# duanzhiihao/lossy-vae

Hardware: AMD Instinct MI355X
Metric: Mpixels/s enc+dec (qarv_base, 512x768) (higher is better)
Workload: dtype f32 (2-term fp16 split of every fp32 operand, hi + lo*2^-11 = 23 of 24 significant bits; 3 fp16 MFMAs per product step in two fp32 accumulators: fp32-class accuracy, parity-tested); 1 GPU; qarv_base batch=8 512x768 synthetic per GPU, compress_batch+decompress_batch, HIP kernels (f16x2) + host rANS, seeded random-init weights (profile typical); global_batch=8, parallelism=dp1 (images sharded, no data-path collective)

## Files before the change

### include/lvae_hip.h

```cpp
#ifndef LVAE_HIP_H
#define LVAE_HIP_H

#include <stddef.h>
#include <stdint.h>

#ifdef __cplusplus
extern "C" {
#endif

int lvae_abi_version(void);
const char* lvae_build_info(void);

int lvae_pmf_to_quantized_cdf(const float* pmf, int n, int precision, uint32_t* cdf_out);

int lvae_build_gaussian_tables(const float* scale_table, int n_scales, double multiplier, int cdf_form,
                               int32_t* qcdf, int row_stride, int32_t* cdf_len, int32_t* offset);

long lvae_rans_encode_with_indexes(const int32_t* sym, const uint8_t* idx, size_t n,
                                   const int32_t* qcdf, int row_stride, const int32_t* cdf_len,
                                   const int32_t* offset, uint8_t* out, size_t out_cap);

int lvae_rans_enc_step_selftest(uint64_t x, uint32_t start, uint32_t freq, uint64_t* by_division, uint64_t* by_reciprocal);

int lvae_rans_decode_with_indexes(const uint8_t* in, size_t in_len, const uint8_t* idx, size_t n,
                                  const int32_t* qcdf, int row_stride, const int32_t* cdf_len,
                                  const int32_t* offset, int32_t* sym_out);

int lvae_rans_encode_batch(int n_streams, const int32_t* const* sym, const uint8_t* const* idx, const size_t* n,
                           const int32_t* qcdf, int row_stride, const int32_t* cdf_len, const int32_t* offset,
                           uint8_t* const* out, const size_t* out_cap, long* out_len, int n_threads);
int lvae_rans_decode_batch(int n_streams, const uint8_t* const* in, const size_t* in_len,
                           const uint8_t* const* idx, const size_t* n,
                           const int32_t* qcdf, int row_stride, const int32_t* cdf_len, const int32_t* offset,
                           int32_t* const* sym_out, int* status, int n_threads);

enum {
    LVAE_STATUS_RANGE = 1, LVAE_STATUS_NONFINITE_PRIOR = 2, LVAE_STATUS_NONFINITE_LATENT = 4, LVAE_STATUS_NONFINITE_IMAGE = 8
};

enum {
    LVAE_A_PLAIN  = 0,
    LVAE_A_PATCH2 = 1,
    LVAE_A_CONV3  = 2
};
enum {
    LVAE_EPI_BIAS       = 0,
    LVAE_EPI_BIAS_GELU  = 1,
    LVAE_EPI_GAMMA_RES  = 2,
    LVAE_EPI_RES        = 3
};
enum {
    LVAE_ST_ROWMAJOR    = 0,
    LVAE_ST_SHUFFLE     = 2,
    LVAE_ST_IMAGE       = 3
};
typedef struct {
    const float* A0; const float* A1;
    long lda0, lda1;
    int  K0, K1;
    int  H, W;
    const float* Wt; long ldw;
    const float* bias;
    const float* gamma;
    const float* res; long ldres;
    float* out; long ldo;
    int  M, N, K;
    int  a_mode, epi, store, r;
    int  a_gelu;
    int  prec;
    const unsigned short* Wt16;
    int  cfg;
    int  ksplit;
    float* ws;
    int  a_bf16, out_bf16;
    int* cnt;
    int* status;
    int  a_h2, out_h2;
    int  defer_reduce;
} lvae_gemm_desc;
int lvae_gemm_f32(const lvae_gemm_desc* d, void* stream);

typedef struct {
    const void* y; const void* w1; const float* b1; const void* w2; const float* b2; const float* gamma;
    const float* res; float* out;
    int M, C, hid;
} lvae_mlp_desc;
int lvae_mlp_h2f(const lvae_mlp_desc* d, void* stream);

typedef struct {
    const void* y; const void* w1; const float* b1; const void* w2; const float* b2; const float* gamma;
    const float* res; float* out; float* ws;
    int M, C, hid, S1, S2;
} lvae_mlp_sk_desc;
int lvae_mlp_sk(const lvae_mlp_sk_desc* d, void* stream);
int lvae_mlp_sk_supported(int C, int hid, int S1, int S2);
int lvae_gemm_num_configs(void);

enum {
    LVAE_OP_GEMM = 1, LVAE_OP_DWCONV_LN_F32, LVAE_OP_DWCONV_LN_H2, LVAE_OP_DWCONV_LN_BF16, LVAE_OP_DWCONV_LN_Q8, LVAE_OP_STEM_F32, LVAE_OP_STEM_BF16,
    LVAE_OP_BIAS_EXPAND_F32, LVAE_OP_BIAS_EXPAND_BF16, LVAE_OP_PRIOR_INDEX, LVAE_OP_QUANTIZE, LVAE_OP_DEQUANTIZE, LVAE_OP_GAUSSIAN_NLL,
    LVAE_OP_LOSSLESS_PARAMS, LVAE_OP_LOSSLESS_OUTPUT, LVAE_OP_MLP_H2F, LVAE_OP_MLP_SK, LVAE_OP_PRIOR_INDEX_SK, LVAE_OP_QUANTIZE_SK,
    LVAE_OP_GAUSSIAN_NLL_CHAN, LVAE_OP_RD_IMAGE, LVAE_OP_PIXEL_NLL,
    LVAE_OP_DWCONV_LN_F32_V, LVAE_OP_DWCONV_LN_H2_V, LVAE_OP_DWCONV_LN_BF16_V, LVAE_OP_DWCONV_LN_Q8_V, LVAE_OP_ORDER
};
typedef struct { int kind; int side; void* p[8]; long i[6]; double f[2]; } lvae_op;
#define LVAE_TRACE_MAGIC 1985229328.0
int lvae_run_ops(const lvae_op* ops, int n, void* stream, void* side_stream, int* failed_index);

typedef struct {
    const lvae_op* ops; int n_ops;
    const uint8_t* idx_dev; uint8_t* idx_host;
    int32_t* sym_host; int32_t* sym_dev;
    size_t per_image;
} lvae_dec_block;
int lvae_decode_blocks(const lvae_dec_block* blocks, int n_blocks, int n_images, const uint8_t* const* strings, const size_t* string_len,
                       const int32_t* qcdf, int row_stride, const int32_t* cdf_len, const int32_t* offset,
                       const lvae_op* tail_ops, int n_tail, const int* status_dev, int* status_host, void* stream, void* side_stream,
                       int n_threads, int* failed_block, int* failed_op, double* seconds);

typedef struct {
    const lvae_op* ops; int n_ops;
    const int32_t* sym_dev; int32_t* sym_host;
    const uint8_t* idx_dev; uint8_t* idx_host;
    size_t per_image;
} lvae_enc_block;
int lvae_encode_blocks(const lvae_enc_block* blocks, int n_blocks, int n_images, uint8_t* const* out, const size_t* out_cap, long* out_len,
                       const int32_t* qcdf, int row_stride, const int32_t* cdf_len, const int32_t* offset,
                       const int* status_dev, int* status_host, void* stream, void* side_stream, int n_threads,
                       int* failed_block, int* failed_op, double* seconds);

int lvae_dwconv_ln_f32(const float* x, const float* wt, const float* bias, const float* ln_w, const float* ln_b,
                       const float* shift, const float* scale1p, float* y,
                       int B, int H, int W, int C, int k, void* stream);

int lvae_dwconv_ln_h2(const float* x, const float* wt, const float* bias, const float* ln_w, const float* ln_b,
                      const float* shift, const float* scale1p, void* y,
                      int B, int H, int W, int C, int k, void* stream);

int lvae_dwconv_ln_q8(const void* x, const float* wt, const float* bias, const float* ln_w, const float* ln_b,
                      const float* shift, const float* scale1p, void* y,
                      int B, int H, int W, int C, int k, void* stream);

int lvae_dwconv_ln_bf16(const void* x, const float* wt, const float* bias, const float* ln_w, const float* ln_b,
                        const float* shift, const float* scale1p, void* y,
                        int B, int H, int W, int C, int k, void* stream);

int lvae_dwconv_ln_f32_v(const float* x, const float* wt, const float* bias, const float* shift, const float* scale1p, float* y,
                         int B, int H, int W, int C, int k, long vstride, void* stream);
int lvae_dwconv_ln_h2_v(const float* x, const float* wt, const float* bias, const float* shift, const float* scale1p, void* y,
                        int B, int H, int W, int C, int k, long vstride, void* stream);
int lvae_dwconv_ln_bf16_v(const void* x, const float* wt, const float* bias, const float* shift, const float* scale1p, void* y,
                          int B, int H, int W, int C, int k, long vstride, void* stream);
int lvae_dwconv_ln_q8_v(const void* x, const float* wt, const float* bias, const float* shift, const float* scale1p, void* y,
                        int B, int H, int W, int C, int k, long vstride, void* stream);

int lvae_dwconv_ln_choice(int fmt, int affines, int per_image_vectors, int B, int H, int W, int C, int k,
                          int* family, int* tile_rows, int* tiles_per_wg);

int lvae_gemm_h2_choice(const lvae_gemm_desc* d, int cu_count, int* kernel, int* params , int* splitk);

int lvae_stem_bf16(const float* im, const float* wt, const float* bias, void* out,
                   int B, int H, int W, int Cout, float im_shift, float im_scale, int* range_flag, void* stream);
int lvae_bias_expand_bf16(const float* bias, void* out, long M, int C, void* stream);

int lvae_stem_f32(const float* im, const float* wt, const float* bias, float* out,
                  int B, int H, int W, int Cout, float im_shift, float im_scale, int* range_flag, void* stream);
int lvae_range_flag_f32(const float* x, long n, float lo, float hi, int* flag, void* stream);

int lvae_gemv_f32(const float* Wt, const float* b, const float* x, float* y, int N, int K,
                  int gelu_in, int gelu_out, void* stream);
int lvae_gemv_batch_f32(const float* Wt, const float* b, const float* x, float* y, int N, int K, int nvec,
                        int gelu_in, int gelu_out, void* stream);

int lvae_prior_index_f32(const float* prm, float* pm, uint8_t* idx, const float* scale_table, int n_scales,
                         float scale_bound, int B, int HW, int z, int* status, void* stream);
int lvae_prior_index_sk_f32(const float* ws, int S, const float* bias, float* prm, float* pm, uint8_t* idx, const float* scale_table,
                            int n_scales, float scale_bound, int B, int HW, int z, int* status, void* stream);

int lvae_quantize_f32(const float* qm, const float* pm, int32_t* sym, float* zhat, int B, int HW, int z, int ldz,
                      int* status, void* stream);
int lvae_quantize_sk_f32(const float* ws, int S, const float* bias, float* qm, const float* pm, int32_t* sym, float* zhat, int B, int HW,
                         int z, int ldz, int* status, void* stream);
int lvae_dequantize_f32(const int32_t* sym, const float* pm, float* zhat, int B, int HW, int z, int ldz, void* stream);

int lvae_prior_sample_f32(const float* prm, float* z, long M, int zdim, int ldz, float t, unsigned long long seed,
                          unsigned long long offset, void* stream);

int lvae_latent_sample_box_f32(const float* prm, const float* lat, float* z, int B, int h, int w, int zdim, int ldz, int r0, int r1,
                               int c0, int c1, float t, unsigned long long seed, unsigned long long offset, void* stream);

int lvae_pixel_sample_f32(const float* raw, float* out, int B, int H, int W, float t, unsigned long long seed, unsigned long long offset,
                          int* status, void* stream);

int lvae_lossless_params_f32(const float* raw, const float* im, float* pm, uint8_t* idx, int32_t* sym, const float* table,
                             int n_scales, float bound, int B, int H, int W, int* status, void* stream);

int lvae_lossless_output_f32(const int32_t* sym, const float* pm, float* out, long n, int* status, void* stream);

int lvae_gaussian_nll_f32(const float* prm, const int32_t* sym, double* out_nats, float scale_bound, int B, int HW, int z,
                          int cdf_form, void* stream);

int lvae_gaussian_nll_map_f32(const float* prm, const int32_t* sym, float* out, float scale_bound, int B, int HW, int z, int cdf_form,
                              void* stream);

#define LVAE_EVAL_CHUNKS 256

int lvae_gaussian_nll_chan_f32(const float* prm, const int32_t* sym, double* out, float scale_bound, int B, int HW, int z, int cdf_form,
                               void* stream);

int lvae_rd_image_f32(const float* raw, const float* im, float* im_hat, double* sums, double* ws, int B, int H, int W, int* status,
                      void* stream);

int lvae_pixel_nll_f32(const float* raw6, const float* im, float* im_hat, double* sums, double* ws, int B, int H, int W, int* status,
                       void* stream);

int lvae_gelu_f32(const float* x, float* y, long n, void* stream);

int lvae_bias_expand_f32(const float* bias, float* out, long M, int C, void* stream);

int lvae_sqerr_sum_f32(const float* a, const float* b, double* out, int B, long n_per_image, void* stream);
int lvae_sqerr_partials_f32(const float* a, const float* b, double* partials, int n_partials, long n, void* stream);

int lvae_msssim_f32(const float* x, long x_img, long x_plane, long x_row, const float* y, long y_img, long y_plane, long y_row,
                    const int* hw, int B, int C, int Hmax, int Wmax, double* out, double* scale_means, void* ws, size_t ws_bytes,
                    void* stream);
size_t lvae_msssim_workspace_bytes(int B, int C, int Hmax, int Wmax);

enum { LVAE_SAMPLE_F32 = 0, LVAE_SAMPLE_U8 = 1, LVAE_SAMPLE_U16_LOW = 2, LVAE_SAMPLE_U16_HIGH = 3 };
int lvae_msssim_planes(const void* const* x, const long* x_row, const void* const* y, const long* y_row, const int* hw,
                       const int* pixstride, int n, int kind, int depth, double data_range, int scales, double* out, double* scale_means,
                       void* ws, size_t ws_bytes, void* stream);
size_t lvae_msssim_planes_workspace_bytes(int n, int Hmax, int Wmax, int scales);

int lvae_image_u8_to_f32(const uint8_t* const* src, const long* src_row, const int* hw, int B, float* dst, long dst_img, int H, int W,
                         void* stream);
int lvae_image_f32_to_u8(const float* src, long src_img, long src_plane, long src_row, int H, int W, const int* hw, int B,
                         uint8_t* const* dst, const long* dst_row, void* stream);

enum { LVAE_YUV_I420 = 0, LVAE_YUV_NV12 = 1 };
enum { LVAE_YUV_BT601 = 0, LVAE_YUV_BT709 = 1 };
enum { LVAE_YUV_LIMITED = 0, LVAE_YUV_FULL = 1 };
enum { LVAE_YUV_NEAREST = 0, LVAE_YUV_BILINEAR = 1 };
int lvae_image_yuv420_to_f32(const uint8_t* const* y, const uint8_t* const* u, const uint8_t* const* v, const long* y_row,
                             const long* u_row, const long* v_row, const int* hw, int B, int fmt, int matrix, int range, int chroma,
                             float* dst, long dst_img, int H, int W, void* stream);
int lvae_image_f32_to_yuv420(const float* src, long src_img, long src_plane, long src_row, int H, int W, const int* hw, int B, int fmt,
                             int matrix, int range, uint8_t* const* y, uint8_t* const* u, uint8_t* const* v, const long* y_row,
                             const long* u_row, const long* v_row, void* stream);
int lvae_sse_u8(const uint8_t* const* a, const long* a_row, const uint8_t* const* b, const long* b_row, const int* hw, int n,
                uint64_t* out, void* stream);

enum { LVAE_YUV_SUB_420 = 0, LVAE_YUV_SUB_422 = 1, LVAE_YUV_SUB_444 = 2 };
enum { LVAE_YUV_SITING_CENTER = 0, LVAE_YUV_SITING_LEFT = 1 };
enum { LVAE_YUV_BT2020 = 2 };
int lvae_image_yuv_to_f32(const void* const* y, const void* const* u, const void* const* v, const long* y_row, const long* u_row,
                          const long* v_row, const int* hw, int B, int depth, int subsampling, int siting, int matrix, int range, int chroma,
                          float* dst, long dst_img, int H, int W, void* stream);
int lvae_image_f32_to_yuv(const float* src, long src_img, long src_plane, long src_row, int H, int W, const int* hw, int B, int depth,
                          int subsampling, int siting, int matrix, int range, void* const* y, void* const* u, void* const* v,
                          const long* y_row, const long* u_row, const long* v_row, void* stream);
int lvae_sse_u16(const uint16_t* const* a, const long* a_row, const uint16_t* const* b, const long* b_row, const int* hw, int n,
                 uint64_t* out, void* stream);

enum { LVAE_YUV_LAYOUT_PLANAR = 0, LVAE_YUV_LAYOUT_SEMIPLANAR = 1 };
int lvae_image_yuvsp_to_f32(const uint16_t* const* y, const uint16_t* const* uv, const long* y_row, const long* uv_row, const int* hw, int B,
                            int depth, int subsampling, int siting, int matrix, int range, int chroma, float* dst, long dst_img, int H, int W,
                            void* stream);
int lvae_image_f32_to_yuvsp(const float* src, long src_img, long src_plane, long src_row, int H, int W, const int* hw, int B, int depth,
                            int subsampling, int siting, int matrix, int range, uint16_t* const* y, uint16_t* const* uv, const long* y_row,
                            const long* uv_row, void* stream);

int lvae_tile_stitch(const float* const* tiles, long tile_plane, long tile_row, const int* oy, const int* ox, int rows, int cols,
                     int th, int tw, int overlap, int h, int w, int y0, int x0, int hh, int ww, void* dst, long dst_plane,
                     long dst_row, int out_u8, void* ws, size_t ws_bytes, void* stream);
size_t lvae_tile_stitch_workspace_bytes(int rows, int cols);
int lvae_tile_stitch_yuv(const float* const* tiles, long tile_plane, long tile_row, const int* oy, const int* ox, int rows, int cols, int th,
                         int tw, int overlap, int h, int w, int y0, int x0, int hh, int ww, int depth, int subsampling, int siting, int matrix,
                         int range, int layout, void* y, void* u, void* v, long y_row, long u_row, long v_row, void* ws, size_t ws_bytes,
                         void* stream);

int lvae_resample_u8_to_f32(const uint8_t* const* src, const long* src_row, int B, int h_in, int w_in, int h_out, int w_out,
                            const int* ystart, const float* ywgt, int ytaps, int yspan, const int* xstart, const float* xwgt, int xtaps,
                            float* dst, long dst_img, int H, int W, void* stream);
int lvae_resample_f32_to_u8(const float* src, long src_img, long src_plane, long src_row, int B, int h_in, int w_in, int h_out, int w_out,
                            const int* ystart, const float* ywgt, int ytaps, int yspan, const int* xstart, const float* xwgt, int xtaps,
                            uint8_t* const* dst, const long* dst_row, void* stream);
int lvae_resample_f32(const float* src, long src_img, long src_plane, long src_row, int B, int h_in, int w_in, int h_out, int w_out,
                      const int* ystart, const float* ywgt, int ytaps, int yspan, const int* xstart, const float* xwgt, int xtaps,
                      int clamp, float* dst, long dst_img, int H, int W, void* stream);

int lvae_resample_yuv_to_f32(const void* const* y, const void* const* u, const void* const* v, const long* y_row, const long* u_row,
                             const long* v_row, const int* hw, int B, int depth, int subsampling, int siting, int matrix, int range, int chroma,
                             int layout, int h_in, int w_in, int h_out, int w_out, const int* ystart, const float* ywgt, int ytaps, int yspan,
                             const int* xstart, const float* xwgt, int xtaps, int xspan, float* dst, long dst_img, int H, int W, void* stream);
int lvae_resample_f32_to_yuv(const float* src, long src_img, long src_plane, long src_row, const int* hw, int B, int depth, int subsampling,
                             int siting, int matrix, int range, int layout, int h_in, int w_in, int h_out, int w_out, const int* ystart,
                             const float* ywgt, int ytaps, int yspan, const int* xstart, const float* xwgt, int xtaps, void* const* y,
                             void* const* u, void* const* v, const long* y_row, const long* u_row, const long* v_row, void* stream);

int lvae_gaussian_nll_pos_f32(const float* prm, const int32_t* sym, double* out, float scale_bound, int B, int HW, int z, int cdf_form,
                              void* stream);
int lvae_pixel_nll_pos_f32(const float* raw6, const float* im, double* out, int B, int H, int W, int* status, void* stream);
int lvae_rate_map_f32(const double* const* pos, const int* lat_h, const int* lat_w, int n_blocks, const double* pix, int B, int H, int W,
                      float* out, long out_img, long out_row, int crop_h, int crop_w, void* stream);

void* lvae_event_create(void);
int   lvae_event_destroy(void* event);
int   lvae_stream_order(void* from_stream, void* to_stream, void* event);

#ifdef __cplusplus
}
#endif
#endif
```

### lossy-vae_amd/csrc/plan_runtime.cpp

```cpp
#include <hip/hip_runtime.h>

#include <chrono>
#include <vector>

#include "plan_ops.h"

extern "C" int lvae_run_ops(const lvae_op* ops, int n, void* stream, void* side_stream, int* failed_index) {
    if (!ops || n < 0) return -22;
    for (int k = 0; k < n; ++k) {
        const lvae_op& o = ops[k];
        int rc = -22;
        if (o.kind == LVAE_OP_ORDER)
            rc = o.i[0] ? lvae_stream_order(stream, side_stream, o.p[0]) : lvae_stream_order(side_stream, stream, o.p[0]);
        else if (o.kind >= 1 && o.kind <= lvae_plan::n_ops)
            rc = lvae_plan::op_table[o.kind - 1].run(o, o.side ? side_stream : stream);
        if (rc != 0) {
            if (failed_index) *failed_index = k;
            return rc;
        }
    }
    return 0;
}


struct LvaeDecTabs;
LvaeDecTabs* lvae_dec_tabs_new();
void lvae_dec_tabs_free(LvaeDecTabs* t);
int lvae_rans_decode_batch_tabs(int n_streams, const uint8_t* const* in, const size_t* in_len, const uint8_t* const* idx,
                                const size_t* n, const int32_t* qcdf, int row_stride, const int32_t* cdf_len, const int32_t* offset,
                                int32_t* const* sym_out, int* status, int n_threads, LvaeDecTabs* tabs);

struct LvaeEncJob;
LvaeEncJob* lvae_rans_encode_batch_begin(int n_streams, const int32_t* const* sym, const uint8_t* const* idx, const size_t* n,
                                         const int32_t* qcdf, int row_stride, const int32_t* cdf_len, const int32_t* offset,
                                         uint8_t* const* out, const size_t* out_cap, long* out_len, int n_threads);
int lvae_rans_encode_batch_end(LvaeEncJob* e);

namespace {
inline double now_s() { return std::chrono::duration<double>(std::chrono::steady_clock::now().time_since_epoch()).count(); }
}

static int decode_blocks_impl(const lvae_dec_block* blocks, int n_blocks, int n_images, const uint8_t* const* strings,
                              const size_t* string_len, const int32_t* qcdf, int row_stride, const int32_t* cdf_len,
                              const int32_t* offset, const lvae_op* tail_ops, int n_tail, const int* status_dev, int* status_host,
                              void* stream, void* side_stream, int n_threads, int* failed_block, int* failed_op, double* seconds) {
    if (!blocks || n_blocks < 0 || n_images <= 0 || !strings || !string_len || !qcdf || !cdf_len || !offset) return -22;
    hipStream_t st = (hipStream_t)stream;
    std::vector<const uint8_t*> idx_ptr(n_images);
    std::vector<int32_t*> out_ptr(n_images);
    std::vector<size_t> cnt(n_images);
    std::vector<int> status(n_images);
    struct TabsGuard { LvaeDecTabs* t; ~TabsGuard() { lvae_dec_tabs_free(t); } } tabs{lvae_dec_tabs_new()};
    if (!tabs.t) return -12;
    double t_gpu = 0.0, t_coder = 0.0;
    int bad = -1;
    const int trace_cap = (seconds && seconds[0] <= -8.0 && seconds[0] >= -4096.0 && seconds[1] == LVAE_TRACE_MAGIC) ? (int)(-seconds[0]) : 0;
    auto stamp = [&](int slot, double t) { if (slot < trace_cap) seconds[slot] = t; };
    for (int b = 0; b < n_blocks; ++b) {
        const lvae_dec_block& k = blocks[b];
        const double t0 = now_s();
        int rc = lvae_run_ops(k.ops, k.n_ops, stream, side_stream, &bad);
        if (rc == 0 && k.idx_dev) rc = (int)hipMemcpyAsync(k.idx_host, k.idx_dev, k.per_image * n_images, hipMemcpyDeviceToHost, st);
        const double t_issued = now_s();
        if (rc == 0) {
            hipError_t q = hipErrorNotReady;
            for (int it = 0; it < 400000 && (q = hipStreamQuery(st)) == hipErrorNotReady; ++it) {}
            rc = q == hipErrorNotReady ? (int)hipStreamSynchronize(st) : (int)q;
        }
        if (rc != 0) {
            if (failed_block) *failed_block = b;
            if (failed_op) *failed_op = bad;
            return rc;
        }
        const double t1 = now_s();
        for (int i = 0; i < n_images; ++i) {
            idx_ptr[i] = k.idx_host + (size_t)i * k.per_image;
            out_ptr[i] = k.sym_host + (size_t)i * k.per_image;
            cnt[i] = k.per_image;
        }
        rc = lvae_rans_decode_batch_tabs(n_images, strings + (size_t)b * n_images, string_len + (size_t)b * n_images, idx_ptr.data(), cnt.data(),
                                         qcdf, row_stride, cdf_len, offset, out_ptr.data(), status.data(), n_threads, tabs.t);
        if (rc != 0) {
            if (failed_block) *failed_block = b;
            if (status_dev && status_host && hipMemcpyAsync(status_host, status_dev, sizeof(int), hipMemcpyDeviceToHost, st) == hipSuccess &&
                hipStreamSynchronize(st) == hipSuccess && *status_host != 0)
                return -75;
            return -74;
        }
        if (k.sym_dev) rc = (int)hipMemcpyAsync(k.sym_dev, k.sym_host, k.per_image * n_images * sizeof(int32_t), hipMemcpyHostToDevice, st);
        if (rc != 0) {
            if (failed_block) *failed_block = b;
            return rc;
        }
        const double t2 = now_s();
        t_gpu += t1 - t0; t_coder += t2 - t1;
        stamp(2 + 4 * b, t0); stamp(3 + 4 * b, t_issued); stamp(4 + 4 * b, t1); stamp(5 + 4 * b, t2);
    }
    if (n_tail > 0) {
        int rc = lvae_run_ops(tail_ops, n_tail, stream, side_stream, &bad);
        if (rc == 0 && status_dev && status_host) rc = (int)hipMemcpyAsync(status_host, status_dev, sizeof(int), hipMemcpyDeviceToHost, st);
        if (rc != 0) {
            if (failed_block) *failed_block = n_blocks;
            if (failed_op) *failed_op = bad;
            return rc;
        }
    }
    stamp(2 + 4 * n_blocks, now_s());
    if (seconds) { seconds[0] = t_gpu; seconds[1] = t_coder; }
    return 0;
}

static int encode_blocks_impl(const lvae_enc_block* blocks, int n_blocks, int n_images, uint8_t* const* out, const size_t* out_cap,
                              long* out_len, const int32_t* qcdf, int row_stride, const int32_t* cdf_len, const int32_t* offset,
                              const int* status_dev, int* status_host, void* stream, void* side_stream, int n_threads,
                              int* failed_block, int* failed_op, double* seconds) {
    if (!blocks || n_blocks <= 0 || n_images <= 0 || !out || !out_cap || !out_len || !qcdf || !cdf_len || !offset) return -22;
    hipStream_t st = (hipStream_t)stream;
    std::vector<hipEvent_t> ev(n_blocks, nullptr);
    auto cleanup = [&]() { for (hipEvent_t e : ev) if (e) (void)hipEventDestroy(e); };
    const double t0 = now_s();
    int bad = -1;
    for (int b = 0; b < n_blocks; ++b) {
        const lvae_enc_block& k = blocks[b];
        int rc = lvae_run_ops(k.ops, k.n_ops, stream, side_stream, &bad);
        if (rc == 0 && k.sym_dev) rc = (int)hipMemcpyAsync(k.sym_host, k.sym_dev, k.per_image * n_images * sizeof(int32_t), hipMemcpyDeviceToHost, st);
        if (rc == 0 && k.idx_dev) rc = (int)hipMemcpyAsync(k.idx_host, k.idx_dev, k.per_image * n_images, hipMemcpyDeviceToHost, st);
        if (rc == 0 && b == n_blocks - 1 && status_dev && status_host) rc = (int)hipMemcpyAsync(status_host, status_dev, sizeof(int), hipMemcpyDeviceToHost, st);
        if (rc == 0) rc = (int)hipEventCreateWithFlags(&ev[b], hipEventDisableTiming);
        if (rc == 0) rc = (int)hipEventRecord(ev[b], st);
        if (rc != 0) {
            if (failed_block) *failed_block = b;
            if (failed_op) *failed_op = bad;
            (void)hipStreamSynchronize(st);
            cleanup();
            return rc;
        }
    }
    const double t1 = now_s();
    std::vector<const int32_t*> sym_ptr(n_images);
    std::vector<const uint8_t*> idx_ptr(n_images);
    std::vector<size_t> cnt(n_images);
    std::vector<LvaeEncJob*> jobs(n_blocks, nullptr);
    double t_wait = 0.0, t_coder = 0.0;
    int rc_all = 0, bad_block = -1;
    for (int b = 0; b < n_blocks && rc_all == 0; ++b) {
        const lvae_enc_block& k = blocks[b];
        const double tw = now_s();
        int rc = (int)hipEventSynchronize(ev[b]);
        t_wait += now_s() - tw;
        if (rc == 0 && b == n_blocks - 1 && status_dev && status_host && *status_host != 0) rc = (*status_host & LVAE_STATUS_RANGE) ? -34 : -75;
        if (rc == 0) {
            for (int i = 0; i < n_images; ++i) {
                sym_ptr[i] = k.sym_host + (size_t)i * k.per_image;
                idx_ptr[i] = k.idx_host + (size_t)i * k.per_image;
                cnt[i] = k.per_image;
            }
            jobs[b] = lvae_rans_encode_batch_begin(n_images, sym_ptr.data(), idx_ptr.data(), cnt.data(), qcdf, row_stride, cdf_len, offset,
                                                   out + (size_t)b * n_images, out_cap + (size_t)b * n_images, out_len + (size_t)b * n_images, n_threads);
            if (!jobs[b]) rc = -12;
        }
        if (rc != 0) { rc_all = rc; bad_block = b; }
    }
    const double tc = now_s();
    for (int b = 0; b < n_blocks; ++b) {
        if (!jobs[b]) continue;
        const int rc = lvae_rans_encode_batch_end(jobs[b]);
        if (rc != 0 && rc_all == 0) { rc_all = rc; bad_block = b; }
    }
    t_coder = now_s() - tc;
    if (rc_all != 0) {
        if (failed_block) *failed_block = bad_block;
        (void)hipStreamSynchronize(st);
        cleanup();
        return rc_all;
    }
    cleanup();
    if (seconds) { seconds[0] = t1 - t0; seconds[1] = t_wait; seconds[2] = t_coder; }
    return 0;
}

extern "C" int lvae_decode_blocks(const lvae_dec_block* blocks, int n_blocks, int n_images, const uint8_t* const* strings,
                                  const size_t* string_len, const int32_t* qcdf, int row_stride, const int32_t* cdf_len,
                                  const int32_t* offset, const lvae_op* tail_ops, int n_tail, const int* status_dev, int* status_host,
                                  void* stream, void* side_stream, int n_threads, int* failed_block, int* failed_op, double* seconds) {
    try {
        return decode_blocks_impl(blocks, n_blocks, n_images, strings, string_len, qcdf, row_stride, cdf_len, offset, tail_ops, n_tail, status_dev,
                                  status_host, stream, side_stream, n_threads, failed_block, failed_op, seconds);
    } catch (...) {
        (void)hipStreamSynchronize((hipStream_t)stream);
        return -12;
    }
}

extern "C" int lvae_encode_blocks(const lvae_enc_block* blocks, int n_blocks, int n_images, uint8_t* const* out, const size_t* out_cap,
                                  long* out_len, const int32_t* qcdf, int row_stride, const int32_t* cdf_len, const int32_t* offset,
                                  const int* status_dev, int* status_host, void* stream, void* side_stream, int n_threads,
                                  int* failed_block, int* failed_op, double* seconds) {
    try {
        return encode_blocks_impl(blocks, n_blocks, n_images, out, out_cap, out_len, qcdf, row_stride, cdf_len, offset, status_dev, status_host,
                                  stream, side_stream, n_threads, failed_block, failed_op, seconds);
    } catch (...) {
        (void)hipStreamSynchronize((hipStream_t)stream);
        return -12;
    }
}
```

### lossy-vae_amd/csrc/pointwise.hip

```cpp
#include <hip/hip_runtime.h>
#include <stdint.h>

#include "../../include/lvae_hip.h"
#include "device_math.h"
#include "rate_terms.h"
#include "dwconv_choice.h"

namespace {

typedef float f32x4 __attribute__((ext_vector_type(4)));
typedef unsigned int u32x2 __attribute__((ext_vector_type(2)));

template <bool BF>
__device__ __forceinline__ f32x4 ld4(const void* base, long off) {
    if (BF) {
        const u32x2 q = *(const u32x2*)((const unsigned short*)base + off);
        return (f32x4){__uint_as_float(q[0] << 16), __uint_as_float(q[0] & 0xffff0000u), __uint_as_float(q[1] << 16),
                       __uint_as_float(q[1] & 0xffff0000u)};
    }
    return *(const f32x4*)((const float*)base + off);
}
__device__ __forceinline__ unsigned f2bf(float x) {
    const unsigned u = __float_as_uint(x);
    return (u + 0x7fffu + ((u >> 16) & 1u)) >> 16;
// ... 171 lines not shown
    switch (C) {
        case 128: return launch_dwln_th<KS, 2, 16, 1, true>(x, wt, bias, ln_w, ln_b, shift, scale1p, y, B, H, W, st);
        case 192: return launch_dwln_th<KS, 3, 16, 1, true>(x, wt, bias, ln_w, ln_b, shift, scale1p, y, B, H, W, st);
        case 256: return launch_dwln_th<KS, 2, 32, 1, true>(x, wt, bias, ln_w, ln_b, shift, scale1p, y, B, H, W, st);
        case 384: return launch_dwln_th<KS, 3, 32, 1, true>(x, wt, bias, ln_w, ln_b, shift, scale1p, y, B, H, W, st);
        case 512: return launch_dwln_th<KS, 4, 32, 1, true>(x, wt, bias, ln_w, ln_b, shift, scale1p, y, B, H, W, st);
    }
    return -22;
}

template <bool BF>
__global__ __launch_bounds__(256) void stem_kernel(const float* __restrict__ im, const float* __restrict__ wt, const float* __restrict__ bias,
                            void* __restrict__ out, int B, int H, int W, int Cout, float im_shift, float im_scale, long M,
                            int* __restrict__ range_flag) {
    __shared__ __attribute__((aligned(16))) float patch[64][48];
    const int n = threadIdx.x;
    const int Ho = H / 4, Wo = W / 4;
    const long p0 = (long)blockIdx.x * 64;
    bool bad = false;
    for (int e = n; e < 64 * 48; e += blockDim.x) {
        const int j = e & 3, p = (e >> 2) & 63, ci_i = e >> 8;
        const long pg = p0 + p;
        float v = 0.f;
        if (pg < M) {
            const int wo = (int)(pg % Wo);
            const long bho = pg / Wo;
            const int ho = (int)(bho % Ho);
            const long b = bho / Ho;
            const int ci = ci_i >> 2, i = ci_i & 3;
            v = im[((b * 3 + ci) * H + (4 * ho + i)) * (long)W + 4 * wo + j];
            bad |= !(v >= 0.0f && v <= 1.0f);
            v = (v + im_shift) * im_scale;
        }
        patch[p][ci_i * 4 + j] = v;
    }
    if (range_flag && bad) atomicOr(range_flag, 1);
    float wr[48];
#pragma unroll
    for (int k = 0; k < 48; ++k) wr[k] = wt[k * Cout + n];
    const float bv = bias[n];
    __syncthreads();
    for (int p = 0; p < 64; p += 4) {
        if (p0 + p >= M) break;
        float a[4] = {bv, bv, bv, bv};
#pragma unroll
        for (int k4 = 0; k4 < 12; ++k4) {
#pragma unroll
            for (int q = 0; q < 4; ++q) {
                const f32x4 pv = *(const f32x4*)&patch[p + q][k4 * 4];
                a[q] = fmaf(pv[0], wr[k4 * 4 + 0], a[q]);
                a[q] = fmaf(pv[1], wr[k4 * 4 + 1], a[q]);
                a[q] = fmaf(pv[2], wr[k4 * 4 + 2], a[q]);
                a[q] = fmaf(pv[3], wr[k4 * 4 + 3], a[q]);
            }
        }
#pragma unroll
        for (int q = 0; q < 4; ++q) {
            const long pg = p0 + p + q;
            if (pg < M) {
                if (BF) ((unsigned short*)out)[pg * Cout + n] = (unsigned short)f2bf(a[q]);
                else ((float*)out)[pg * Cout + n] = a[q];
            }
        }
    }
}

__global__ __launch_bounds__(256) void gemv_kernel(const float* __restrict__ Wt, const float* __restrict__ b,
                                                   const float* __restrict__ x, float* __restrict__ y, int N, int K,
                                                   int gelu_in, int gelu_out) {
    const int lane = threadIdx.x & 63;
    const int n = blockIdx.x * 4 + (threadIdx.x >> 6);
    if (n >= N) return;
    float s = 0.f;
    for (int k = lane * 4; k < K; k += 256) {
        const f32x4 wv = *(const f32x4*)(Wt + (long)n * K + k);
        f32x4 xv = *(const f32x4*)(x + k);
        if (gelu_in) { xv[0] = gelu_erf(xv[0]); xv[1] = gelu_erf(xv[1]); xv[2] = gelu_erf(xv[2]); xv[3] = gelu_erf(xv[3]); }
        s = fmaf(wv[0], xv[0], s); s = fmaf(wv[1], xv[1], s); s = fmaf(wv[2], xv[2], s); s = fmaf(wv[3], xv[3], s);
    }
#pragma unroll
    for (int o = 32; o > 0; o >>= 1) s += __shfl_xor(s, o, 64);
    if (lane == 0) {
        s += b[n];
        y[n] = gelu_out ? gelu_erf(s) : s;
    }
}

constexpr int GEMV_NB = 8, GEMV_KR = 4;
template <bool WREG>
__global__ __launch_bounds__(256) void gemv_batch_kernel(const float* __restrict__ Wt, const float* __restrict__ b,
                                                         const float* __restrict__ x, float* __restrict__ y, int N, int K, int nvec,
                                                         int gelu_in, int gelu_out) {
    const int lane = threadIdx.x & 63;
    const int n = blockIdx.x * 4 + (threadIdx.x >> 6);
    if (n >= N) return;
    f32x4 wr[GEMV_KR];
    if constexpr (WREG) {
#pragma unroll
        for (int t = 0; t < GEMV_KR; ++t) {
            const int k = lane * 4 + 256 * t;
            wr[t] = k < K ? *(const f32x4*)(Wt + (long)n * K + k) : (f32x4){0.f, 0.f, 0.f, 0.f};
        }
    }
    for (int i0 = 0; i0 < nvec; i0 += GEMV_NB) {
        float s[GEMV_NB];
#pragma unroll
        for (int i = 0; i < GEMV_NB; ++i) s[i] = 0.f;
        auto step = [&](const f32x4 wv, int k) {
#pragma unroll
            for (int i = 0; i < GEMV_NB; ++i) {
                if (i0 + i < nvec) {
                    f32x4 xv = *(const f32x4*)(x + (long)(i0 + i) * K + k);
                    if (gelu_in) { xv[0] = gelu_erf(xv[0]); xv[1] = gelu_erf(xv[1]); xv[2] = gelu_erf(xv[2]); xv[3] = gelu_erf(xv[3]); }
                    s[i] = fmaf(wv[0], xv[0], s[i]); s[i] = fmaf(wv[1], xv[1], s[i]); s[i] = fmaf(wv[2], xv[2], s[i]); s[i] = fmaf(wv[3], xv[3], s[i]);
                }
            }
        };
        if constexpr (WREG) {
#pragma unroll
            for (int t = 0; t < GEMV_KR; ++t) {
                const int k = lane * 4 + 256 * t;
                if (k < K) step(wr[t], k);
            }
        } else {
            for (int k = lane * 4; k < K; k += 256) step(*(const f32x4*)(Wt + (long)n * K + k), k);
        }
#pragma unroll
        for (int i = 0; i < GEMV_NB; ++i) {
            float t = s[i];
#pragma unroll
            for (int o = 32; o > 0; o >>= 1) t += __shfl_xor(t, o, 64);
            if (lane == 0 && i0 + i < nvec) {
                t += b[n];
                y[(long)(i0 + i) * N + n] = gelu_out ? gelu_erf(t) : t;
            }
        }
    }
}

__global__ void lossless_params_kernel(const float* __restrict__ raw, const float* __restrict__ im, float* __restrict__ pm,
                                       uint8_t* __restrict__ idx, int32_t* __restrict__ sym, const float* __restrict__ table,
                                       int n_scales, float bound, long total, int HW, int* __restrict__ status) {
#pragma clang fp contract(off)
    const long e = (long)blockIdx.x * blockDim.x + threadIdx.x;
    if (e >= total) return;
    const long bc = e / HW;
    const int p = (int)(e - bc * HW);
    const long b = bc / 3;
    const int c = (int)(bc - b * 3);
    const float* r = raw + (b * HW + p) * 6;
    const float bin = (float)(1.0 / 127.5);
    float m = r[c] * 127.5f;
    m = m + 127.5f;
    m = rintf(m) / 127.5f;
    m = m - 1.0f;
    m = m / bin;
    if (status && !(fabsf(r[c]) <= 3.4028234664e38f && fabsf(r[3 + c]) <= 3.4028234664e38f)) atomicOr(status, LVAE_STATUS_NONFINITE_PRIOR);
    const float ls = r[3 + c] - (float)(-4.848116360536466);
    const float s = fmaxf(expf(ls), bound);
    int lo = 0, hi = n_scales - 1;
    while (lo < hi) {
        const int mid = (lo + hi) >> 1;
        if (table[mid] < s) lo = mid + 1; else hi = mid;
    }
    pm[e] = m;
    idx[e] = (uint8_t)lo;
    if (im) {
        float x = im[e] - 0.5f;
        x = x * 2.0f;
        x = x / bin;
        sym[e] = (int32_t)rintf(x - m);
    }
}

__global__ void lossless_output_kernel(const int32_t* __restrict__ sym, const float* __restrict__ pm, float* __restrict__ out, long n,
                                       int* __restrict__ status) {
#pragma clang fp contract(off)
    const long e = (long)blockIdx.x * blockDim.x + threadIdx.x;
    if (e >= n) return;
    float x = (float)sym[e] + pm[e];
    if (status && !(fabsf(x) <= 3.4028234664e38f)) atomicOr(status, LVAE_STATUS_NONFINITE_IMAGE);
    x = x * (float)(1.0 / 127.5);
    x = fminf(fmaxf(x, -1.0f), 1.0f);
    x = x * 0.5f;
    out[e] = x + 0.5f;
}

__device__ __forceinline__ void philox4x32_10(uint32_t c0, uint32_t c1, uint32_t c2, uint32_t c3, uint32_t k0, uint32_t k1,
                                              uint32_t (&out)[4]) {
#pragma unroll
    for (int r = 0; r < 10; ++r) {
        const uint64_t p0 = (uint64_t)0xD2511F53u * c0, p1 = (uint64_t)0xCD9E8D57u * c2;
        const uint32_t n0 = (uint32_t)(p1 >> 32) ^ c1 ^ k0, n1 = (uint32_t)p1;
        const uint32_t n2 = (uint32_t)(p0 >> 32) ^ c3 ^ k1, n3 = (uint32_t)p0;
        c0 = n0; c1 = n1; c2 = n2; c3 = n3;
        k0 += 0x9E3779B9u; k1 += 0xBB67AE85u;
    }
    out[0] = c0; out[1] = c1; out[2] = c2; out[3] = c3;
}

__device__ __forceinline__ void philox_variates(uint64_t seed, uint64_t ctr, float& nrm, float& uni) {
    uint32_t r[4];
    philox4x32_10((uint32_t)ctr, (uint32_t)(ctr >> 32), 0u, 0u, (uint32_t)seed, (uint32_t)(seed >> 32), r);
    const float u1 = ((float)(r[0] >> 8) + 0.5f) * (1.0f / 16777216.0f);
    const float u2 = ((float)(r[1] >> 8) + 0.5f) * (1.0f / 16777216.0f);
    nrm = sqrtf(-2.0f * logf(u1)) * cospif(2.0f * u2);
    uni = ((float)(r[2] >> 8) + 0.5f) * (1.0f / 16777216.0f) - 0.5f;
}

__device__ __forceinline__ float prior_draw(float mean, float lv, float t, uint64_t seed, uint64_t ctr) {
    const float xs = lv + 2.3f;
    const float sp = xs > 20.0f ? xs : log1pf(expf(xs));
    const float pv = expf(sp - 2.3f);
    float nrm, uni;
    philox_variates(seed, ctr, nrm, uni);
    return mean + pv * nrm * t + uni * t;
}

__global__ void prior_sample_kernel(const float* __restrict__ prm, float* __restrict__ z, long total, int zdim, int ldz, float t,
                                    uint64_t seed, uint64_t offset) {
    const long e = (long)blockIdx.x * blockDim.x + threadIdx.x;
    if (e >= total) return;
    const long m = e / ldz;
    const int c = (int)(e - m * ldz);
    if (c >= zdim) { z[e] = 0.f; return; }
    z[e] = prior_draw(prm[m * 2 * zdim + c], prm[m * 2 * zdim + zdim + c], t, seed, offset + (uint64_t)(m * zdim + c));
}

__global__ void pixel_sample_kernel(const float* __restrict__ raw, float* __restrict__ out, long total, int HW, float t, uint64_t seed,
                                    uint64_t offset, int* __restrict__ status) {
#pragma clang fp contract(off)
    const long e = (long)blockIdx.x * blockDim.x + threadIdx.x;
    if (e >= total) return;
    const long bc = e / HW;
    const int p = (int)(e - bc * HW);
    const long b = bc / 3;
    const int c = (int)(bc - b * 3);
    const float* r = raw + (b * HW + p) * 6;
    float nrm, uni;
    philox_variates(seed, offset + (uint64_t)e, nrm, uni);
    float s = expf(r[3 + c]);
    s = s * t;
    float x = s * nrm;
    x = r[c] + x;
    if (status && !(fabsf(x) <= 3.4028234664e38f)) atomicOr(status, LVAE_STATUS_NONFINITE_IMAGE);
    x = fminf(fmaxf(x, -1.0f), 1.0f);
    x = x * 0.5f;
    out[e] = x + 0.5f;
}

constexpr int CT_PIX = 64, CT_CH = 16, CT_LD = CT_PIX + 1;

template <bool SK>
__global__ __launch_bounds__(256) void prior_index_kernel(const float* __restrict__ prm_in, float* __restrict__ pm, uint8_t* __restrict__ idx,
                                                          const float* __restrict__ table, int n_scales, float bound, int HW, int z,
                                                          int* __restrict__ status, const float* __restrict__ ws, int S, long plane,
                                                          const float* __restrict__ bias, float* __restrict__ prm_out) {
#pragma clang fp contract(off)
    __shared__ int tile[CT_CH * CT_LD];
    __shared__ float tab[256];
    if ((int)threadIdx.x < n_scales) tab[threadIdx.x] = table[threadIdx.x];
    __syncthreads();
    const int b = blockIdx.z, p0 = blockIdx.x * CT_PIX, np = (HW - p0) < CT_PIX ? (HW - p0) : CT_PIX;
    const long m0 = (long)b * HW + p0;
    {
        const int c0 = blockIdx.y * CT_CH;
        const int zc = (z - c0) < CT_CH ? (z - c0) : CT_CH;
        for (int i = threadIdx.x; i < np * zc; i += 256) {
            const int pl = i / zc, c = c0 + (i - pl * zc);
            const long m = m0 + pl;
            float mean, lv;
            if constexpr (SK) {
                const float* w = ws + m * 2 * z + c;
                mean = w[0]; lv = w[z];
                for (int sl = 1; sl < S; ++sl) { mean += w[sl * plane]; lv += w[sl * plane + z]; }
                mean += bias[c]; lv += bias[z + c];
                prm_out[m * 2 * z + c] = mean; prm_out[m * 2 * z + z + c] = lv;
            } else {
                mean = prm_in[m * 2 * z + c];
                lv = prm_in[m * 2 * z + z + c];
            }
            if (status && !(fabsf(mean) <= 3.4028234664e38f && fabsf(lv) <= 3.4028234664e38f)) atomicOr(status, LVAE_STATUS_NONFINITE_PRIOR);
            const float xs = lv + 2.3f;
            const float sp = xs > 20.0f ? xs : log1pf(expf(xs));
            const float pv = expf(sp - 2.3f);
            const float sc = fmaxf(pv, bound);
            int lo = 0, hi = n_scales - 1;
            while (lo < hi) {
                const int mid = (lo + hi) >> 1;
                if (tab[mid] < sc) lo = mid + 1; else hi = mid;
            }
            pm[m * z + c] = mean;
            tile[(c - c0) * CT_LD + pl] = lo;
        }
        __syncthreads();
        for (int j = threadIdx.x; j < zc * CT_PIX; j += 256) {
            const int cl = j / CT_PIX, pl = j - cl * CT_PIX;
            if (pl < np) idx[((long)b * z + c0 + cl) * HW + p0 + pl] = (uint8_t)tile[cl * CT_LD + pl];
        }
        __syncthreads();
    }
}

template <bool SK>
__global__ __launch_bounds__(256) void quantize_kernel(const float* __restrict__ qm, const float* __restrict__ pm, int32_t* __restrict__ sym,
                                                       float* __restrict__ zhat, int HW, int z, int ldz, int* __restrict__ status,
                                                       const float* __restrict__ ws, int S, long plane, const float* __restrict__ bias,
                                                       float* __restrict__ qm_out) {
#pragma clang fp contract(off)
    __shared__ int tile[CT_CH * CT_LD];
    const int b = blockIdx.z, p0 = blockIdx.x * CT_PIX, np = (HW - p0) < CT_PIX ? (HW - p0) : CT_PIX;
    const long m0 = (long)b * HW + p0;
    {
        const int c0 = blockIdx.y * CT_CH;
        const int zc = (ldz - c0) < CT_CH ? (ldz - c0) : CT_CH;
        for (int i = threadIdx.x; i < np * zc; i += 256) {
            const int pl = i / zc, c = c0 + (i - pl * zc);
            const long m = m0 + pl;
            if (c >= z) { zhat[m * ldz + c] = 0.f; continue; }
            const float mu = pm[m * z + c];
            float q;
            if constexpr (SK) {
                const float* w = ws + m * z + c;
                q = w[0];
                for (int sl = 1; sl < S; ++sl) q += w[sl * plane];
                q += bias[c];
                qm_out[m * z + c] = q;
            } else {
                q = qm[m * z + c];
            }
            const float r = rintf(q - mu);
            if (status && !(fabsf(r) < 2147483648.0f)) atomicOr(status, LVAE_STATUS_NONFINITE_LATENT);
            zhat[m * ldz + c] = r + mu;
            tile[(c - c0) * CT_LD + pl] = (int32_t)r;
        }
        __syncthreads();
        for (int j = threadIdx.x; j < zc * CT_PIX; j += 256) {
            const int cl = j / CT_PIX, pl = j - cl * CT_PIX;
            if (pl < np && c0 + cl < z) sym[((long)b * z + c0 + cl) * HW + p0 + pl] = tile[cl * CT_LD + pl];
        }
        __syncthreads();
    }
}

__global__ __launch_bounds__(256) void dequantize_kernel(const int32_t* __restrict__ sym, const float* __restrict__ pm, float* __restrict__ zhat,
                                                         int HW, int z, int ldz) {
    __shared__ int tile[CT_CH * CT_LD];
    const int b = blockIdx.z, p0 = blockIdx.x * CT_PIX, np = (HW - p0) < CT_PIX ? (HW - p0) : CT_PIX;
    const long m0 = (long)b * HW + p0;
    {
        const int c0 = blockIdx.y * CT_CH;
        const int zc = (ldz - c0) < CT_CH ? (ldz - c0) : CT_CH;
        for (int j = threadIdx.x; j < zc * CT_PIX; j += 256) {
            const int cl = j / CT_PIX, pl = j - cl * CT_PIX;
            if (pl < np && c0 + cl < z) tile[cl * CT_LD + pl] = sym[((long)b * z + c0 + cl) * HW + p0 + pl];
        }
        __syncthreads();
        for (int i = threadIdx.x; i < np * zc; i += 256) {
            const int pl = i / zc, c = c0 + (i - pl * zc);
            const long m = m0 + pl;
            zhat[m * ldz + c] = c >= z ? 0.f : (float)tile[(c - c0) * CT_LD + pl] + pm[m * z + c];
        }
        __syncthreads();
    }
}

__global__ __launch_bounds__(256) void latent_sample_box_kernel(const float* __restrict__ prm, const float* __restrict__ lat,
                                                                float* __restrict__ zout, int HW, int w, int zdim, int ldz, int r0,
                                                                int r1, int c0b, int c1b, float t, uint64_t seed, uint64_t offset) {
    __shared__ float tile[CT_CH * CT_LD];
    const int b = blockIdx.z, p0 = blockIdx.x * CT_PIX, np = (HW - p0) < CT_PIX ? (HW - p0) : CT_PIX;
    const long m0 = (long)b * HW + p0;
    const int c0 = blockIdx.y * CT_CH;
    const int zc = (ldz - c0) < CT_CH ? (ldz - c0) : CT_CH;
    if (lat) {
        for (int j = threadIdx.x; j < zc * CT_PIX; j += 256) {
            const int cl = j / CT_PIX, pl = j - cl * CT_PIX;
            if (pl < np && c0 + cl < zdim) tile[cl * CT_LD + pl] = lat[((long)b * zdim + c0 + cl) * HW + p0 + pl];
        }
        __syncthreads();
    }
    for (int i = threadIdx.x; i < np * zc; i += 256) {
        const int pl = i / zc, c = c0 + (i - pl * zc);
        const long m = m0 + pl;
        float v = 0.f;
        if (c < zdim) {
            const int p = p0 + pl, y = p / w, x = p - y * w;
            if (!lat || (y >= r0 && y < r1 && x >= c0b && x < c1b))
                v = prior_draw(prm[m * 2 * zdim + c], prm[m * 2 * zdim + zdim + c], t, seed, offset + (uint64_t)(m * zdim + c));
            else
                v = tile[(c - c0) * CT_LD + pl];
        }
        zout[m * ldz + c] = v;
    }
}

__global__ __launch_bounds__(256) void gaussian_nll_kernel(const float* __restrict__ prm, const int32_t* __restrict__ sym,
                                                           double* __restrict__ out, float bound, long per_image, int HW,
                                                           int z, int cdf_form) {
    const int b = blockIdx.y;
    double acc = 0.0;
    for (long e = (long)blockIdx.x * 256 + threadIdx.x; e < per_image; e += (long)gridDim.x * 256) {
        const long p = e / z;
        const int c = (int)(e - p * z);
        const long m = (long)b * HW + p;
        acc -= (double)gaussian_logp(prm[m * 2 * z + z + c], sym[((long)b * z + c) * HW + p], bound, cdf_form);
    }
#pragma unroll
    for (int o = 32; o > 0; o >>= 1) acc += __shfl_xor(acc, o, 64);
    __shared__ double ws[4];
    if ((threadIdx.x & 63) == 0) ws[threadIdx.x >> 6] = acc;
    __syncthreads();
    if (threadIdx.x == 0) atomicAdd(out + b, ws[0] + ws[1] + ws[2] + ws[3]);
}

__global__ __launch_bounds__(256) void gaussian_nll_map_kernel(const float* __restrict__ prm, const int32_t* __restrict__ sym,
                                                               float* __restrict__ out, float bound, long total, int HW, int z,
                                                               int cdf_form) {
    const long e = (long)blockIdx.x * 256 + threadIdx.x;
    if (e >= total) return;
    const long bc = e / HW;
    const int p = (int)(e - bc * HW);
    const long b = bc / z;
    const int c = (int)(bc - b * z);
    out[e] = -gaussian_logp(prm[(b * HW + p) * 2 * z + z + c], sym[e], bound, cdf_form);
}


template <int NT>
__device__ __forceinline__ double wg_sum_f64(double v, double* ws ) {
#pragma unroll
    for (int o = 32; o > 0; o >>= 1) v += __shfl_xor(v, o, 64);
    if ((threadIdx.x & 63) == 0) ws[threadIdx.x >> 6] = v;
    __syncthreads();
    double s = 0.0;
    if (threadIdx.x == 0)
        for (int w = 0; w < NT / 64; ++w) s += ws[w];
    return s;
}

template <int NT>
__global__ __launch_bounds__(NT) void gaussian_nll_chan_kernel(const float* __restrict__ prm, const int32_t* __restrict__ sym,
                                                               double* __restrict__ out, float bound, int HW, int z, int cdf_form) {
    __shared__ double ws[NT / 64];
    const int c = blockIdx.x, b = blockIdx.y;
    const int32_t* sc = sym + ((long)b * z + c) * HW;
    const float* lv = prm + (long)b * HW * 2 * z + z + c;
    double acc = 0.0;
    for (int p = threadIdx.x; p < HW; p += NT) acc += (double)(-gaussian_logp(lv[(long)p * 2 * z], sc[p], bound, cdf_form));
    acc = wg_sum_f64<NT>(acc, ws);
    if (threadIdx.x == 0) out[(long)b * z + c] = acc;
}

constexpr int EV_WG = 256;

__device__ __forceinline__ void eval_chunk(int HW, int& p_lo, int& p_hi) {
    const int cs = (HW + LVAE_EVAL_CHUNKS - 1) / LVAE_EVAL_CHUNKS;
    p_lo = blockIdx.x * cs;
    p_hi = (HW - p_lo) < cs ? HW : p_lo + cs;
}

__global__ __launch_bounds__(64) void eval_sums_kernel(const double* __restrict__ ws, double* __restrict__ sums) {
    const int b = blockIdx.x;
    const double* w = ws + (long)b * LVAE_EVAL_CHUNKS * 2;
#pragma unroll
    for (int q = 0; q < 2; ++q) {
        double s = 0.0;
        for (int k = threadIdx.x; k < LVAE_EVAL_CHUNKS; k += 64) s += w[2 * k + q];
#pragma unroll
        for (int o = 32; o > 0; o >>= 1) s += __shfl_xor(s, o, 64);
        if (threadIdx.x == 0) sums[2 * b + q] = s;
    }
}

__global__ __launch_bounds__(EV_WG) void rd_image_kernel(const float* __restrict__ raw, const float* __restrict__ im,
                                                         float* __restrict__ im_hat, double* __restrict__ part, int HW,
                                                         int* __restrict__ status) {
    __shared__ double ws[EV_WG / 64];
    const int b = blockIdx.y;
    int p_lo, p_hi;
    eval_chunk(HW, p_lo, p_hi);
    const float* r = raw + (long)b * HW * 3;
    const float* x = im + (long)b * 3 * HW;
    float* o = im_hat + (long)b * 3 * HW;
    double se = 0.0, sq = 0.0;
    bool bad = false;
    for (int p0 = p_lo + threadIdx.x; p0 < p_hi; p0 += 4 * EV_WG) {
        float vv[4][3], tt[4][3];
#pragma unroll
        for (int u = 0; u < 4; ++u) {
            const int p = p0 + u * EV_WG;
#pragma unroll
            for (int c = 0; c < 3; ++c) {
                vv[u][c] = p < p_hi ? r[(long)p * 3 + c] : 0.0f;
                tt[u][c] = p < p_hi ? x[(long)c * HW + p] : 0.0f;
            }
        }
#pragma unroll
        for (int u = 0; u < 4; ++u) {
            const int p = p0 + u * EV_WG;
            if (p >= p_hi) continue;
#pragma unroll
            for (int c = 0; c < 3; ++c) {
                const float v = vv[u][c], t = tt[u][c];
                bad |= !(fabsf(v) <= 3.4028234664e38f);
                const float h = fminf(fmaxf(v, -1.0f), 1.0f) * 0.5f + 0.5f;
                o[(long)c * HW + p] = h;
                const float d = v - (t - 0.5f) * 2.0f, e = h - t;
                se += (double)d * (double)d;
                sq += (double)e * (double)e;
            }
        }
    }
    if (status && bad) atomicOr(status, LVAE_STATUS_NONFINITE_IMAGE);
    se = wg_sum_f64<EV_WG>(se, ws);
    __syncthreads();
    sq = wg_sum_f64<EV_WG>(sq, ws);
    if (threadIdx.x == 0) {
        double* w = part + ((long)b * LVAE_EVAL_CHUNKS + blockIdx.x) * 2;
        w[0] = se;
        w[1] = sq;
    }
}

__global__ __launch_bounds__(EV_WG) void pixel_nll_kernel(const float* __restrict__ raw, const float* __restrict__ im,
                                                          float* __restrict__ im_hat, double* __restrict__ part, int HW,
                                                          int* __restrict__ status) {
#pragma clang fp contract(off)
    __shared__ double ws[EV_WG / 64];
    const int b = blockIdx.y;
    int p_lo, p_hi;
    eval_chunk(HW, p_lo, p_hi);
    const float* r6 = raw + (long)b * HW * 6;
    const float* xi = im + (long)b * 3 * HW;
    float* o = im_hat + (long)b * 3 * HW;
    double nll = 0.0, sq = 0.0;
    bool bad = false;
    for (int p = p_lo + threadIdx.x; p < p_hi; p += EV_WG) {
#pragma unroll
        for (int c = 0; c < 3; ++c) {
            const float m = r6[(long)p * 6 + c];
            const float t = xi[(long)c * HW + p];
            const float lp = pixel_logp(m, r6[(long)p * 6 + 3 + c], t);
            bad |= !(fabsf(m) <= 3.4028234664e38f) || !(fabsf(lp) <= 3.4028234664e38f);
            const float h = fminf(fmaxf(m, -1.0f), 1.0f) * 0.5f + 0.5f;
            o[(long)c * HW + p] = h;
            const float e = h - t;
            nll -= (double)lp;
            sq += (double)e * (double)e;
        }
    }
    if (status && bad) atomicOr(status, LVAE_STATUS_NONFINITE_IMAGE);
    nll = wg_sum_f64<EV_WG>(nll, ws);
    __syncthreads();
    sq = wg_sum_f64<EV_WG>(sq, ws);
    if (threadIdx.x == 0) {
        double* w = part + ((long)b * LVAE_EVAL_CHUNKS + blockIdx.x) * 2;
        w[0] = nll;
        w[1] = sq;
    }
}

__global__ void bias_expand_kernel(const float* __restrict__ bias, float* __restrict__ out, long total4, int C4) {
    const long e = (long)blockIdx.x * blockDim.x + threadIdx.x;
    if (e >= total4) return;
    ((f32x4*)out)[e] = ((const f32x4*)bias)[e % C4];
}

__global__ __launch_bounds__(256) void sqerr_kernel(const float* __restrict__ a, const float* __restrict__ b,
                                                    double* __restrict__ out, long n) {
    const int img = blockIdx.y;
    const float* pa = a + (long)img * n;
    const float* pb = b + (long)img * n;
    double s = 0.0;
    for (long i = (long)blockIdx.x * 256 + threadIdx.x; i < n; i += (long)gridDim.x * 256) {
        const float dlt = pa[i] - pb[i];
        s += (double)dlt * (double)dlt;
    }
#pragma unroll
    for (int o = 32; o > 0; o >>= 1) s += __shfl_xor(s, o, 64);
    __shared__ double ws[4];
    if ((threadIdx.x & 63) == 0) ws[threadIdx.x >> 6] = s;
    __syncthreads();
    if (threadIdx.x == 0) atomicAdd(out + img, ws[0] + ws[1] + ws[2] + ws[3]);
}

}

int lvae_dwln_cl_launch(int fmt, int C, int k, const void* x, const float* wt, const float* bias, const float* aw, const float* ab, void* y,
                        int B, int H, int W, int th, int tpw, long vs, hipStream_t st);

static int dwln(int fmt, const long* vstride, const void* x, const float* wt, const float* bias, const float* ln_w, const float* ln_b,
                const float* shift, const float* scale1p, void* y, int B, int H, int W, int C, int k, void* stream) {
    if (!x || !wt || !bias || !y || B <= 0 || H <= 0 || W <= 0) return -22;
    if (vstride ? (!shift || !scale1p || *vstride < 0) : ((ln_w == nullptr) != (ln_b == nullptr) || (shift == nullptr) != (scale1p == nullptr))) return -22;
    hipStream_t st = (hipStream_t)stream;
    lvae_dwln::Choice ch;
    const int rc = lvae_dwln::choose(fmt, (ln_w ? 1 : 0) + (shift ? 1 : 0), vstride != nullptr, B, H, W, C, k, &ch);
    if (rc) return rc;
    if (ch.family == 0)
        return lvae_dwln_cl_launch(fmt, C, k, x, wt, bias, ln_w ? ln_w : scale1p, ln_w ? ln_b : shift, y, B, H, W, ch.tile_rows, ch.tiles_per_wg,
                                   vstride ? *vstride : 0, st);
    const float* xf = (const float*)x;
    float* yf = (float*)y;
    const int th = ch.tile_rows;
    switch (k) {
        case 1: return fmt ? dispatch_dwln_bf16<1>(C, x, wt, bias, ln_w, ln_b, shift, scale1p, y, B, H, W, st)
                           : dispatch_dwln_c<1>(C, xf, wt, bias, ln_w, ln_b, shift, scale1p, yf, B, H, W, th, st);
        case 3: return fmt ? dispatch_dwln_bf16<3>(C, x, wt, bias, ln_w, ln_b, shift, scale1p, y, B, H, W, st)
                           : dispatch_dwln_c<3>(C, xf, wt, bias, ln_w, ln_b, shift, scale1p, yf, B, H, W, th, st);
        case 5: return fmt ? dispatch_dwln_bf16<5>(C, x, wt, bias, ln_w, ln_b, shift, scale1p, y, B, H, W, st)
                           : dispatch_dwln_c<5>(C, xf, wt, bias, ln_w, ln_b, shift, scale1p, yf, B, H, W, th, st);
        case 7: return fmt ? dispatch_dwln_bf16<7>(C, x, wt, bias, ln_w, ln_b, shift, scale1p, y, B, H, W, st)
                           : dispatch_dwln_c<7>(C, xf, wt, bias, ln_w, ln_b, shift, scale1p, yf, B, H, W, th, st);
    }
    return -22;
}

extern "C" int lvae_dwconv_ln_choice(int fmt, int affines, int per_image_vectors, int B, int H, int W, int C, int k, int* family,
                                     int* tile_rows, int* tiles_per_wg) {
    lvae_dwln::Choice ch;
    const int rc = lvae_dwln::choose(fmt, affines, per_image_vectors, B, H, W, C, k, &ch);
    if (rc) return rc;
    if (family) *family = ch.family;
    if (tile_rows) *tile_rows = ch.tile_rows;
    if (tiles_per_wg) *tiles_per_wg = ch.tiles_per_wg;
    return 0;
}

extern "C" int lvae_dwconv_ln_f32(const float* x, const float* wt, const float* bias, const float* ln_w, const float* ln_b,
                                  const float* shift, const float* scale1p, float* y, int B, int H, int W, int C, int k, void* stream) {
    return dwln(0, nullptr, x, wt, bias, ln_w, ln_b, shift, scale1p, y, B, H, W, C, k, stream);
}
extern "C" int lvae_dwconv_ln_bf16(const void* x, const float* wt, const float* bias, const float* ln_w, const float* ln_b,
                                   const float* shift, const float* scale1p, void* y, int B, int H, int W, int C, int k, void* stream) {
    return dwln(1, nullptr, x, wt, bias, ln_w, ln_b, shift, scale1p, y, B, H, W, C, k, stream);
}
extern "C" int lvae_dwconv_ln_h2(const float* x, const float* wt, const float* bias, const float* ln_w, const float* ln_b,
                                 const float* shift, const float* scale1p, void* y, int B, int H, int W, int C, int k, void* stream) {
    return dwln(2, nullptr, x, wt, bias, ln_w, ln_b, shift, scale1p, y, B, H, W, C, k, stream);
}
extern "C" int lvae_dwconv_ln_q8(const void* x, const float* wt, const float* bias, const float* ln_w, const float* ln_b,
                                 const float* shift, const float* scale1p, void* y, int B, int H, int W, int C, int k, void* stream) {
    return dwln(3, nullptr, x, wt, bias, ln_w, ln_b, shift, scale1p, y, B, H, W, C, k, stream);
}
extern "C" int lvae_dwconv_ln_f32_v(const float* x, const float* wt, const float* bias, const float* shift, const float* scale1p, float* y,
                                    int B, int H, int W, int C, int k, long vstride, void* stream) {
    return dwln(0, &vstride, x, wt, bias, nullptr, nullptr, shift, scale1p, y, B, H, W, C, k, stream);
}
extern "C" int lvae_dwconv_ln_bf16_v(const void* x, const float* wt, const float* bias, const float* shift, const float* scale1p, void* y,
                                     int B, int H, int W, int C, int k, long vstride, void* stream) {
    return dwln(1, &vstride, x, wt, bias, nullptr, nullptr, shift, scale1p, y, B, H, W, C, k, stream);
}
extern "C" int lvae_dwconv_ln_h2_v(const float* x, const float* wt, const float* bias, const float* shift, const float* scale1p, void* y,
                                   int B, int H, int W, int C, int k, long vstride, void* stream) {
    return dwln(2, &vstride, x, wt, bias, nullptr, nullptr, shift, scale1p, y, B, H, W, C, k, stream);
}
extern "C" int lvae_dwconv_ln_q8_v(const void* x, const float* wt, const float* bias, const float* shift, const float* scale1p, void* y,
                                   int B, int H, int W, int C, int k, long vstride, void* stream) {
    return dwln(3, &vstride, x, wt, bias, nullptr, nullptr, shift, scale1p, y, B, H, W, C, k, stream);
}

template <bool BF>
static int stem(const float* im, const float* wt, const float* bias, void* out, int B, int H, int W, int Cout, float im_shift, float im_scale,
                int* range_flag, void* stream) {
    if (!im || !wt || !bias || !out || B <= 0 || (H & 3) || (W & 3) || Cout <= 0 || Cout > 256) return -22;
    const long M = (long)B * (H / 4) * (W / 4);
    hipLaunchKernelGGL(stem_kernel<BF>, dim3((unsigned)((M + 63) / 64)), dim3(Cout), 0, (hipStream_t)stream, im, wt, bias, out,
                       B, H, W, Cout, im_shift, im_scale, M, range_flag);
    return (int)hipGetLastError();
}
extern "C" int lvae_stem_f32(const float* im, const float* wt, const float* bias, float* out, int B, int H, int W,
                             int Cout, float im_shift, float im_scale, int* range_flag, void* stream) {
    return stem<false>(im, wt, bias, out, B, H, W, Cout, im_shift, im_scale, range_flag, stream);
}
extern "C" int lvae_stem_bf16(const float* im, const float* wt, const float* bias, void* out, int B, int H, int W,
                              int Cout, float im_shift, float im_scale, int* range_flag, void* stream) {
    return stem<true>(im, wt, bias, out, B, H, W, Cout, im_shift, im_scale, range_flag, stream);
}

namespace {
__global__ void bias_expand_bf16_kernel(const float* __restrict__ bias, unsigned short* __restrict__ out, long total4, int C4) {
    const long e = (long)blockIdx.x * blockDim.x + threadIdx.x;
    if (e >= total4) return;
    st4<true>(out, e * 4, ((const f32x4*)bias)[e % C4]);
}
}

extern "C" int lvae_bias_expand_bf16(const float* bias, void* out, long M, int C, void* stream) {
    if (!bias || !out || M <= 0 || C <= 0 || (C & 3)) return -22;
    const long total4 = M * (C / 4);
    hipLaunchKernelGGL(bias_expand_bf16_kernel, dim3((unsigned)((total4 + 255) / 256)), dim3(256), 0, (hipStream_t)stream, bias,
                       (unsigned short*)out, total4, C / 4);
    return (int)hipGetLastError();
}

namespace {
__global__ __launch_bounds__(256) void range_flag_kernel(const float* __restrict__ x, long n4, float lo, float hi, int* __restrict__ flag) {
    bool bad = false;
    for (long i = (long)blockIdx.x * 256 + threadIdx.x; i < n4; i += (long)gridDim.x * 256) {
        const f32x4 v = ((const f32x4*)x)[i];
#pragma unroll
        for (int e = 0; e < 4; ++e) bad |= !(v[e] >= lo && v[e] <= hi);
    }
    if (bad) atomicOr(flag, 1);
}
}

extern "C" int lvae_range_flag_f32(const float* x, long n, float lo, float hi, int* flag, void* stream) {
    if (!x || !flag || n <= 0 || (n & 3)) return -22;
    const long n4 = n / 4;
    long bx = (n4 + 256 * 8 - 1) / (256 * 8);
    if (bx > 2048) bx = 2048;
    hipLaunchKernelGGL(range_flag_kernel, dim3((unsigned)bx), dim3(256), 0, (hipStream_t)stream, x, n4, lo, hi, flag);
    return (int)hipGetLastError();
}

extern "C" int lvae_gemv_f32(const float* Wt, const float* b, const float* x, float* y, int N, int K, int gelu_in,
                             int gelu_out, void* stream) {
    if (!Wt || !b || !x || !y || N <= 0 || K <= 0 || (K & 3)) return -22;
    hipLaunchKernelGGL(gemv_kernel, dim3((N + 3) / 4), dim3(256), 0, (hipStream_t)stream, Wt, b, x, y, N, K, gelu_in,
                       gelu_out);
    return (int)hipGetLastError();
}

extern "C" int lvae_gemv_batch_f32(const float* Wt, const float* b, const float* x, float* y, int N, int K, int nvec, int gelu_in,
                                   int gelu_out, void* stream) {
    if (!Wt || !b || !x || !y || N <= 0 || K <= 0 || (K & 3) || nvec <= 0) return -22;
    if (K <= 256 * GEMV_KR)
        hipLaunchKernelGGL(gemv_batch_kernel<true>, dim3((N + 3) / 4), dim3(256), 0, (hipStream_t)stream, Wt, b, x, y, N, K, nvec, gelu_in,
                           gelu_out);
    else
        hipLaunchKernelGGL(gemv_batch_kernel<false>, dim3((N + 3) / 4), dim3(256), 0, (hipStream_t)stream, Wt, b, x, y, N, K, nvec, gelu_in,
                           gelu_out);
    return (int)hipGetLastError();
}

extern "C" int lvae_prior_index_f32(const float* prm, float* pm, uint8_t* idx, const float* scale_table, int n_scales,
                                    float scale_bound, int B, int HW, int z, int* status, void* stream) {
    if (!prm || !pm || !idx || !scale_table || n_scales < 2 || n_scales > 256 || B <= 0 || B > 65535 || HW <= 0 || z <= 0) return -22;
    hipLaunchKernelGGL(prior_index_kernel<false>, dim3((unsigned)((HW + CT_PIX - 1) / CT_PIX), (unsigned)((z + CT_CH - 1) / CT_CH), (unsigned)B), dim3(256), 0, (hipStream_t)stream, prm, pm,
                       idx, scale_table, n_scales, scale_bound, HW, z, status, (const float*)nullptr, 0, 0L, (const float*)nullptr, (float*)nullptr);
    return (int)hipGetLastError();
}

extern "C" int lvae_prior_index_sk_f32(const float* ws, int S, const float* bias, float* prm, float* pm, uint8_t* idx, const float* scale_table,
                                       int n_scales, float scale_bound, int B, int HW, int z, int* status, void* stream) {
    if (!ws || S < 2 || !bias || !prm || !pm || !idx || !scale_table || n_scales < 2 || n_scales > 256 || B <= 0 || B > 65535 || HW <= 0 || z <= 0) return -22;
    hipLaunchKernelGGL(prior_index_kernel<true>, dim3((unsigned)((HW + CT_PIX - 1) / CT_PIX), (unsigned)((z + CT_CH - 1) / CT_CH), (unsigned)B), dim3(256), 0, (hipStream_t)stream,
                       (const float*)nullptr, pm, idx, scale_table, n_scales, scale_bound, HW, z, status, ws, S, (long)B * HW * 2 * z, bias, prm);
    return (int)hipGetLastError();
}

extern "C" int lvae_quantize_f32(const float* qm, const float* pm, int32_t* sym, float* zhat, int B, int HW, int z, int ldz,
                                 int* status, void* stream) {
    if (!qm || !pm || !sym || !zhat || B <= 0 || B > 65535 || HW <= 0 || z <= 0 || ldz < z) return -22;
    hipLaunchKernelGGL(quantize_kernel<false>, dim3((unsigned)((HW + CT_PIX - 1) / CT_PIX), (unsigned)((ldz + CT_CH - 1) / CT_CH), (unsigned)B), dim3(256), 0, (hipStream_t)stream, qm, pm, sym,
                       zhat, HW, z, ldz, status, (const float*)nullptr, 0, 0L, (const float*)nullptr, (float*)nullptr);
    return (int)hipGetLastError();
}

extern "C" int lvae_quantize_sk_f32(const float* ws, int S, const float* bias, float* qm, const float* pm, int32_t* sym, float* zhat, int B, int HW,
                                    int z, int ldz, int* status, void* stream) {
    if (!ws || S < 2 || !bias || !qm || !pm || !sym || !zhat || B <= 0 || B > 65535 || HW <= 0 || z <= 0 || ldz < z) return -22;
    hipLaunchKernelGGL(quantize_kernel<true>, dim3((unsigned)((HW + CT_PIX - 1) / CT_PIX), (unsigned)((ldz + CT_CH - 1) / CT_CH), (unsigned)B), dim3(256), 0, (hipStream_t)stream,
                       (const float*)nullptr, pm, sym, zhat, HW, z, ldz, status, ws, S, (long)B * HW * z, bias, qm);
    return (int)hipGetLastError();
}

extern "C" int lvae_dequantize_f32(const int32_t* sym, const float* pm, float* zhat, int B, int HW, int z, int ldz,
                                   void* stream) {
    if (!sym || !pm || !zhat || B <= 0 || B > 65535 || HW <= 0 || z <= 0 || ldz < z) return -22;
    hipLaunchKernelGGL(dequantize_kernel, dim3((unsigned)((HW + CT_PIX - 1) / CT_PIX), (unsigned)((ldz + CT_CH - 1) / CT_CH), (unsigned)B), dim3(256), 0, (hipStream_t)stream, sym, pm,
                       zhat, HW, z, ldz);
    return (int)hipGetLastError();
}

extern "C" int lvae_gaussian_nll_f32(const float* prm, const int32_t* sym, double* out_nats, float scale_bound, int B, int HW,
                                     int z, int cdf_form, void* stream) {
    if (!prm || !sym || !out_nats || B <= 0 || HW <= 0 || z <= 0 || (cdf_form != 0 && cdf_form != 1)) return -22;
    const long per_image = (long)HW * z;
    long bx = (per_image + 256 * 4 - 1) / (256 * 4);
    if (bx > 512) bx = 512;
    hipLaunchKernelGGL(gaussian_nll_kernel, dim3((unsigned)bx, (unsigned)B), dim3(256), 0, (hipStream_t)stream, prm, sym, out_nats,
                       scale_bound, per_image, HW, z, cdf_form);
    return (int)hipGetLastError();
}

extern "C" int lvae_gaussian_nll_map_f32(const float* prm, const int32_t* sym, float* out, float scale_bound, int B, int HW, int z,
                                         int cdf_form, void* stream) {
    if (!prm || !sym || !out || B <= 0 || HW <= 0 || z <= 0 || (cdf_form != 0 && cdf_form != 1)) return -22;
    const long total = (long)B * HW * z;
    hipLaunchKernelGGL(gaussian_nll_map_kernel, dim3((unsigned)((total + 255) / 256)), dim3(256), 0, (hipStream_t)stream, prm, sym, out,
                       scale_bound, total, HW, z, cdf_form);
    return (int)hipGetLastError();
}

extern "C" int lvae_gaussian_nll_chan_f32(const float* prm, const int32_t* sym, double* out, float scale_bound, int B, int HW, int z,
                                          int cdf_form, void* stream) {
    if (!prm || !sym || !out || B <= 0 || B > 65535 || HW <= 0 || z <= 0 || (cdf_form != 0 && cdf_form != 1)) return -22;
    if (HW <= 8192)
        hipLaunchKernelGGL(gaussian_nll_chan_kernel<256>, dim3((unsigned)z, (unsigned)B), dim3(256), 0, (hipStream_t)stream, prm, sym, out,
                           scale_bound, HW, z, cdf_form);
    else
        hipLaunchKernelGGL(gaussian_nll_chan_kernel<1024>, dim3((unsigned)z, (unsigned)B), dim3(1024), 0, (hipStream_t)stream, prm, sym, out,
                           scale_bound, HW, z, cdf_form);
    return (int)hipGetLastError();
}

extern "C" int lvae_rd_image_f32(const float* raw, const float* im, float* im_hat, double* sums, double* ws, int B, int H, int W, int* status,
                                 void* stream) {
    if (!raw || !im || !im_hat || !sums || !ws || B <= 0 || B > 65535 || H <= 0 || W <= 0 || (long)H * W * 6 > 0x7fffffffL) return -22;
    hipLaunchKernelGGL(rd_image_kernel, dim3(LVAE_EVAL_CHUNKS, (unsigned)B), dim3(EV_WG), 0, (hipStream_t)stream, raw, im, im_hat, ws, H * W,
                       status);
    hipLaunchKernelGGL(eval_sums_kernel, dim3((unsigned)B), dim3(64), 0, (hipStream_t)stream, ws, sums);
    return (int)hipGetLastError();
}

extern "C" int lvae_pixel_nll_f32(const float* raw6, const float* im, float* im_hat, double* sums, double* ws, int B, int H, int W, int* status,
                                  void* stream) {
    if (!raw6 || !im || !im_hat || !sums || !ws || B <= 0 || B > 65535 || H <= 0 || W <= 0 || (long)H * W * 6 > 0x7fffffffL) return -22;
    hipLaunchKernelGGL(pixel_nll_kernel, dim3(LVAE_EVAL_CHUNKS, (unsigned)B), dim3(EV_WG), 0, (hipStream_t)stream, raw6, im, im_hat, ws, H * W,
                       status);
    hipLaunchKernelGGL(eval_sums_kernel, dim3((unsigned)B), dim3(64), 0, (hipStream_t)stream, ws, sums);
    return (int)hipGetLastError();
}

extern "C" int lvae_bias_expand_f32(const float* bias, float* out, long M, int C, void* stream) {
    if (!bias || !out || M <= 0 || C <= 0 || (C & 3)) return -22;
    const long total4 = M * (C / 4);
    hipLaunchKernelGGL(bias_expand_kernel, dim3((unsigned)((total4 + 255) / 256)), dim3(256), 0, (hipStream_t)stream, bias,
                       out, total4, C / 4);
    return (int)hipGetLastError();
}

namespace {
__global__ __launch_bounds__(256) void sqerr_partials_kernel(const float* __restrict__ a, const float* __restrict__ b,
                                                             double* __restrict__ partials, long n) {
    double s = 0.0;
    for (long i = (long)blockIdx.x * 256 + threadIdx.x; i < n; i += (long)gridDim.x * 256) {
        const float dlt = a[i] - b[i];
        s += (double)dlt * (double)dlt;
    }
#pragma unroll
    for (int o = 32; o > 0; o >>= 1) s += __shfl_xor(s, o, 64);
    __shared__ double ws[4];
    if ((threadIdx.x & 63) == 0) ws[threadIdx.x >> 6] = s;
    __syncthreads();
    if (threadIdx.x == 0) partials[blockIdx.x] = (ws[0] + ws[1]) + (ws[2] + ws[3]);
}
}

extern "C" int lvae_sqerr_partials_f32(const float* a, const float* b, double* partials, int n_partials, long n, void* stream) {
    if (!a || !b || !partials || n_partials <= 0 || n <= 0) return -22;
    hipLaunchKernelGGL(sqerr_partials_kernel, dim3((unsigned)n_partials), dim3(256), 0, (hipStream_t)stream, a, b, partials, n);
    return (int)hipGetLastError();
}

extern "C" int lvae_sqerr_sum_f32(const float* a, const float* b, double* out, int B, long n_per_image, void* stream) {
    if (!a || !b || !out || B <= 0 || n_per_image <= 0) return -22;
    long bx = (n_per_image + 256 * 8 - 1) / (256 * 8);
    if (bx > 1024) bx = 1024;
    hipLaunchKernelGGL(sqerr_kernel, dim3((unsigned)bx, (unsigned)B), dim3(256), 0, (hipStream_t)stream, a, b, out,
                       n_per_image);
    return (int)hipGetLastError();
}

namespace {
__global__ void gelu_kernel(const float* __restrict__ x, float* __restrict__ y, long n) {
    const long i = (long)blockIdx.x * blockDim.x + threadIdx.x;
    if (i < n) y[i] = gelu_erf(x[i]);
}
}

extern "C" int lvae_gelu_f32(const float* x, float* y, long n, void* stream) {
    if (!x || !y || n <= 0) return -22;
    hipLaunchKernelGGL(gelu_kernel, dim3((unsigned)((n + 255) / 256)), dim3(256), 0, (hipStream_t)stream, x, y, n);
    return (int)hipGetLastError();
}

extern "C" int lvae_prior_sample_f32(const float* prm, float* z, long M, int zdim, int ldz, float t, unsigned long long seed,
                                     unsigned long long offset, void* stream) {
    if (!prm || !z || M <= 0 || zdim <= 0 || ldz < zdim) return -22;
    const long total = M * ldz;
    hipLaunchKernelGGL(prior_sample_kernel, dim3((unsigned)((total + 255) / 256)), dim3(256), 0, (hipStream_t)stream, prm, z, total,
                       zdim, ldz, t, (uint64_t)seed, (uint64_t)offset);
    return (int)hipGetLastError();
}

extern "C" int lvae_latent_sample_box_f32(const float* prm, const float* lat, float* z, int B, int h, int w, int zdim, int ldz, int r0,
                                          int r1, int c0, int c1, float t, unsigned long long seed, unsigned long long offset,
                                          void* stream) {
    if (!prm || !z || B <= 0 || B > 65535 || h <= 0 || w <= 0 || zdim <= 0 || ldz < zdim || (long)h * w > 0x7fffffffL) return -22;
    const int HW = h * w;
    hipLaunchKernelGGL(latent_sample_box_kernel, dim3((unsigned)((HW + CT_PIX - 1) / CT_PIX), (unsigned)((ldz + CT_CH - 1) / CT_CH), (unsigned)B),
                       dim3(256), 0, (hipStream_t)stream, prm, lat, z, HW, w, zdim, ldz, r0, r1, c0, c1, t, (uint64_t)seed, (uint64_t)offset);
    return (int)hipGetLastError();
}

extern "C" int lvae_pixel_sample_f32(const float* raw, float* out, int B, int H, int W, float t, unsigned long long seed,
                                     unsigned long long offset, int* status, void* stream) {
    if (!raw || !out || B <= 0 || H <= 0 || W <= 0 || (long)H * W > 0x7fffffffL) return -22;
    const long total = (long)B * 3 * H * W;
    hipLaunchKernelGGL(pixel_sample_kernel, dim3((unsigned)((total + 255) / 256)), dim3(256), 0, (hipStream_t)stream, raw, out, total, H * W,
                       t, (uint64_t)seed, (uint64_t)offset, status);
    return (int)hipGetLastError();
}

extern "C" int lvae_lossless_params_f32(const float* raw, const float* im, float* pm, uint8_t* idx, int32_t* sym, const float* table,
                                        int n_scales, float bound, int B, int H, int W, int* status, void* stream) {
    if (!raw || !pm || !idx || !table || n_scales <= 0 || n_scales > 256 || B <= 0 || H <= 0 || W <= 0 || (im && !sym)) return -22;
    const long total = (long)B * 3 * H * W;
    hipLaunchKernelGGL(lossless_params_kernel, dim3((unsigned)((total + 255) / 256)), dim3(256), 0, (hipStream_t)stream, raw, im, pm,
                       idx, sym, table, n_scales, bound, total, H * W, status);
    return (int)hipGetLastError();
}

extern "C" int lvae_lossless_output_f32(const int32_t* sym, const float* pm, float* out, long n, int* status, void* stream) {
    if (!sym || !pm || !out || n <= 0) return -22;
    hipLaunchKernelGGL(lossless_output_kernel, dim3((unsigned)((n + 255) / 256)), dim3(256), 0, (hipStream_t)stream, sym, pm, out, n, status);
    return (int)hipGetLastError();
}

extern "C" void* lvae_event_create(void) {
    hipEvent_t e = nullptr;
    if (hipEventCreateWithFlags(&e, hipEventDisableTiming) != hipSuccess) return nullptr;
    return (void*)e;
}
extern "C" int lvae_event_destroy(void* ev) { return ev ? (int)hipEventDestroy((hipEvent_t)ev) : -22; }
extern "C" int lvae_stream_order(void* from_stream, void* to_stream, void* ev) {
    if (!ev) return -22;
    hipError_t e = hipEventRecord((hipEvent_t)ev, (hipStream_t)from_stream);
    if (e != hipSuccess) return (int)e;
    return (int)hipStreamWaitEvent((hipStream_t)to_stream, (hipEvent_t)ev, 0);
}

extern "C" int lvae_abi_version(void) { return 27; }
extern "C" const char* lvae_build_info(void) { return "liblvae_hip gfx950 (MI355X) fp32-MFMA; hipcc " __VERSION__; }
```

### lossy-vae_amd/csrc/rans_host.cpp

```cpp
#include <atomic>
#include <cmath>
#include <cstdint>
#include <cstdlib>
#include <cstring>
#include <condition_variable>
#include <deque>
#include <memory>
#include <mutex>
#include <new>
#include <thread>
#include <vector>

#include "../../include/lvae_hip.h"

namespace {
constexpr uint32_t kPrecision = 16;
constexpr uint32_t kBypassPrecision = 4;
constexpr int32_t kMaxBypassVal = (1 << kBypassPrecision) - 1;
constexpr uint64_t kRansL = 1ull << 31;
constexpr int32_t kMaxCdfLen = 257, kMinCdfLenEnc = 3, kMinCdfLenDec = 2;

struct BackWriter {
    uint32_t* base;
    uint32_t* ptr;
    bool overflow = false;
    inline void put(uint32_t w) {
        if (ptr == base) { overflow = true; return; }
        *--ptr = w;
    }
};

inline void enc_put(uint64_t& x, BackWriter& w, uint32_t start, uint32_t freq) {
    const uint64_t x_max = ((kRansL >> kPrecision) << 32) * freq;
    if (x >= x_max) { w.put((uint32_t)x); x >>= 32; }
    x = ((x / freq) << kPrecision) + (x % freq) + start;
}
inline void enc_put_bits(uint64_t& x, BackWriter& w, uint32_t val) {
    const uint32_t freq = 1u << (16 - kBypassPrecision);
    const uint64_t x_max = ((kRansL >> 16) << 32) * freq;
    if (x >= x_max) { w.put((uint32_t)x); x >>= 32; }
    x = (x << kBypassPrecision) | val;
}
inline uint32_t dec_get_bits(uint64_t& x, const uint32_t*& ptr, const uint32_t* end, bool& overrun) {
    const uint32_t val = (uint32_t)(x & ((1u << kBypassPrecision) - 1));
    x >>= kBypassPrecision;
    if (x < kRansL) {
        uint32_t w = 0;
        if (ptr < end) w = *ptr; else overrun = true;
        ++ptr;
        x = (x << 32) | w;
    }
    return val;
}
}

extern "C" int lvae_pmf_to_quantized_cdf(const float* pmf, int n, int precision, uint32_t* cdf) {
    if (n <= 0 || precision <= 0 || precision > 16) return -22;
    for (int i = 0; i < n; ++i)
        if (pmf[i] < 0 || !std::isfinite(pmf[i])) return -1;
    cdf[0] = 0;
    const float scale = (float)(1 << precision);
    for (int i = 0; i < n; ++i) cdf[i + 1] = (uint32_t)std::round(pmf[i] * scale);
    uint32_t total = 0;
    for (int i = 0; i <= n; ++i) total += cdf[i];
    if (total == 0) return -2;
    for (int i = 0; i <= n; ++i) cdf[i] = (uint32_t)((((uint64_t)1 << precision) * cdf[i]) / total);
    for (int i = 1; i <= n; ++i) cdf[i] += cdf[i - 1];
    cdf[n] = 1u << precision;
    for (int i = 0; i < n; ++i) {
        if (cdf[i] != cdf[i + 1]) continue;
        uint32_t best_freq = ~0u;
        int best = -1;
        for (int j = 0; j < n; ++j) {
            const uint32_t f = cdf[j + 1] - cdf[j];
            if (f > 1 && f < best_freq) { best_freq = f; best = j; }
        }
        if (best < 0) return -3;
        if (best < i) for (int j = best + 1; j <= i; ++j) cdf[j]--;
        else          for (int j = i + 1; j <= best; ++j) cdf[j]++;
    }
    return 0;
}

extern "C" int lvae_build_gaussian_tables(const float* scale_table, int n_scales, double multiplier, int cdf_form,
                                          int32_t* qcdf, int row_stride, int32_t* cdf_len, int32_t* offset) {
    if (n_scales <= 0) return -22;
    int max_len = 0;
    std::vector<int> centers(n_scales);
    const float mult = (float)multiplier;
    for (int i = 0; i < n_scales; ++i) {
        centers[i] = (int)std::ceil(scale_table[i] * mult);
        max_len = std::max(max_len, 2 * centers[i] + 1);
    }
    if (max_len + 2 > row_stride) return -2;
    auto phi = [cdf_form](float v) -> float {
        if (cdf_form == 0) return 0.5f * (1.0f + (float)erf((double)(v / (float)M_SQRT2)));
        return 0.5f * (float)erfc((double)(-(float)M_SQRT1_2 * v));
    };
    std::vector<float> pmf(max_len + 1);
    std::vector<uint32_t> cdf(max_len + 2);
    for (int i = 0; i < n_scales; ++i) {
        const int c = centers[i], len = 2 * c + 1;
        const float s = scale_table[i];
        float lower0 = 0.f;
        for (int k = 0; k < len; ++k) {
            const float a = (float)std::abs(k - c);
            const float up = phi((0.5f - a) / s), lo = phi((-0.5f - a) / s);
            pmf[k] = up - lo;
            if (k == 0) lower0 = lo;
        }
        pmf[len] = 2.0f * lower0;
        const int rc = lvae_pmf_to_quantized_cdf(pmf.data(), len + 1, 16, cdf.data());
        if (rc) return rc;
        int32_t* row = qcdf + (size_t)i * row_stride;
        std::memset(row, 0, sizeof(int32_t) * row_stride);
        for (int k = 0; k < len + 2; ++k) row[k] = (int32_t)cdf[k];
        cdf_len[i] = len + 2;
        offset[i] = -c;
    }
    return max_len + 2;
}

namespace {
struct EncEnt { uint64_t rcp; uint32_t bias; uint16_t freq; uint8_t shift; uint8_t ready; };
struct EncRow {
    int32_t offset = 0, max_value = 0;
    EncEnt e[kMaxCdfLen - 1];
};
inline void enc_ent_init(EncEnt& s, uint32_t start, uint32_t freq) {
    s.freq = (uint16_t)freq;
    s.ready = 1;
    if (freq < 2) {
        s.rcp = ~0ull; s.shift = 0; s.bias = start + (1u << kPrecision) - 1;
    } else {
        uint32_t shift = 0;
        while (freq > (1u << shift)) ++shift;
        uint64_t x0 = freq - 1;
        const uint64_t x1 = 1ull << (shift + 31);
        const uint64_t t1 = x1 / freq;
        x0 += (x1 % freq) << 32;
        const uint64_t t0 = x0 / freq;
        s.rcp = t0 + (t1 << 32);
        s.shift = (uint8_t)(shift - 1);
        s.bias = start;
    }
}
inline void enc_put_ent(uint64_t& x, BackWriter& w, const EncEnt& s) {
    const uint64_t x_max = (uint64_t)s.freq << 47;
    if (x >= x_max) { w.put((uint32_t)x); x >>= 32; }
    const uint64_t q = (uint64_t)(((unsigned __int128)x * s.rcp) >> 64) >> s.shift;
    x = x + s.bias + q * (uint64_t)((1u << kPrecision) - s.freq);
}
struct EncTabs {
    std::unique_ptr<EncRow> rows[256];
    EncRow* row(int r, const int32_t* cdf_len, const int32_t* offset) {
        if (rows[r]) return rows[r].get();
        if (cdf_len[r] < kMinCdfLenEnc || cdf_len[r] > kMaxCdfLen) return nullptr;
        const int32_t mv = cdf_len[r] - 2;
        rows[r].reset(new (std::nothrow) EncRow);
        if (!rows[r]) return nullptr;
        rows[r]->offset = offset[r];
        rows[r]->max_value = mv;
        for (auto& e : rows[r]->e) e.ready = 0;
        return rows[r].get();
    }
};
}

extern "C" long lvae_rans_encode_with_indexes(const int32_t* sym, const uint8_t* idx, size_t n,
                                              const int32_t* qcdf, int row_stride, const int32_t* cdf_len,
                                              const int32_t* offset, uint8_t* out, size_t out_cap) {
    if (out_cap < 8) return -2;
    uint8_t* aligned = (uint8_t*)(((uintptr_t)out + 3) & ~(uintptr_t)3);
    const size_t cap_words = (out_cap - (size_t)(aligned - out)) / 4;
    BackWriter w{(uint32_t*)aligned, (uint32_t*)aligned + cap_words};
    uint64_t x = kRansL;
    std::unique_ptr<EncTabs> T(new (std::nothrow) EncTabs);
    if (!T) return -12;
    EncRow* cur = nullptr;
    int32_t cur_row = -1;
    for (size_t ii = n; ii-- > 0;) {
        const int32_t row_i = idx[ii];
        if (row_i != cur_row) {
            cur = T->row(row_i, cdf_len, offset);
            if (!cur) return -4;
            cur_row = row_i;
        }
        const int32_t max_value = cur->max_value;
        const int32_t value = sym[ii] - cur->offset;
        const bool in_range = value >= 0 && value < max_value;
        EncEnt& e = cur->e[in_range ? value : max_value];
        if (__builtin_expect(!e.ready, 0)) {
            const int32_t* cdf = qcdf + (size_t)row_i * row_stride;
            const int32_t v = in_range ? value : max_value;
            enc_ent_init(e, (uint32_t)cdf[v], (uint32_t)(cdf[v + 1] - cdf[v]));
        }
        if (__builtin_expect(in_range, 1)) {
            enc_put_ent(x, w, e);
            continue;
        }
        uint32_t raw;
        if (value < 0) raw = (uint32_t)(-2 * (int64_t)value - 1);
        else           raw = (uint32_t)(2 * ((int64_t)value - max_value));
        int32_t n_bypass = 0;
        while (n_bypass < 8 && (raw >> (n_bypass * kBypassPrecision)) != 0) ++n_bypass;
        for (int32_t j = n_bypass - 1; j >= 0; --j) enc_put_bits(x, w, (raw >> (j * kBypassPrecision)) & kMaxBypassVal);
        const int32_t n15 = n_bypass / kMaxBypassVal, rem = n_bypass % kMaxBypassVal;
        enc_put_bits(x, w, (uint32_t)rem);
        for (int32_t j = 0; j < n15; ++j) enc_put_bits(x, w, (uint32_t)kMaxBypassVal);
        enc_put_ent(x, w, e);
    }
    w.put((uint32_t)(x >> 32));
    w.put((uint32_t)x);
    if (w.overflow) return -2;
    const size_t nbytes = (size_t)(((uint32_t*)aligned + cap_words) - w.ptr) * 4;
    std::memmove(out, w.ptr, nbytes);
    return (long)nbytes;
}

extern "C" int lvae_rans_enc_step_selftest(uint64_t x, uint32_t start, uint32_t freq, uint64_t* by_division, uint64_t* by_reciprocal) {
    if (freq < 1 || freq > 65535 || !by_division || !by_reciprocal) return -22;
    uint32_t sink[4];
    BackWriter w1{sink, sink + 4}, w2{sink, sink + 4};
    uint64_t a = x, b = x;
    enc_put(a, w1, start, freq);
    EncEnt e;
    enc_ent_init(e, start, freq);
    enc_put_ent(b, w2, e);
    *by_division = a; *by_reciprocal = b;
    return (w1.ptr == w2.ptr) ? 0 : 1;
}

struct RowTab { uint16_t freq[256]; uint16_t start[256]; uint8_t lut[256]; };
struct RowInfo { uint32_t mfreq, mstart; int32_t msym, max_value; uint32_t mpeak; };
struct LvaeDecTabs {
    RowTab tabs[256];
    RowInfo info[256];
    std::atomic<uint8_t> state[256];
    LvaeDecTabs() { for (auto& st : state) st.store(0, std::memory_order_relaxed); }
};

namespace {
inline void spin_pause() {
#if defined(__x86_64__) || defined(__i386__)
    __builtin_ia32_pause();
#endif
}
constexpr uint32_t kMpsPeak = 52429;
inline bool ensure_row(LvaeDecTabs& D, int row, const int32_t* cdf, int32_t size) {
    uint8_t st = D.state[row].load(std::memory_order_acquire);
    if (st == 2) return true;
    for (;;) {
        if (st == 3) return false;
        if (st == 0 && D.state[row].compare_exchange_strong(st, 1, std::memory_order_acq_rel)) break;
        if (st == 2) return true;
        spin_pause();
        st = D.state[row].load(std::memory_order_acquire);
    }
    if (size < kMinCdfLenDec || size > kMaxCdfLen) { D.state[row].store(3, std::memory_order_release); return false; }
    RowTab& T = D.tabs[row];
    int32_t sidx = 0;
    for (int b = 0; b < 256; ++b) {
        const uint32_t v = (uint32_t)b << 8;
        while (sidx + 1 < size - 1 && (uint32_t)cdf[sidx + 1] <= v) ++sidx;
        T.lut[b] = (uint8_t)sidx;
        const uint32_t f = (uint32_t)(cdf[sidx + 1] - cdf[sidx]);
        const bool pure = (uint32_t)cdf[sidx + 1] >= v + 256 && f <= 0xFFFFu;
        T.freq[b] = pure ? (uint16_t)f : (uint16_t)0;
        T.start[b] = pure ? (uint16_t)cdf[sidx] : (uint16_t)0;
    }
    RowInfo& R = D.info[row];
    R.max_value = size - 2;
    R.mfreq = 0; R.mstart = 0; R.msym = 0;
    for (int32_t s = 0; s < size - 2; ++s) {
        const uint32_t f = (uint32_t)(cdf[s + 1] - cdf[s]);
        if (cdf[s] >= 0 && cdf[s + 1] <= 65536 && cdf[s + 1] > cdf[s] && f > R.mfreq) { R.mfreq = f; R.mstart = (uint32_t)cdf[s]; R.msym = s; }
    }
    R.mpeak = R.mfreq >= kMpsPeak ? R.mfreq : 0;
    D.state[row].store(2, std::memory_order_release);
    return true;
}

constexpr size_t kMpsWindow = 1024;
constexpr uint32_t kMpsMaxMiss = 200;
constexpr int kMpsCoolWindows = 8;
constexpr int kMpsCoolMax = 512;

int decode_stream(const uint8_t* in, size_t in_len, const uint8_t* idx, size_t n, const int32_t* qcdf, int row_stride,
                  const int32_t* cdf_len, const int32_t* offset, int32_t* sym_out, LvaeDecTabs& D) {
    if (in_len < 8 || (in_len & 3)) return -1;
    std::vector<uint32_t> tmp;
    const uint32_t* words;
    if (((uintptr_t)in & 3) == 0) words = (const uint32_t*)in;
    else { tmp.resize(in_len / 4); std::memcpy(tmp.data(), in, in_len); words = tmp.data(); }
    const uint32_t* ptr = words;
    const uint32_t* end = words + in_len / 4;
    uint64_t x = (uint64_t)ptr[0] | ((uint64_t)ptr[1] << 32);
    ptr += 2;
    bool overrun = false;
    bool mine[256] = {false};
    bool use_mps = true;
    uint32_t miss = 0;
    int cool = 0, cool_len = kMpsCoolWindows;
    size_t next_look = kMpsWindow;
    for (size_t i = 0; i < n; ++i) {
        const int32_t row_i = idx[i];
        if (!mine[row_i]) {
            if (!ensure_row(D, row_i, qcdf + (size_t)row_i * row_stride, cdf_len[row_i])) return -4;
            mine[row_i] = true;
        }
        if (i == next_look) {
            if (use_mps) {
                if (miss > kMpsMaxMiss) { use_mps = false; cool = cool_len; cool_len = cool_len * 2 < kMpsCoolMax ? cool_len * 2 : kMpsCoolMax; }
                else cool_len = kMpsCoolWindows;
            } else if (--cool <= 0) use_mps = true;
            miss = 0;
            next_look += kMpsWindow;
        }
        const RowInfo& R = D.info[row_i];
        const uint32_t cf = (uint32_t)(x & 0xFFFF);
        const uint32_t dm = cf - R.mstart;
        if (__builtin_expect(dm < (use_mps ? R.mfreq : R.mpeak), 1)) {
            x = (uint64_t)R.mfreq * (x >> kPrecision) + dm;
            if (x < kRansL) {
                uint32_t wv = 0;
                if (ptr < end) wv = *ptr; else overrun = true;
                ++ptr;
                x = (x << 32) | wv;
                if (overrun) return -3;
            }
            sym_out[i] = R.msym + offset[row_i];
            continue;
        }
        ++miss;
        const int32_t* cdf = qcdf + (size_t)row_i * row_stride;
        const RowTab& T = D.tabs[row_i];
        uint32_t freq = T.freq[cf >> 8], start = T.start[cf >> 8];
        int32_t s = T.lut[cf >> 8];
        if (__builtin_expect(freq == 0, 0)) {
            while ((uint32_t)cdf[s + 1] <= cf) ++s;
            start = (uint32_t)cdf[s]; freq = (uint32_t)(cdf[s + 1] - cdf[s]);
        }
        x = (uint64_t)freq * (x >> kPrecision) + cf - start;
        if (x < kRansL) {
            uint32_t wv = 0;
            if (ptr < end) wv = *ptr; else overrun = true;
            ++ptr;
            x = (x << 32) | wv;
        }
        int32_t value = s;
        if (value == R.max_value) {
            int32_t val = (int32_t)dec_get_bits(x, ptr, end, overrun);
            int32_t n_bypass = val;
            while (val == kMaxBypassVal) {
                val = (int32_t)dec_get_bits(x, ptr, end, overrun);
                n_bypass += val;
                if (overrun) return -3;
            }
            uint32_t raw = 0;
            for (int32_t j = 0; j < n_bypass; ++j) {
                val = (int32_t)dec_get_bits(x, ptr, end, overrun);
                if (j < 8) raw |= (uint32_t)val << (j * kBypassPrecision);
            }
            value = (int32_t)(raw >> 1);
            if (raw & 1) value = -value - 1;
            else value += R.max_value;
        }
        sym_out[i] = value + offset[row_i];
        if (overrun) return -3;
    }
    return 0;
}
}

extern "C" int lvae_rans_decode_with_indexes(const uint8_t* in, size_t in_len, const uint8_t* idx, size_t n,
                                             const int32_t* qcdf, int row_stride, const int32_t* cdf_len,
                                             const int32_t* offset, int32_t* sym_out) {
    std::unique_ptr<LvaeDecTabs> D(new (std::nothrow) LvaeDecTabs);
    if (!D) return -12;
    try { return decode_stream(in, in_len, idx, n, qcdf, row_stride, cdf_len, offset, sym_out, *D); } catch (...) { return -12; }
}

namespace {
inline void cpu_relax() {
#if defined(__x86_64__) || defined(__i386__)
    __builtin_ia32_pause();
#elif defined(__aarch64__)
    asm volatile("yield" ::: "memory");
#else
    std::this_thread::yield();
#endif
}

struct Job {
    int n = 0, max_workers = 0;
    std::atomic<int> next{0}, done{0}, workers{0};
    void (*run)(void*, int) = nullptr;
    void* ctx = nullptr;
    std::mutex m;
    std::condition_variable cv;
};

class Pool {
public:
    static Pool& get() { static Pool* p = new Pool;  return *p; }
    void submit(const std::shared_ptr<Job>& j) {
        { std::lock_guard<std::mutex> l(m_); q_.push_back(j); }
        epoch_.fetch_add(1, std::memory_order_release);
        const int need = j->max_workers < (int)th_.size() ? j->max_workers : (int)th_.size();
        for (int i = 0; i < need; ++i) cv_.notify_one();
    }
    int size() const { return (int)th_.size(); }
private:
    Pool() {
        int n = (int)std::thread::hardware_concurrency();
        if (n < 2) n = 2;
        if (n > 64) n = 64;
        for (int i = 0; i < n; ++i) th_.emplace_back([this, i] { loop(i < kSpinners); });
        for (auto& t : th_) t.detach();
    }
    static constexpr int kSpinners = 8;
    void loop(bool spinner) {
        for (;;) {
            std::shared_ptr<Job> j;
            if (spinner) {
                const unsigned seen = epoch_.load(std::memory_order_acquire);
                for (int it = 0; it < 20000 && epoch_.load(std::memory_order_acquire) == seen; ++it) cpu_relax();
            }
            {
                std::unique_lock<std::mutex> l(m_);
                cv_.wait(l, [this] { return !q_.empty(); });
                while (!q_.empty()) {
                    const std::shared_ptr<Job>& f = q_.front();
                    if (f->next.load() >= f->n || f->workers.load() >= f->max_workers) { q_.pop_front(); continue; }
                    j = f;
                    j->workers.fetch_add(1);
                    break;
                }
            }
            if (j) work(*j);
        }
    }
public:
    static void work(Job& j) {
        int did = 0;
        for (int i; (i = j.next.fetch_add(1)) < j.n;) { j.run(j.ctx, i); ++did; }
        if (did && j.done.fetch_add(did) + did == j.n) { std::lock_guard<std::mutex> l(j.m); j.cv.notify_all(); }
    }
private:
    std::mutex m_;
    std::condition_variable cv_;
    std::atomic<unsigned> epoch_{0};
    std::deque<std::shared_ptr<Job>> q_;
    std::vector<std::thread> th_;
};

template <class F>
void parallel_for(int n, int n_threads, F&& f) {
    if (n_threads <= 0) n_threads = (int)std::thread::hardware_concurrency();
    if (n_threads < 1) n_threads = 1;
    if (n_threads > n) n_threads = n;
    if (n_threads <= 1) { for (int i = 0; i < n; ++i) f(i); return; }
    auto j = std::make_shared<Job>();
    j->n = n;
    j->max_workers = n_threads - 1;
    j->ctx = (void*)&f;
    j->run = [](void* c, int i) { (*(typename std::remove_reference<F>::type*)c)(i); };
    Pool::get().submit(j);
    Pool::work(*j);
    for (int it = 0; it < 20000 && j->done.load(std::memory_order_acquire) < n; ++it) cpu_relax();
    std::unique_lock<std::mutex> l(j->m);
    j->cv.wait(l, [&] { return j->done.load() >= n; });
}
}

extern "C" int lvae_rans_encode_batch(int n_streams, const int32_t* const* sym, const uint8_t* const* idx,
                                      const size_t* n, const int32_t* qcdf, int row_stride, const int32_t* cdf_len,
                                      const int32_t* offset, uint8_t* const* out, const size_t* out_cap,
                                      long* out_len, int n_threads) {
    if (n_streams < 0) return -22;
    try {
        parallel_for(n_streams, n_threads, [&](int s) {
            out_len[s] = lvae_rans_encode_with_indexes(sym[s], idx[s], n[s], qcdf, row_stride, cdf_len, offset, out[s],
                                                       out_cap[s]);
        });
    } catch (...) { return -12; }
    int rc = 0;
    for (int s = 0; s < n_streams; ++s) if (out_len[s] < 0) rc = (int)out_len[s];
    return rc;
}

struct LvaeEncJob {
    std::vector<const int32_t*> sym;
    std::vector<const uint8_t*> idx;
    std::vector<size_t> n, out_cap;
    std::vector<uint8_t*> out;
    long* out_len = nullptr;
    const int32_t *qcdf = nullptr, *cdf_len = nullptr, *offset = nullptr;
    int row_stride = 0;
    std::shared_ptr<Job> job;
    void run(int s) {
        out_len[s] = lvae_rans_encode_with_indexes(sym[s], idx[s], n[s], qcdf, row_stride, cdf_len, offset, out[s], out_cap[s]);
    }
};
LvaeEncJob* lvae_rans_encode_batch_begin(int n_streams, const int32_t* const* sym, const uint8_t* const* idx, const size_t* n,
                                         const int32_t* qcdf, int row_stride, const int32_t* cdf_len, const int32_t* offset,
                                         uint8_t* const* out, const size_t* out_cap, long* out_len, int n_threads) {
    if (n_streams < 0) return nullptr;
    LvaeEncJob* e = new (std::nothrow) LvaeEncJob;
    if (!e) return nullptr;
    try {
    e->sym.assign(sym, sym + n_streams); e->idx.assign(idx, idx + n_streams); e->n.assign(n, n + n_streams);
    e->out.assign(out, out + n_streams); e->out_cap.assign(out_cap, out_cap + n_streams);
    e->out_len = out_len; e->qcdf = qcdf; e->cdf_len = cdf_len; e->offset = offset; e->row_stride = row_stride;
    for (int s = 0; s < n_streams; ++s) out_len[s] = 0;
    if (n_threads <= 0) n_threads = (int)std::thread::hardware_concurrency();
    if (n_threads <= 1) {
        for (int s = 0; s < n_streams; ++s) e->run(s);
    } else if (n_streams > 0) {
        auto j = std::make_shared<Job>();
        j->n = n_streams;
        j->max_workers = n_threads < n_streams ? n_threads : n_streams;
        j->ctx = (void*)e;
        j->run = [](void* c, int i) { ((LvaeEncJob*)c)->run(i); };
        e->job = j;
        Pool::get().submit(j);
    }
    } catch (...) {
        delete e;
        return nullptr;
    }
    return e;
}
int lvae_rans_encode_batch_end(LvaeEncJob* e) {
    if (!e) return -12;
    const int n = (int)e->sym.size();
    if (e->job) {
        Job& j = *e->job;
        Pool::work(j);
        for (int it = 0; it < 20000 && j.done.load(std::memory_order_acquire) < n; ++it) cpu_relax();
        std::unique_lock<std::mutex> l(j.m);
        j.cv.wait(l, [&] { return j.done.load() >= n; });
    }
    int rc = 0;
    for (int s = 0; s < n; ++s) if (e->out_len[s] < 0) rc = (int)e->out_len[s];
    delete e;
    return rc;
}

LvaeDecTabs* lvae_dec_tabs_new() { return new (std::nothrow) LvaeDecTabs; }
void lvae_dec_tabs_free(LvaeDecTabs* t) { delete t; }
int lvae_rans_decode_batch_tabs(int n_streams, const uint8_t* const* in, const size_t* in_len, const uint8_t* const* idx,
                                const size_t* n, const int32_t* qcdf, int row_stride, const int32_t* cdf_len, const int32_t* offset,
                                int32_t* const* sym_out, int* status, int n_threads, LvaeDecTabs* tabs) {
    if (n_streams < 0 || !tabs) return -22;
    try {
        parallel_for(n_streams, n_threads, [&](int s) {
            int rc = -12;
            try { rc = decode_stream(in[s], in_len[s], idx[s], n[s], qcdf, row_stride, cdf_len, offset, sym_out[s], *tabs); } catch (...) {}
            status[s] = rc;
        });
    } catch (...) { return -12; }
    int rc = 0;
    for (int s = 0; s < n_streams; ++s) if (status[s] < 0) rc = status[s];
    return rc;
}

extern "C" int lvae_rans_decode_batch(int n_streams, const uint8_t* const* in, const size_t* in_len,
                                      const uint8_t* const* idx, const size_t* n, const int32_t* qcdf,
                                      int row_stride, const int32_t* cdf_len, const int32_t* offset,
                                      int32_t* const* sym_out, int* status, int n_threads) {
    if (n_streams < 0) return -22;
    std::unique_ptr<LvaeDecTabs> D(new (std::nothrow) LvaeDecTabs);
    if (!D) return -12;
    return lvae_rans_decode_batch_tabs(n_streams, in, in_len, idx, n, qcdf, row_stride, cdf_len, offset, sym_out, status, n_threads, D.get());
}
```

### lossy-vae_amd/lvae/_native/__init__.py

```python
import ctypes as C
import os

_HERE = os.path.dirname(os.path.abspath(__file__))
LIB_PATH = os.path.join(_HERE, 'liblvae_hip.so')
ABI_VERSION = 27
_lib = None


class GemmDesc(C.Structure):
    _fields_ = [
        ('A0', C.c_void_p), ('A1', C.c_void_p),
        ('lda0', C.c_long), ('lda1', C.c_long),
        ('K0', C.c_int), ('K1', C.c_int),
        ('H', C.c_int), ('W', C.c_int),
        ('Wt', C.c_void_p), ('ldw', C.c_long),
        ('bias', C.c_void_p), ('gamma', C.c_void_p),
        ('res', C.c_void_p), ('ldres', C.c_long),
        ('out', C.c_void_p), ('ldo', C.c_long),
        ('M', C.c_int), ('N', C.c_int), ('K', C.c_int),
        ('a_mode', C.c_int), ('epi', C.c_int), ('store', C.c_int), ('r', C.c_int),
        ('a_gelu', C.c_int), ('prec', C.c_int), ('Wt16', C.c_void_p), ('cfg', C.c_int), ('ksplit', C.c_int), ('ws', C.c_void_p), ('a_bf16', C.c_int), ('out_bf16', C.c_int), ('cnt', C.c_void_p),
        ('status', C.c_void_p), ('a_h2', C.c_int), ('out_h2', C.c_int), ('defer_reduce', C.c_int),
    ]


class Op(C.Structure):
    _fields_ = [('kind', C.c_int), ('side', C.c_int), ('p', C.c_void_p * 8), ('i', C.c_long * 6), ('f', C.c_double * 2)]


class MlpDesc(C.Structure):
    _fields_ = [('y', C.c_void_p), ('w1', C.c_void_p), ('b1', C.c_void_p), ('w2', C.c_void_p), ('b2', C.c_void_p), ('gamma', C.c_void_p),
                ('res', C.c_void_p), ('out', C.c_void_p), ('M', C.c_int), ('C', C.c_int), ('hid', C.c_int)]


class MlpSkDesc(C.Structure):
    _fields_ = [('y', C.c_void_p), ('w1', C.c_void_p), ('b1', C.c_void_p), ('w2', C.c_void_p), ('b2', C.c_void_p), ('gamma', C.c_void_p),
                ('res', C.c_void_p), ('out', C.c_void_p), ('ws', C.c_void_p), ('M', C.c_int), ('C', C.c_int), ('hid', C.c_int),
                ('S1', C.c_int), ('S2', C.c_int)]


class DecBlock(C.Structure):
    _fields_ = [('ops', C.c_void_p), ('n_ops', C.c_int), ('idx_dev', C.c_void_p), ('idx_host', C.c_void_p), ('sym_host', C.c_void_p),
                ('sym_dev', C.c_void_p), ('per_image', C.c_size_t)]


class EncBlock(C.Structure):
    _fields_ = [('ops', C.c_void_p), ('n_ops', C.c_int), ('sym_dev', C.c_void_p), ('sym_host', C.c_void_p), ('idx_dev', C.c_void_p),
                ('idx_host', C.c_void_p), ('per_image', C.c_size_t)]


OP_KINDS = {name: k + 1 for k, name in enumerate([
    'lvae_gemm_f32', 'lvae_dwconv_ln_f32', 'lvae_dwconv_ln_h2', 'lvae_dwconv_ln_bf16', 'lvae_dwconv_ln_q8', 'lvae_stem_f32', 'lvae_stem_bf16',
    'lvae_bias_expand_f32', 'lvae_bias_expand_bf16', 'lvae_prior_index_f32', 'lvae_quantize_f32', 'lvae_dequantize_f32',
    'lvae_gaussian_nll_f32', 'lvae_lossless_params_f32', 'lvae_lossless_output_f32', 'lvae_mlp_h2f', 'lvae_mlp_sk', 'lvae_prior_index_sk_f32', 'lvae_quantize_sk_f32',
    'lvae_gaussian_nll_chan_f32', 'lvae_rd_image_f32', 'lvae_pixel_nll_f32',
    'lvae_dwconv_ln_f32_v', 'lvae_dwconv_ln_h2_v', 'lvae_dwconv_ln_bf16_v', 'lvae_dwconv_ln_q8_v'])}
OP_ORDER = len(OP_KINDS) + 1

TRACE_MAGIC = 1985229328.0
A_PLAIN, A_PATCH2, A_CONV3 = 0, 1, 2
STATUS_RANGE, STATUS_NONFINITE_PRIOR, STATUS_NONFINITE_LATENT, STATUS_NONFINITE_IMAGE = 1, 2, 4, 8
EPI_BIAS, EPI_BIAS_GELU, EPI_GAMMA_RES, EPI_RES = 0, 1, 2, 3
ST_ROWMAJOR, ST_SHUFFLE, ST_IMAGE = 0, 2, 3
YUV_FORMATS, YUV_MATRICES, YUV_RANGES, YUV_CHROMA = ('i420', 'nv12'), ('bt601', 'bt709'), ('limited', 'full'), ('nearest', 'bilinear')
YUV_SUBSAMPLINGS, YUV_SITINGS, YUV_MATRICES2 = ('420', '422', '444'), ('center', 'left'), ('bt601', 'bt709', 'bt2020')
YUV_DEPTHS = (8, 10, 12)
YUV_LAYOUTS = ('planar', 'semiplanar')
SAMPLE_KINDS = ('f32', 'u8', 'u16_low', 'u16_high')
EVAL_CHUNKS = 256

_vp, _i, _l, _f, _d, _sz = C.c_void_p, C.c_int, C.c_long, C.c_float, C.c_double, C.c_size_t
SIGNATURES = {
    'lvae_abi_version': (_i, []),
    'lvae_build_info': (C.c_char_p, []),
    'lvae_pmf_to_quantized_cdf': (_i, [_vp, _i, _i, _vp]),
    'lvae_build_gaussian_tables': (_i, [_vp, _i, _d, _i, _vp, _i, _vp, _vp]),
    'lvae_rans_encode_with_indexes': (_l, [_vp, _vp, _sz, _vp, _i, _vp, _vp, _vp, _sz]),
    'lvae_rans_decode_with_indexes': (_i, [_vp, _sz, _vp, _sz, _vp, _i, _vp, _vp, _vp]),
    'lvae_rans_enc_step_selftest': (_i, [C.c_uint64, C.c_uint32, C.c_uint32, _vp, _vp]),
    'lvae_rans_encode_batch': (_i, [_i, _vp, _vp, _vp, _vp, _i, _vp, _vp, _vp, _vp, _vp, _i]),
    'lvae_rans_decode_batch': (_i, [_i, _vp, _vp, _vp, _vp, _vp, _i, _vp, _vp, _vp, _vp, _i]),
    'lvae_gemm_f32': (_i, [C.POINTER(GemmDesc), _vp]),
    'lvae_gemm_num_configs': (_i, []),
    'lvae_gemm_h2_choice': (_i, [C.POINTER(GemmDesc), _i, _vp, _vp, _vp]),
    'lvae_mlp_h2f': (_i, [C.POINTER(MlpDesc), _vp]),
    'lvae_mlp_sk': (_i, [C.POINTER(MlpSkDesc), _vp]),
    'lvae_mlp_sk_supported': (_i, [_i, _i, _i, _i]),
    'lvae_gelu_f32': (_i, [_vp, _vp, _l, _vp]),
    'lvae_dwconv_ln_f32': (_i, [_vp] * 8 + [_i] * 5 + [_vp]),
    'lvae_dwconv_ln_h2': (_i, [_vp] * 8 + [_i] * 5 + [_vp]),
    'lvae_dwconv_ln_q8': (_i, [_vp] * 8 + [_i] * 5 + [_vp]),
    'lvae_stem_f32': (_i, [_vp, _vp, _vp, _vp, _i, _i, _i, _i, _f, _f, _vp, _vp]),
    'lvae_range_flag_f32': (_i, [_vp, _l, _f, _f, _vp, _vp]),
    'lvae_dwconv_ln_bf16': (_i, [_vp] * 8 + [_i] * 5 + [_vp]),
    'lvae_dwconv_ln_f32_v': (_i, [_vp] * 6 + [_i] * 5 + [_l, _vp]),
    'lvae_dwconv_ln_h2_v': (_i, [_vp] * 6 + [_i] * 5 + [_l, _vp]),
    'lvae_dwconv_ln_bf16_v': (_i, [_vp] * 6 + [_i] * 5 + [_l, _vp]),
    'lvae_dwconv_ln_q8_v': (_i, [_vp] * 6 + [_i] * 5 + [_l, _vp]),
    'lvae_dwconv_ln_choice': (_i, [_i] * 8 + [_vp] * 3),
    'lvae_stem_bf16': (_i, [_vp, _vp, _vp, _vp, _i, _i, _i, _i, _f, _f, _vp, _vp]),
    'lvae_bias_expand_bf16': (_i, [_vp, _vp, _l, _i, _vp]),
    'lvae_gemv_f32': (_i, [_vp, _vp, _vp, _vp, _i, _i, _i, _i, _vp]),
    'lvae_gemv_batch_f32': (_i, [_vp, _vp, _vp, _vp, _i, _i, _i, _i, _i, _vp]),
    'lvae_prior_index_f32': (_i, [_vp, _vp, _vp, _vp, _i, _f, _i, _i, _i, _vp, _vp]),
    'lvae_prior_index_sk_f32': (_i, [_vp, _i, _vp, _vp, _vp, _vp, _vp, _i, _f, _i, _i, _i, _vp, _vp]),
    'lvae_quantize_sk_f32': (_i, [_vp, _i, _vp, _vp, _vp, _vp, _vp, _i, _i, _i, _i, _vp, _vp]),
    'lvae_quantize_f32': (_i, [_vp, _vp, _vp, _vp, _i, _i, _i, _i, _vp, _vp]),
    'lvae_dequantize_f32': (_i, [_vp, _vp, _vp, _i, _i, _i, _i, _vp]),
    'lvae_lossless_params_f32': (_i, [_vp, _vp, _vp, _vp, _vp, _vp, _i, _f, _i, _i, _i, _vp, _vp]),
    'lvae_lossless_output_f32': (_i, [_vp, _vp, _vp, C.c_long, _vp, _vp]),
    'lvae_prior_sample_f32': (_i, [_vp, _vp, C.c_long, _i, _i, C.c_float, C.c_ulonglong, C.c_ulonglong, _vp]),
    'lvae_gaussian_nll_f32': (_i, [_vp, _vp, _vp, _f, _i, _i, _i, _i, _vp]),
    'lvae_latent_sample_box_f32': (_i, [_vp, _vp, _vp] + [_i] * 9 + [C.c_float, C.c_ulonglong, C.c_ulonglong, _vp]),
    'lvae_pixel_sample_f32': (_i, [_vp, _vp, _i, _i, _i, C.c_float, C.c_ulonglong, C.c_ulonglong, _vp, _vp]),
    'lvae_gaussian_nll_map_f32': (_i, [_vp, _vp, _vp, _f, _i, _i, _i, _i, _vp]),
    'lvae_gaussian_nll_chan_f32': (_i, [_vp, _vp, _vp, _f, _i, _i, _i, _i, _vp]),
    'lvae_rd_image_f32': (_i, [_vp, _vp, _vp, _vp, _vp, _i, _i, _i, _vp, _vp]),
    'lvae_pixel_nll_f32': (_i, [_vp, _vp, _vp, _vp, _vp, _i, _i, _i, _vp, _vp]),
    'lvae_bias_expand_f32': (_i, [_vp, _vp, _l, _i, _vp]),
    'lvae_event_create': (_vp, []),
    'lvae_event_destroy': (_i, [_vp]),
    'lvae_stream_order': (_i, [_vp, _vp, _vp]),
    'lvae_run_ops': (_i, [_vp, _i, _vp, _vp, _vp]),
    'lvae_decode_blocks': (_i, [_vp, _i, _i, _vp, _vp, _vp, _i, _vp, _vp, _vp, _i, _vp, _vp, _vp, _vp, _i, _vp, _vp, _vp]),
    'lvae_encode_blocks': (_i, [_vp, _i, _i, _vp, _vp, _vp, _vp, _i, _vp, _vp, _vp, _vp, _vp, _vp, _i, _vp, _vp, _vp]),
    'lvae_sqerr_sum_f32': (_i, [_vp, _vp, _vp, _i, _l, _vp]),
    'lvae_sqerr_partials_f32': (_i, [_vp, _vp, _vp, _i, _l, _vp]),
    'lvae_msssim_f32': (_i, [_vp, _l, _l, _l, _vp, _l, _l, _l, _vp, _i, _i, _i, _i, _vp, _vp, _vp, _sz, _vp]),
    'lvae_msssim_workspace_bytes': (_sz, [_i, _i, _i, _i]),
    'lvae_msssim_planes': (_i, [_vp] * 6 + [_i, _i, _i, _d, _i, _vp, _vp, _vp, _sz, _vp]),
    'lvae_msssim_planes_workspace_bytes': (_sz, [_i, _i, _i, _i]),
    'lvae_image_u8_to_f32': (_i, [_vp, _vp, _vp, _i, _vp, _l, _i, _i, _vp]),
    'lvae_image_f32_to_u8': (_i, [_vp, _l, _l, _l, _i, _i, _vp, _i, _vp, _vp, _vp]),
    'lvae_image_yuv420_to_f32': (_i, [_vp] * 7 + [_i] * 5 + [_vp, _l, _i, _i, _vp]),
    'lvae_image_f32_to_yuv420': (_i, [_vp, _l, _l, _l, _i, _i, _vp] + [_i] * 4 + [_vp] * 7),
    'lvae_sse_u8': (_i, [_vp] * 5 + [_i, _vp, _vp]),
    'lvae_image_yuv_to_f32': (_i, [_vp] * 7 + [_i] * 7 + [_vp, _l, _i, _i, _vp]),
    'lvae_image_f32_to_yuv': (_i, [_vp, _l, _l, _l, _i, _i, _vp] + [_i] * 6 + [_vp] * 7),
    'lvae_image_yuvsp_to_f32': (_i, [_vp] * 5 + [_i] * 7 + [_vp, _l, _i, _i, _vp]),
    'lvae_image_f32_to_yuvsp': (_i, [_vp, _l, _l, _l, _i, _i, _vp] + [_i] * 6 + [_vp] * 5),
    'lvae_sse_u16': (_i, [_vp] * 5 + [_i, _vp, _vp]),
    'lvae_tile_stitch': (_i, [_vp, _l, _l, _vp, _vp] + [_i] * 11 + [_vp, _l, _l, _i, _vp, _sz, _vp]),
    'lvae_tile_stitch_workspace_bytes': (_sz, [_i, _i]),
    'lvae_tile_stitch_yuv': (_i, [_vp, _l, _l, _vp, _vp] + [_i] * 17 + [_vp, _vp, _vp, _l, _l, _l, _vp, _sz, _vp]),
    'lvae_resample_u8_to_f32': (_i, [_vp, _vp] + [_i] * 5 + [_vp, _vp, _i, _i, _vp, _vp, _i] + [_vp, _l, _i, _i, _vp]),
    'lvae_resample_f32_to_u8': (_i, [_vp, _l, _l, _l] + [_i] * 5 + [_vp, _vp, _i, _i, _vp, _vp, _i] + [_vp, _vp, _vp]),
    'lvae_resample_f32': (_i, [_vp, _l, _l, _l] + [_i] * 5 + [_vp, _vp, _i, _i, _vp, _vp, _i] + [_i, _vp, _l, _i, _i, _vp]),
    'lvae_resample_yuv_to_f32': (_i, [_vp] * 7 + [_i] * 8 + [_i] * 4 + [_vp, _vp, _i, _i, _vp, _vp, _i, _i] + [_vp, _l, _i, _i, _vp]),
    'lvae_resample_f32_to_yuv': (_i, [_vp, _l, _l, _l, _vp] + [_i] * 7 + [_i] * 4 + [_vp, _vp, _i, _i, _vp, _vp, _i] + [_vp] * 7),
    'lvae_gaussian_nll_pos_f32': (_i, [_vp, _vp, _vp, _f, _i, _i, _i, _i, _vp]),
    'lvae_pixel_nll_pos_f32': (_i, [_vp, _vp, _vp, _i, _i, _i, _vp, _vp]),
    'lvae_rate_map_f32': (_i, [_vp, _vp, _vp, _i, _vp, _i, _i, _i, _vp, _l, _l, _i, _i, _vp]),
}


def lib():
    global _lib
    if _lib is None:
        if not os.path.exists(LIB_PATH):
            raise RuntimeError(
                f'{LIB_PATH} not found: the HIP extension is the product path and there is no fallback. '
                f'Build it with `python lossy-vae_amd/build_native.py` (hipcc --offload-arch=gfx950).')
        L = C.CDLL(LIB_PATH)
        for name, (res, args) in SIGNATURES.items():
            fn = getattr(L, name)
            fn.restype, fn.argtypes = res, args
            fn.lvae_name = name
        v = L.lvae_abi_version()
        if v != ABI_VERSION:
            raise RuntimeError(f'liblvae_hip.so ABI {v} != expected {ABI_VERSION}; rebuild')
        _lib = L
    return _lib


def check(rc, what):
    if rc != 0:
        raise RuntimeError(f'{what} failed with code {rc} (hipError_t if > 0, argument error if < 0)')
```

### lossy-vae_amd/lvae/models/base.py

```python
import ctypes
import functools
import logging
import math
import os
import threading
import time

import numpy as np
import torch
import torch.nn as nn

from .. import _native
from ..engine import NonFiniteError, Plan
from .entropy_coding import rans_decode_streams

_W16_LOCK = threading.Lock()


def split_bf16x3(t):
    hi = t.to(torch.bfloat16)
    r1 = t - hi.float()
    mid = r1.to(torch.bfloat16)
    lo = (r1 - mid.float()).to(torch.bfloat16)
    return torch.stack([hi, mid, lo], 0).contiguous()


def pack_bf16x3(t):
    planes = split_bf16x3(t)
    n, k = t.shape
    if k % 32:
        return planes.reshape(-1)
    inter = planes.view(3, n, k // 16, 16).permute(1, 2, 0, 3).contiguous()
    return torch.cat([planes.reshape(-1), inter.reshape(-1)])


def split_f16x2(t):
    hi = t.to(torch.float16)
    lo = ((t - hi.float()) * 2048.0).to(torch.float16)
    return torch.stack([hi, lo], 0).contiguous()


def pack_f16x2(t):
    n, k = t.shape
    if k % 16 or not bool(torch.isfinite(t).all()) or float(t.abs().max()) >= 65504.0:
        return None
    planes = split_f16x2(t.float())
    return planes.view(2, n, k // 16, 16).permute(1, 2, 0, 3).contiguous().reshape(-1)


def pack_f16x2_k32(t):
    n, k = t.shape
    if k % 32 or not bool(torch.isfinite(t).all()) or float(t.abs().max()) >= 65504.0:
        return None
    planes = split_f16x2(t.float())
    return planes.view(2, n, k // 32, 32).permute(1, 2, 0, 3).contiguous().reshape(-1)


def unpack_f16x2_k32(buf, n, k):
    v = buf.view(torch.float16).reshape(n, k // 32, 2, 32)
    return v[:, :, 0, :].reshape(n, k), v[:, :, 1, :].reshape(n, k)


def pack_mxfp8(t):
    n, k = t.shape
    kp = (k + 63) // 64 * 64
    w = torch.zeros(n, kp, dtype=torch.float32, device=t.device)
    w[:, :k] = t.float()
    blk = w.view(n, kp // 32, 32)
    amax = blk.abs().amax(dim=2)
    bits = amax.view(torch.int32)
    eb = ((bits >> 23) & 0xff) - 8
    eb = eb + ((bits & 0x7fffff) > 0x600000).to(torch.int32)
    eb = eb.clamp(1, 254)
    inv = ((254 - eb) << 23).view(torch.float32)
    q = (blk * inv.unsqueeze(2)).to(torch.float8_e4m3fn).view(torch.uint8).reshape(n, kp)
    return torch.cat([q.reshape(-1), eb.to(torch.uint8).reshape(-1)]).contiguous()


def pack_mxfp8_q8(t):
    n, k = t.shape
    assert k % 64 == 0
    buf = pack_mxfp8(t)
    data, sc = buf[:n * k], buf[n * k:].view(n, k // 64, 2)
    return torch.cat([data, sc.permute(1, 0, 2).contiguous().reshape(-1)]).contiguous()


def unpack_mxfp8_q8(buf, n, k):
    buf = buf.view(torch.uint8).reshape(-1)
    data, sc = buf[:n * k], buf[n * k:n * k + n * k // 32].view(k // 64, n, 2).permute(1, 0, 2).contiguous().reshape(-1)
    return unpack_mxfp8(torch.cat([data, sc]), n, k)


def unpack_mxfp8(buf, n, k):
    kp = (k + 63) // 64 * 64
    q = buf[:n * kp].view(torch.float8_e4m3fn).float().view(n, kp // 32, 32)
    eb = buf[n * kp:].to(torch.int32).view(n, kp // 32)
    scale = torch.pow(2.0, (eb - 127).double()).float()
    return (q * scale.unsqueeze(2)).view(n, kp)[:, :k].contiguous()


class LazyW16:

    def __init__(self, tensors, mode):
        self.by_ptr = {t.data_ptr(): t for t in tensors.values()
                       if t.dim() == 2 and t.dtype == torch.float32 and t.shape[1] % 8 == 0}
        self.mode, self.map, self.keep = mode, {}, []

    def get(self, ptr):
        h = self.map.get(ptr)
        if h is not None:
            return h
        t = self.by_ptr.get(ptr)
        if t is None:
            return None
        with _W16_LOCK:
            h = self.map.get(ptr)
            if h is None:
                c = (pack_bf16x3(t) if self.mode == 'bf16x3' else pack_mxfp8(t) if self.mode == 'fp8'
                     else pack_f16x2(t) if self.mode == 'f16x2' else pack_f16x2_k32(t) if self.mode == 'f16x2k32'
                     else (pack_mxfp8_q8(t) if t.shape[1] % 64 == 0 else None) if self.mode == 'mxfp8q8'
                     else t.to(torch.bfloat16).contiguous())
                if c is None:
                    self.map[ptr] = 0
                    return None
                self.keep.append(c)
                h = self.map[ptr] = c.data_ptr()
        return h or None


DEFAULT_PRECISION = 'f16x2'
PRECISIONS = ('fp32', 'bf16', 'bf16x3', 'f16x2', 'fp8')
PREC_CODE = {'fp32': 0, 'bf16': 1, 'bf16x3': 2, 'fp8': 3, 'f16x2': 4}
assert DEFAULT_PRECISION in PRECISIONS, DEFAULT_PRECISION
_log = logging.getLogger('lvae')


class PackedWeights:

    def __init__(self, model, device):
        self.t, self.device, self._w16 = {}, device, {}
        dg = model._dg()
        self.scale_table = dg.scale_table.detach().to(device=device, dtype=torch.float32).contiguous()
        self.scale_bound = float(dg.lower_bound_scale.bound.item())

    def put(self, name, t):
        self.t[name] = t.detach().to(device=self.device, dtype=torch.float32).contiguous()

    def p(self, name):
        return self.t[name].data_ptr()

    def bf16_map(self, mode):
        with _W16_LOCK:
            if mode not in self._w16:
                self._w16[mode] = LazyW16(self.t, mode)
        return self._w16[mode]


class CodecPlan(Plan):
    lp_storage = False
    use_mlp_sk = False

    def __init__(self, model, pk, B):
        super().__init__(pk.device)
        self.model, self.pk, self.B = model, pk, B
        if model._prec == 'fp8' and not self.lp_storage:
            raise NotImplementedError("the 'fp8' mode (bf16 activation storage + MX-fp8 GEMMs, BASELINE config 5) is built for qarv_base")
        self.prec = PREC_CODE[model._prec]
        self.prec_name = model._prec
        self.w16 = pk.bf16_map(model._prec) if self.prec else None
        self.w16_x3 = pk.bf16_map('bf16x3') if self.prec == 4 else None
        self.w16_k32 = pk.bf16_map('f16x2k32') if self.prec == 4 else None
        self.w16_q8 = pk.bf16_map('mxfp8q8') if self.prec == 3 else None
        self.lp = self.prec == 3
        self.adt = torch.bfloat16 if self.lp else torch.float32
        self.lat_shapes, self.lat_hw = [], []
        self.idx_off, self.sym_off = [], []
        self.cuts, self.qcuts = [], []
        self.pm_bufs = []
        self.prm_bufs, self.qm_bufs, self.zhat_bufs, self.zhat_ld = [], [], [], []

    def alloc_symbols(self, n_sym, host=True):
        self.n_sym = n_sym
        self.sym_all, self.idx_all = self.new(n_sym, torch.int32), self.new(n_sym, torch.uint8)
        if host:
            self.sym_host = torch.empty(n_sym, dtype=torch.int32).pin_memory()
            self.idx_host = torch.empty(n_sym, dtype=torch.uint8).pin_memory()
            self.sym_np, self.idx_np = self.sym_host.numpy(), self.idx_host.numpy()

    def alloc_pos(self):
        self.pos_bufs = [self.new(self.B * hw, torch.float64) for _, hw in self.lat_shapes]

    def dwln_add(self, fmt, p, x, y, H, W, C, k):
        raise NotImplementedError

    def cnx(self, p, m, x, out, H, W):
        pk = self.pk
        C, k, hid = m.dim, m.kernel_size, m.hidden
        M = self.B * H * W
        y = self.buf(self.sname('y'), M * C, self.adt).data_ptr()
        mlp = dict(y=y, M=M, C=C, hid=hid, w1=pk.p(p + '.fc1_w'), b1=pk.p(p + '.fc1_b'), w2=pk.p(p + '.fc2_w'), b2=pk.p(p + '.fc2_b'),
                   gamma=pk.p(p + '.gamma'), res=x, out=out, label=p + '.mlp')
        if self.mlp_fused_ok(C, hid, k, M=M, rows_per_image=H * W):
            self.dwln_add('h2', p, x, y, H, W, C, k)
            self.mlp_fused(**mlp)
            return
        sk = self.mlp_sk_ok(C, hid, k, H * W, M) if self.use_mlp_sk else None
        if sk is not None:
            self.dwln_add('h2', p, x, y, H, W, C, k)
            self.mlp_sk(S1=sk[0], S2=sk[1], **mlp)
            return
        h = self.buf(self.sname('hid'), M * hid, self.adt).data_ptr()
        if self.mlp_q8_ok(C, hid, k):
            pre1, pre2, S1, S2 = True, True, None, None
        else:
            pre1, pre2, S1, S2 = self.mlp_pipeline(C, hid, k, H * W)
        fmt = ('q8' if pre1 else 'bf16') if self.lp else ('h2' if pre1 else 'f32')
        self.dwln_add(fmt, p, x, y, H, W, C, k)
        self.gemm(A0=y, K0=C, M=M, N=hid, Wt=pk.p(p + '.fc1_w'), bias=pk.p(p + '.fc1_b'), out=h,
                  epi=_native.EPI_BIAS_GELU, a_h2=pre1, out_h2=pre2, ksplit=S1, label=p + '.fc1')
        self.gemm(A0=h, K0=hid, M=M, N=C, Wt=pk.p(p + '.fc2_w'), bias=pk.p(p + '.fc2_b'),
                  gamma=pk.p(p + '.gamma'), res=x, ldres=C, out=out, epi=_native.EPI_GAMMA_RES, a_h2=pre2, ksplit=S2, label=p + '.fc2')


def on_model_device(fn):
    @functools.wraps(fn)
    def wrapper(self, *a, **k):
        dev = self._dummy.device
        if dev.type == 'cuda' and torch.cuda.current_device() != dev.index:
            with torch.cuda.device(dev):
                return fn(self, *a, **k)
        return fn(self, *a, **k)
    return wrapper


class CodecBase(nn.Module):
    def _init_codec_base(self):
        self.coder_threads = 0
        self.pipeline_groups = int(os.environ.get('LVAE_GROUPS', '2'))
        self.enc_groups = int(os.environ.get('LVAE_ENC_GROUPS', '0'))
        self.dec_groups = int(os.environ.get('LVAE_DEC_GROUPS', '0'))
        self._streams = []
        self._pool = None
        self.serial_groups = False
        self._prec = DEFAULT_PRECISION
        self._packed, self._plans = None, {}

    def _invalidate(self):
        self._packed, self._plans = None, {}

    def _apply(self, fn, *a, **k):
        self._invalidate()
        return super()._apply(fn, *a, **k)

    def load_state_dict(self, *a, **k):
        self._invalidate()
        return super().load_state_dict(*a, **k)

    def _prepare(self):
        dev = self._dummy.device
        if self._packed is None or self._packed.device != dev:
            if dev.type != 'cuda':
                raise RuntimeError('lvae (MI355X build): compress/decompress run on the GPU only; move the model with '
                                   '.to("cuda") -- there is deliberately no CPU fallback')
            _native.lib()
            self._invalidate()
            with torch.no_grad():
                self._packed = self._build_packed(dev)
        return self._packed

    def _plan(self, kind, *a, **k):
        key = self._plan_key(kind, *a, **k)
        pl = self._plans.get(key)
        if pl is None:
            self._prepare()
            pl = self._plans[key] = self._build_plan(kind, *a, **k)
        return pl

    def _dg(self):
        for b in self._latent_blocks():
            return b.discrete_gaussian
        raise RuntimeError('no latent block')

    def _build_cdf_tables(self, build):
        first, *rest = dgs = [b.discrete_gaussian for b in self._latent_blocks()]
        build(first)
        for dg in rest:
            dg._quantized_cdf, dg._offset, dg._cdf_length, dg._host = first._quantized_cdf, first._offset, first._cdf_length, None
        return dgs

    def set_gemm_precision(self, mode):
        assert mode in PRECISIONS
        self._prec = mode
        self._prec_logged = None

    def _log_precision(self):
        if getattr(self, '_prec_logged', None) != self._prec:
            self._prec_logged = self._prec
            _log.warning("lvae: %s codes with GEMM arithmetic %r%s; a bitstream decodes only under the arithmetic that wrote it "
                         "(streams of builds that defaulted to 'bf16x3' need model.set_gemm_precision('bf16x3') on this side too)",
                         type(self).__name__, self._prec, ' (package default)' if self._prec == DEFAULT_PRECISION else ' (set explicitly)')

    native_group_loops = True


    @staticmethod
    def _alias_host(pl, seg, n_ops):
        raster_ops = {_native.OP_KINDS[k] for k in ('lvae_prior_index_f32', 'lvae_prior_index_sk_f32', 'lvae_quantize_f32', 'lvae_quantize_sk_f32', 'lvae_dequantize_f32')}
        spans = [(pl.sym_all.data_ptr(), pl.sym_all.numel() * 4, pl.sym_host.data_ptr()), (pl.idx_all.data_ptr(), pl.idx_all.numel(), pl.idx_host.data_ptr())]
        out = (_native.Op * max(1, n_ops))()
        ctypes.memmove(out, seg, ctypes.sizeof(_native.Op) * n_ops)
        for o in out[:n_ops]:
            if o.kind not in raster_ops:
                continue
            for j in range(len(o.p)):
                a = o.p[j]
                if a:
                    for lo_, size, host in spans:
                        if lo_ <= a < lo_ + size:
                            o.p[j] = host + (a - lo_)
        return out

    @classmethod
    def _group_blocks(cls_, pl, kind, cuts, offs, n):
        key = '_native_blocks_' + kind
        cached = getattr(pl, key, None)
        if cached is None:
            cls = _native.DecBlock if kind == 'dec' else _native.EncBlock
            arr = (cls * len(cuts))()
            segs, lo = [], 0
            for li, cut in enumerate(cuts):
                seg, n_ops = pl._segment(lo, cut)
                seg = cls_._alias_host(pl, seg, n_ops)
                segs.append(seg)
                z, hw = pl.lat_shapes[li]
                o = offs[li]
                b = arr[li]
                b.ops, b.n_ops, b.per_image = ctypes.cast(seg, ctypes.c_void_p).value, n_ops, z * hw
                b.idx_dev, b.idx_host = None, pl.idx_host.data_ptr() + o
                b.sym_dev, b.sym_host = None, pl.sym_host.data_ptr() + 4 * o
                lo = cut
            tail, n_tail = pl._segment(lo, len(pl.ops)) if kind == 'dec' else (None, 0)
            if n_tail:
                tail = cls_._alias_host(pl, tail, n_tail)
            early = None
            if kind == 'dec' and len(cuts):
                early = (cls * len(cuts))()
                ctypes.memmove(early, arr, ctypes.sizeof(arr))
                early[0].n_ops = 0
            cached = (arr, segs, tail, n_tail, early)
            setattr(pl, key, cached)
        return cached

    def _decode_group_native(self, pl, cuts, offs, n, strings, tables, nthreads, stream, T=None):
        arr, segs, tail, n_tail, early = self._group_blocks(pl, 'dec', cuts, offs, n)
        nb = len(cuts)
        if early is not None:
            with torch.cuda.device(pl.device):
                pl._run_native(0, cuts[0], stream.cuda_stream, seg=(segs[0], arr[0].n_ops))
            arr = early
        if callable(strings):
            strings = strings()
        qcdf, cdf_len, offset = tables
        addr, size = [], []
        for li in range(nb):
            for b in range(n):
                s_ = strings[b][li]
                if isinstance(s_, tuple):
                    base, off, ln = s_
                    assert isinstance(base, bytes)
                    addr.append(ctypes.cast(ctypes.c_char_p(base), ctypes.c_void_p).value + off); size.append(ln)
                else:
                    addr.append(ctypes.cast(ctypes.c_char_p(s_), ctypes.c_void_p).value if len(s_) else None); size.append(len(s_))
        sp = (ctypes.c_void_p * len(addr))(*addr)
        sl = (ctypes.c_size_t * len(size))(*size)
        fb, fo = ctypes.c_int(-1), ctypes.c_int(-1)
        trace = getattr(self, 'dec_trace', None)
        secs = (ctypes.c_double * (64 if trace is not None else 2))()
        if trace is not None:
            secs[0], secs[1] = -64.0, _native.TRACE_MAGIC
        ss = pl.side_stream.cuda_stream if pl.side_stream is not None else None
        st_dev = pl.status_ptr()
        with torch.cuda.device(pl.device):
            rc = _native.lib().lvae_decode_blocks(arr, nb, n, sp, sl, qcdf.ctypes.data, qcdf.shape[1], cdf_len.ctypes.data, offset.ctypes.data,
                                                  ctypes.cast(tail, ctypes.c_void_p) if n_tail else None, n_tail, st_dev, pl.status_host.data_ptr(),
                                                  ctypes.c_void_p(stream.cuda_stream),
                                                  ctypes.c_void_p(ss) if ss is not None else None, int(nthreads), ctypes.byref(fb), ctypes.byref(fo), secs)
        if rc != 0:
            stream.synchronize()
            word = int(pl.status_host[0]) if rc == -75 else 0
            self._reset_status(pl)
            if rc == -75:
                raise NonFiniteError(word, getattr(pl, 'prec_name', None), f'while decoding (latent block {fb.value} of {nb})')
            if rc == -74:
                raise ValueError(f'rANS decode failed in latent block {fb.value} (corrupt or truncated bitstream)')
            raise RuntimeError(f'native decode failed: rc={rc} at latent block {fb.value}, launch {fo.value}')
        if trace is not None:
            trace.append((n, nb, list(secs)))
        if T is not None:
            T['dec_gpu_seg'] = T.get('dec_gpu_seg', 0) + secs[0]
            T['dec_rans'] = T.get('dec_rans', 0) + secs[1]

    def _encode_group_native(self, pl, cuts, offs, n, tables, nthreads, stream, T=None):
        arr, _segs, _tail, _nt, _early = self._group_blocks(pl, 'enc', cuts, offs, n)
        nb = len(cuts)
        qcdf, cdf_len, offset = tables
        caps = [8 * pl.lat_shapes[li][0] * pl.lat_shapes[li][1] + 64 for li in range(nb)]
        outs = getattr(pl, '_native_enc_out', None)
        if outs is None:
            outs = pl._native_enc_out = [np.empty(caps[li], dtype=np.uint8) for li in range(nb) for _ in range(n)]
        op = (ctypes.c_void_p * len(outs))(*[x.ctypes.data for x in outs])
        oc = (ctypes.c_size_t * len(outs))(*[caps[li] for li in range(nb) for _ in range(n)])
        out_len = (ctypes.c_long * len(outs))()
        fb, fo = ctypes.c_int(-1), ctypes.c_int(-1)
        secs = (ctypes.c_double * 3)()
        ss = pl.side_stream.cuda_stream if pl.side_stream is not None else None
        st_dev = pl.status_ptr()
        with torch.cuda.device(pl.device):
            rc = _native.lib().lvae_encode_blocks(arr, nb, n, op, oc, out_len, qcdf.ctypes.data, qcdf.shape[1], cdf_len.ctypes.data, offset.ctypes.data,
                                                  st_dev, pl.status_host.data_ptr(), ctypes.c_void_p(stream.cuda_stream),
                                                  ctypes.c_void_p(ss) if ss is not None else None, int(nthreads), ctypes.byref(fb), ctypes.byref(fo), secs)
        if rc in (-34, -75):
            word = int(pl.status_host[0])
            self._reset_status(pl)
            pl.raise_if_flagged(word, where='while encoding')
            raise RuntimeError(f'native encode reported rc={rc} without a status word')
        if rc != 0:
            self._reset_status(pl)
            raise RuntimeError(f'native encode failed: rc={rc} at latent block {fb.value}, launch {fo.value}')
        if T is not None:
            T['enc_launch'] = T.get('enc_launch', 0) + secs[0]
            T['enc_gpu_wait'] = T.get('enc_gpu_wait', 0) + secs[1]
            T['enc_rans'] = T.get('enc_rans', 0) + secs[2]
        return [[outs[li * n + b][:out_len[li * n + b]].tobytes() for b in range(n)] for li in range(nb)]

    def _decode_group_loop(self, pl, n, strings, tables, nthreads, stream, T=None):
        lo = 0
        for li, cut in enumerate(pl.cuts):
            t0 = time.time()
            pl.run(lo, cut, stream=stream.cuda_stream)
            lo = cut
            t1 = self._decode_block(pl, li, n, [s[li] for s in strings], tables, nthreads, stream)
            if T is not None:
                t2 = time.time()
                T['dec_gpu_seg'] = T.get('dec_gpu_seg', 0) + t1 - t0
                T['dec_rans'] = T.get('dec_rans', 0) + t2 - t1
        pl.run(lo, None, stream=stream.cuda_stream)
        pl.fetch_status()

    def _decode_block(self, pl, li, n, strings, tables, nthreads, stream):
        z, hw = pl.lat_shapes[li]
        o, cnt = pl.idx_off[li], n * z * hw
        pl.idx_host[o:o + cnt].copy_(pl.idx_all[o:o + cnt], non_blocking=True)
        stream.synchronize()
        t1 = time.time()
        iv = [pl.idx_np[o + b * z * hw:o + (b + 1) * z * hw] for b in range(n)]
        sv = [pl.sym_np[o + b * z * hw:o + (b + 1) * z * hw] for b in range(n)]
        rans_decode_streams(tables, strings, iv, sv, nthreads)
        pl.sym_all[o:o + cnt].copy_(pl.sym_host[o:o + cnt], non_blocking=True)
        return t1

    @staticmethod
    def _reset_status(pl):
        if getattr(pl, 'status', None) is not None:
            torch.cuda.synchronize(pl.device)
            pl.status.zero_()
            pl.status_host.zero_()
            torch.cuda.synchronize(pl.device)

    def _check_decoded(self, groups, plan_of):
        torch.cuda.current_stream(self._dummy.device).synchronize()
        err = None
        for g, (_start, n) in enumerate(groups):
            try:
                plan_of(g, n).raise_if_flagged(where='while decoding')
            except ArithmeticError as e:
                err = err or e
        if err is not None:
            raise err

    variable_rate = False

    def _pack_blob(self, body, size):
        raise NotImplementedError

    def _unpack_blob(self, blob):
        raise NotImplementedError

    @staticmethod
    def _load_input(dst, im, u8, start, n):
        if u8 is not None:
            u8.fill(dst, start, n)
        else:
            dst.copy_(im[start:start + n])

    @torch.no_grad()
    def compress_images(self, images, lmb=None):
        from ..utils.image import U8Batch
        return self._compress_byte_batch(U8Batch(images, self.max_stride, self._dummy.device), lmb, 'compress_images')

    def _compress_byte_batch(self, batch, lmb, who):
        _, _, H, W = batch.shape
        d = self.max_stride
        assert all((d * math.ceil(h / d), d * math.ceil(w / d)) == (H, W) for h, w in batch.sizes), f'{who}: padded sizes differ'
        if self.variable_rate:
            bodies = self.compress_batch(None, lmb=lmb, u8=batch)
        else:
            if lmb is not None:
                raise ValueError(f'{type(self).__name__} is a fixed-rate model: it takes no lmb')
            bodies = self.compress_batch(None, u8=batch)
        return [self._pack_blob(body, size) for body, size in zip(bodies, batch.sizes)]

    def _decompress_blobs(self, blobs, convert):
        parsed = [self._unpack_blob(b) for b in blobs]
        by_key = {}
        for i, (_, _, key) in enumerate(parsed):
            by_key.setdefault(key, []).append(i)
        out = [None] * len(blobs)
        for idxs in by_key.values():
            x = self.decompress_batch([parsed[i][0] for i in idxs])
            for i, item in zip(idxs, convert(x, [parsed[i][1] for i in idxs])):
                out[i] = item
        return out

    @torch.no_grad()
    def compress_yuv420(self, frames, lmb=None, matrix='bt709', range='limited', chroma='bilinear'):
        from ..utils.yuv import Yuv420Frame, _as_frames
        return self.compress_yuv(_as_frames(frames, Yuv420Frame), lmb, matrix, range, chroma)

    @torch.no_grad()
    def decompress_yuv420(self, blobs, fmt='i420', matrix='bt709', range='limited'):
        from ..utils.yuv import _check
        _check(matrix, range, fmt=fmt)
        return self.decompress_yuv(blobs, matrix=matrix, range=range, layout=fmt)

    @torch.no_grad()
    def compress_yuv(self, frames, lmb=None, matrix='bt709', range='limited', chroma='bilinear', siting='center'):
        from ..utils.yuv import FrameFormat
        frames, fmt = FrameFormat.shared(frames, 'compress_yuv')
        return self._compress_byte_batch(fmt.batch(frames, self.max_stride, self._dummy.device, matrix, range, chroma, siting), lmb, 'compress_yuv')

    @torch.no_grad()
    def decompress_yuv(self, blobs, depth=8, subsampling='420', siting='center', matrix='bt709', range='limited', layout='planar'):
        from ..utils.yuv import _check2, _extent_ok, check_layout, from_rgb01_any
        _check2(range=range)
        check_layout(layout, depth, subsampling, siting, matrix)
        for i, b in enumerate(blobs):
            h, w = self._unpack_blob(b)[1]
            if not _extent_ok(h, w, subsampling):
                raise ValueError(f'decompress_yuv: blob {i} holds a {h} x {w} image, which does not fit subsampling {subsampling}')
        conv = lambda x, sizes: from_rgb01_any(x, sizes, depth=depth, subsampling=subsampling, siting=siting, matrix=matrix, range=range,
                                               layout=layout)
        return self._decompress_blobs(blobs, conv)

    @property
    def _registry_name(self):
        return getattr(self, 'model_name', None) or type(self).__name__

    @torch.no_grad()
    def compress_yuv_sequence(self, frames_or_path, width=None, height=None, depth=8, subsampling='420', layout='planar', siting='center',
                              matrix='bt709', range='limited', chroma='bilinear', frames=None, lmb=None, max_batch=8, tile=None, overlap=0,
                              scale=None, size=None, filter='lanczos3'):
        from ..utils import resample, yuv, yuvseq
        scaled = scale is not None or size is not None
        if scaled:
            if tile is not None:
                raise ValueError('compress_yuv_sequence: scale / size and tile may not be combined (scaled and tiled coding are separate)')
            if scale is not None and size is not None:
                raise ValueError('compress_yuv_sequence: give one of scale and size, not both')
            resample._filter(filter)
        if lmb is not None and not self.variable_rate:
            raise ValueError(f'{type(self).__name__} is a fixed-rate model: it takes no lmb')
        if isinstance(frames_or_path, (str, os.PathLike)):
            if width is None or height is None:
                raise ValueError('compress_yuv_sequence: a raw file needs width and height')
            fmt = yuv.FrameFormat(layout, depth, subsampling, siting, matrix)
            path, limit = frames_or_path, None if frames is None else int(frames)
            per, nbytes = fmt.frame_bytes(width, height), os.path.getsize(path)
            if nbytes == 0 or nbytes % per:
                raise ValueError(f'compress_yuv_sequence: {path} holds {nbytes} bytes, not a whole number of {width}x{height} frames of {per} bytes')
            total = nbytes // per if limit is None else min(limit, nbytes // per)
            source = lambda start, n: fmt.read(path, width, height, frames=min(n, total - start), start=start) if start < total else []
        else:
            source, fmt = yuv.FrameFormat.shared(frames_or_path, 'compress_yuv_sequence')
            (height, width) = source[0].size
            if any(yuv.FrameFormat.of(f) != fmt or f.size != (height, width) for f in source):
                raise ValueError('compress_yuv_sequence: the frames of a sequence share one kind, one plane layout and one size')
            yuvseq.check_layout(*fmt, siting, matrix)
        compress = lambda chunk, **kw: self.compress_yuv(chunk, matrix=matrix, range=range, chroma=chroma, siting=siting, **kw)
        if scaled:
            resample.scaled_size(height, width, scale=scale, size=size)
            compress = lambda chunk, **kw: self.compress_yuv_scaled(chunk, scale=scale, size=size, filter=filter, matrix=matrix, range=range,
                                                                    chroma=chroma, siting=siting, **kw)
        if tile is not None:
            self._tile_args(tile, overlap)

            def compress(chunk, lmb=None):
                per = lmb if isinstance(lmb, list) else [lmb] * len(chunk)
                return [self.compress_yuv_tiled(f, tile=tile, overlap=overlap, lmb=v, max_batch=max_batch, matrix=matrix, range=range,
                                                chroma=chroma, siting=siting) for f, v in zip(chunk, per)]
        blobs = yuvseq.code_sequence(compress, source, max_batch, lmb)
        meta = dict(fmt._asdict(), width=width, height=height, siting=siting, matrix=matrix, range=range, chroma=chroma,
                    model=self._registry_name, gemm=self._prec)
        return yuvseq.pack_sequence(meta, blobs)

    def yuv_sequence_info(self, blob):
        from ..utils import resample, tiling, yuvseq
        info = yuvseq.yuv_sequence_info(blob)
        lmb_of = lambda fb: (self.tiled_info(fb)['lmb'] if tiling.is_tiled(fb) else self.scaled_info(fb)['lmb'] if resample.is_scaled(fb)
                             else self._blob_lmb(fb))
        info['lmb'] = [lmb_of(yuvseq.frame_blob(blob, info, k)) for k in range(info['frames'])] if self.variable_rate else None
        return info

    @torch.no_grad()
    def decompress_yuv_sequence(self, blob, frames=None, layout=None, out_path=None, max_batch=8):
        from ..utils import resample, tiling, yuv, yuvseq
        info = yuvseq.yuv_sequence_info(blob)
        if info['model'] != self._registry_name:
            raise ValueError(f"decompress_yuv_sequence: the sequence was written by model {info['model']!r}, this model is {self._registry_name!r}")
        if info['gemm'] != self._prec:
            raise ValueError(f"decompress_yuv_sequence: the sequence was written under GEMM precision {info['gemm']!r}, this model runs "
                             f"{self._prec!r}; call set_gemm_precision({info['gemm']!r}) first")
        how = {k: info[k] for k in ('depth', 'subsampling', 'siting', 'matrix', 'range')}
        how['layout'] = info['layout'] if layout is None else layout
        yuvseq.check_layout(**{k: v for k, v in how.items() if k != 'range'})
        decode = lambda bl: self.decompress_yuv(bl, **how)
        decode_tiled = lambda b: self.decompress_yuv_tiled(b, max_batch=max_batch, **how)
        idxs, step, out = yuvseq.frame_indexes(info, frames), max(1, int(max_batch)), []
        for o in range(0, len(idxs), step):
            entries = [yuvseq.frame_blob(blob, info, k) for k in idxs[o:o + step]]
            whole = [b for b in entries if not tiling.is_tiled(b) and not resample.is_scaled(b)]
            small = [b for b in entries if resample.is_scaled(b)]
            got, got_small = iter(decode(whole) if whole else []), iter(self.decompress_yuv_scaled(small, **how) if small else [])
            got = [decode_tiled(b) if tiling.is_tiled(b) else next(got_small) if resample.is_scaled(b) else next(got) for b in entries]
            for f in got:
                if f.size != (info['height'], info['width']):
                    raise ValueError(f"YUV sequence container: a frame holds {f.size[1]} x {f.size[0]} pixels, the header says {info['width']} x {info['height']}")
            if out_path is None:
                out += got
            else:
                yuv.write_frames(got, out_path, append=o > 0)
        return out if out_path is None else len(idxs)

    @torch.no_grad()
    def decompress_images(self, blobs):
        from ..utils.image import to_u8
        return self._decompress_blobs(blobs, to_u8)

    @torch.no_grad()
    def decompress_to_files(self, bits_paths, image_paths):
        from ..utils.image import save_u8
        blobs = []
        for p in bits_paths:
            with open(p, 'rb') as f:
                blobs.append(f.read())
        ims = self.decompress_images(blobs)
        host = [torch.empty(t.shape, dtype=torch.uint8, pin_memory=True).copy_(t, non_blocking=True) for t in ims]
        torch.cuda.current_stream(self._dummy.device).synchronize()
        for t, p in zip(host, image_paths):
            save_u8(t, p)

    def _compress_to_files(self, images, output_paths, lmb=None):
        for blob, out in zip(self.compress_images(images, lmb=lmb), output_paths):
            with open(out, 'wb') as f:
                f.write(blob)

    LOG2E = 1.4426950408889634

    @staticmethod
    def _run_with_pos(pl, cdf_form, upto=None):
        lib = pl.lib
        st = ctypes.c_void_p(torch.cuda.current_stream(pl.device).cuda_stream)
        lo = 0
        for li, cut in enumerate(pl.qcuts):
            pl.run(lo, cut)
            lo = cut
            z, hw = pl.lat_shapes[li]
            _native.check(lib.lvae_gaussian_nll_pos_f32(pl.prm_bufs[li].data_ptr(), pl.sym_all.data_ptr() + 4 * pl.sym_off[li],
                                                        pl.pos_bufs[li].data_ptr(), pl.pk.scale_bound, pl.B, hw, z, cdf_form, st),
                          'lvae_gaussian_nll_pos_f32')
        if upto is None or upto > lo:
            pl.run(lo, upto)

    def _rate_map_run(self, im, u8, B, H, W, lmb, return_rec):
        raise NotImplementedError

    @torch.no_grad()
    @on_model_device
    def rate_map(self, im, lmb=None, blocks=False, return_rec=False):
        if lmb is not None and not self.variable_rate:
            raise TypeError(f'{type(self).__name__} is a fixed-rate model: rate_map takes no lmb')
        u8 = None
        if isinstance(im, (list, tuple)):
            from ..utils.image import U8Batch
            u8 = U8Batch(im, self.max_stride, self._dummy.device)
            B, _, H, W = u8.shape
            d = self.max_stride
            assert all((d * math.ceil(h / d), d * math.ceil(w / d)) == (H, W) for h, w in u8.sizes), 'rate_map: padded sizes differ'
            im = None
        else:
            im = im.to(self._dummy.device)
            assert im.dim() == 4 and im.shape[1] == 3 and im.dtype == torch.float32 and not im.requires_grad, f'{im.shape=}'
            B, _, H, W = im.shape
        assert H % self.max_stride == 0 and W % self.max_stride == 0, f'{(B, 3, H, W)=}'
        pl, pix, im_hat = self._rate_map_run(im, u8, B, H, W, lmb, return_rec)
        n = len(pl.pos_bufs)
        lat_h = (ctypes.c_int * n)(*[h for h, _ in pl.lat_hw])
        lat_w = (ctypes.c_int * n)(*[w for _, w in pl.lat_hw])
        lib = _native.lib()
        st = ctypes.c_void_p(torch.cuda.current_stream(pl.device).cuda_stream)
        dev = pl.device

        def compose(out, b0, nb, row, ch, cw):
            pos = (ctypes.c_void_p * n)(*[t.data_ptr() + 8 * b0 * h * w for t, (h, w) in zip(pl.pos_bufs, pl.lat_hw)])
            _native.check(lib.lvae_rate_map_f32(pos, lat_h, lat_w, n, None if pix is None else pix.data_ptr() + 8 * b0 * H * W, nb, H, W,
                                                out.data_ptr(), ch * row, row, ch, cw, st), 'lvae_rate_map_f32')

        if u8 is None:
            out = torch.empty(B, 1, H, W, dtype=torch.float32, device=dev)
            compose(out, 0, B, W, H, W)
        else:
            out = [torch.empty(1, h, w, dtype=torch.float32, device=dev) for h, w in u8.sizes]
            for b, (h, w) in enumerate(u8.sizes):
                compose(out[b], b, 1, w, h, w)
# ... 423 lines not shown
```

Measured before the change: 174.9 Mpixels/s.

## Transfer quantized symbols as int8 over host link with int32 fallback

Adds int8 symbol paths for quantize, dequantize and rANS encode/decode, so latent symbols cross the host-device link as one byte instead of four. A 'wide' flag detects symbols that do not fit, and those blocks fall back to the int32 path. It also widens int8 to int32 on the host in background jobs and can optionally use a separate copy stream for the D2H transfers. This cuts PCIe traffic and host memory bandwidth per block, at the cost of more code paths and a re-run of a block whenever the fallback triggers.

```diff
diff --git a/include/lvae_hip.h b/include/lvae_hip.h
--- a/include/lvae_hip.h
+++ b/include/lvae_hip.h
@@ -33,6 +33,14 @@
                            const uint8_t* const* idx, const size_t* n,
                            const int32_t* qcdf, int row_stride, const int32_t* cdf_len, const int32_t* offset,
                            int32_t* const* sym_out, int* status, int n_threads);
+#define LVAE_RANS_SYMBOL_TOO_WIDE (-7)
+int lvae_rans_encode_batch8(int n_streams, const int8_t* const* sym, const uint8_t* const* idx, const size_t* n,
+                            const int32_t* qcdf, int row_stride, const int32_t* cdf_len, const int32_t* offset,
+                            uint8_t* const* out, const size_t* out_cap, long* out_len, int n_threads);
+int lvae_rans_decode_batch8(int n_streams, const uint8_t* const* in, const size_t* in_len,
+                            const uint8_t* const* idx, const size_t* n,
+                            const int32_t* qcdf, int row_stride, const int32_t* cdf_len, const int32_t* offset,
+                            int8_t* const* sym_out, int* status, int n_threads);
 
 enum {
     LVAE_STATUS_RANGE = 1, LVAE_STATUS_NONFINITE_PRIOR = 2, LVAE_STATUS_NONFINITE_LATENT = 4, LVAE_STATUS_NONFINITE_IMAGE = 8
@@ -129,6 +137,28 @@
                        const int* status_dev, int* status_host, void* stream, void* side_stream, int n_threads,
                        int* failed_block, int* failed_op, double* seconds);
 
+typedef struct {
+    const lvae_op* ops; int n_ops;
+    uint8_t* idx_host;
+    int8_t* sym8_host; int32_t* sym_host;
+    size_t per_image;
+} lvae_dec_block8;
+int lvae_decode_blocks8(const lvae_dec_block8* blocks, int n_blocks, int n_images, const uint8_t* const* strings, const size_t* string_len,
+                        const int32_t* qcdf, int row_stride, const int32_t* cdf_len, const int32_t* offset,
+                        const lvae_op* tail_ops, int n_tail, const int* status_dev, int* status_host, void* stream, void* side_stream,
+                        int n_threads, int* failed_block, int* failed_op, double* seconds, int* wide_blocks);
+typedef struct {
+    const lvae_op* ops; int n_ops;
+    int8_t* sym8_dev; int8_t* sym8_host; int32_t* sym_host;
+    const uint8_t* idx_dev; uint8_t* idx_host;
+    int* wide;
+    size_t per_image;
+} lvae_enc_block8;
+int lvae_encode_blocks8(const lvae_enc_block8* blocks, int n_blocks, int n_images, uint8_t* const* out, const size_t* out_cap, long* out_len,
+                        const int32_t* qcdf, int row_stride, const int32_t* cdf_len, const int32_t* offset,
+                        const int* status_dev, int* status_host, void* stream, void* side_stream, void* copy_stream, int n_threads,
+                        int* failed_block, int* failed_op, double* seconds, int* wide_blocks);
+
 int lvae_dwconv_ln_f32(const float* x, const float* wt, const float* bias, const float* ln_w, const float* ln_b,
                        const float* shift, const float* scale1p, float* y,
                        int B, int H, int W, int C, int k, void* stream);
@@ -182,6 +212,12 @@
 int lvae_quantize_sk_f32(const float* ws, int S, const float* bias, float* qm, const float* pm, int32_t* sym, float* zhat, int B, int HW,
                          int z, int ldz, int* status, void* stream);
 int lvae_dequantize_f32(const int32_t* sym, const float* pm, float* zhat, int B, int HW, int z, int ldz, void* stream);
+
+int lvae_quantize8_f32(const float* qm, const float* pm, int8_t* sym, float* zhat, int B, int HW, int z, int ldz,
+                       int* status, int* wide, void* stream);
+int lvae_quantize8_sk_f32(const float* ws, int S, const float* bias, float* qm, const float* pm, int8_t* sym, float* zhat, int B, int HW,
+                          int z, int ldz, int* status, int* wide, void* stream);
+int lvae_dequantize8_f32(const int8_t* sym, const float* pm, float* zhat, int B, int HW, int z, int ldz, void* stream);
 
 int lvae_prior_sample_f32(const float* prm, float* z, long M, int zdim, int ldz, float t, unsigned long long seed,
                           unsigned long long offset, void* stream);
diff --git a/lossy-vae_amd/csrc/plan_runtime.cpp b/lossy-vae_amd/csrc/plan_runtime.cpp
--- a/lossy-vae_amd/csrc/plan_runtime.cpp
+++ b/lossy-vae_amd/csrc/plan_runtime.cpp
@@ -35,6 +35,16 @@
                                          const int32_t* qcdf, int row_stride, const int32_t* cdf_len, const int32_t* offset,
                                          uint8_t* const* out, const size_t* out_cap, long* out_len, int n_threads);
 int lvae_rans_encode_batch_end(LvaeEncJob* e);
+
+int lvae_rans_decode_batch_tabs8(int n_streams, const uint8_t* const* in, const size_t* in_len, const uint8_t* const* idx,
+                                 const size_t* n, const int32_t* qcdf, int row_stride, const int32_t* cdf_len, const int32_t* offset,
+                                 int8_t* const* sym_out, int* status, int n_threads, LvaeDecTabs* tabs);
+LvaeEncJob* lvae_rans_encode_batch_begin8(int n_streams, const int8_t* const* sym, int32_t* const* mirror, const uint8_t* const* idx, const size_t* n,
+                                          const int32_t* qcdf, int row_stride, const int32_t* cdf_len, const int32_t* offset,
+                                          uint8_t* const* out, const size_t* out_cap, long* out_len, int n_threads);
+struct LvaeWidenJob;
+LvaeWidenJob* lvae_widen_begin(int n_streams, const int8_t* const* src, int32_t* const* dst, const size_t* n);
+void lvae_widen_end(LvaeWidenJob* e);
 
 namespace {
 inline double now_s() { return std::chrono::duration<double>(std::chrono::steady_clock::now().time_since_epoch()).count(); }
@@ -179,6 +189,243 @@
     return 0;
 }
 
+namespace {
+int launch_dequantize(const lvae_op& o, const int8_t* sym8, void* stream, void* side_stream) {
+    if (o.kind != LVAE_OP_DEQUANTIZE) return -22;
+    void* st = o.side ? side_stream : stream;
+    if (!sym8) return lvae_plan::op_table[o.kind - 1].run(o, st);
+    return lvae_dequantize8_f32(sym8, (const float*)o.p[1], (float*)o.p[2], (int)o.i[0], (int)o.i[1], (int)o.i[2], (int)o.i[3], st);
+}
+int launch_quantize8(const lvae_op& o, int8_t* sym8, int* wide, void* stream, void* side_stream) {
+    void* st = o.side ? side_stream : stream;
+    if (o.kind == LVAE_OP_QUANTIZE)
+        return lvae_quantize8_f32((const float*)o.p[0], (const float*)o.p[1], sym8, (float*)o.p[3], (int)o.i[0], (int)o.i[1], (int)o.i[2], (int)o.i[3],
+                                  (int*)o.p[4], wide, st);
+    if (o.kind == LVAE_OP_QUANTIZE_SK)
+        return lvae_quantize8_sk_f32((const float*)o.p[0], (int)o.i[0], (const float*)o.p[1], (float*)o.p[2], (const float*)o.p[3], sym8, (float*)o.p[5],
+                                     (int)o.i[1], (int)o.i[2], (int)o.i[3], (int)o.i[4], (int*)o.p[6], wide, st);
+    return -22;
+}
+struct WidenJobs {
+    std::vector<LvaeWidenJob*> jobs;
+    ~WidenJobs() { for (LvaeWidenJob* j : jobs) lvae_widen_end(j); }
+};
+}
+
+static int decode_blocks8_impl(const lvae_dec_block8* blocks, int n_blocks, int n_images, const uint8_t* const* strings,
+                               const size_t* string_len, const int32_t* qcdf, int row_stride, const int32_t* cdf_len,
+                               const int32_t* offset, const lvae_op* tail_ops, int n_tail, const int* status_dev, int* status_host,
+                               void* stream, void* side_stream, int n_threads, int* failed_block, int* failed_op, double* seconds, int* wide_blocks) {
+    if (!blocks || n_blocks < 0 || n_blocks > 32 || n_images <= 0 || !strings || !string_len || !qcdf || !cdf_len || !offset) return -22;
+    hipStream_t st = (hipStream_t)stream;
+    std::vector<const uint8_t*> idx_ptr(n_images);
+    std::vector<int32_t*> out_ptr(n_images);
+    std::vector<int8_t*> out8_ptr(n_images);
+    std::vector<size_t> cnt(n_images);
+    std::vector<int> status(n_images);
+    struct TabsGuard { LvaeDecTabs* t; ~TabsGuard() { lvae_dec_tabs_free(t); } } tabs{lvae_dec_tabs_new()};
+    if (!tabs.t) return -12;
+    WidenJobs widen;
+    widen.jobs.reserve(n_blocks);
+    double t_gpu = 0.0, t_coder = 0.0;
+    int bad = -1, wide = 0;
+    bool prev_wide = false;
+    const int trace_cap = (seconds && seconds[0] <= -8.0 && seconds[0] >= -4096.0 && seconds[1] == LVAE_TRACE_MAGIC) ? (int)(-seconds[0]) : 0;
+    auto stamp = [&](int slot, double t) { if (slot < trace_cap) seconds[slot] = t; };
+    auto run_segment = [&](const lvae_op* ops, int n, int b) {
+        int first = 0, rc = 0;
+        if (b > 0 && n > 0) {
+            rc = launch_dequantize(ops[0], prev_wide ? nullptr : blocks[b - 1].sym8_host, stream, side_stream);
+            bad = 0;
+            first = 1;
+        }
+        if (rc == 0) {
+            rc = lvae_run_ops(ops + first, n - first, stream, side_stream, &bad);
+            if (rc != 0) bad += first;
+        }
+        return rc;
+    };
+    for (int b = 0; b < n_blocks; ++b) {
+        const lvae_dec_block8& k = blocks[b];
+        if (!k.idx_host || !k.sym8_host || !k.sym_host) return -22;
+        const double t0 = now_s();
+        int rc = run_segment(k.ops, k.n_ops, b);
+        const double t_issued = now_s();
+        if (rc == 0) {
+            hipError_t q = hipErrorNotReady;
+            for (int it = 0; it < 400000 && (q = hipStreamQuery(st)) == hipErrorNotReady; ++it) {}
+            rc = q == hipErrorNotReady ? (int)hipStreamSynchronize(st) : (int)q;
+        }
+        if (rc != 0) {
+            if (failed_block) *failed_block = b;
+            if (failed_op) *failed_op = bad;
+            return rc;
+        }
+        const double t1 = now_s();
+        for (int i = 0; i < n_images; ++i) {
+            idx_ptr[i] = k.idx_host + (size_t)i * k.per_image;
+            out_ptr[i] = k.sym_host + (size_t)i * k.per_image;
+            out8_ptr[i] = k.sym8_host + (size_t)i * k.per_image;
+            cnt[i] = k.per_image;
+        }
+        const uint8_t* const* in = strings + (size_t)b * n_images;
+        const size_t* in_len = string_len + (size_t)b * n_images;
+        rc = lvae_rans_decode_batch_tabs8(n_images, in, in_len, idx_ptr.data(), cnt.data(), qcdf, row_stride, cdf_len, offset, out8_ptr.data(),
+                                          status.data(), n_threads, tabs.t);
+        prev_wide = rc == LVAE_RANS_SYMBOL_TOO_WIDE;
+        if (prev_wide) {
+            wide |= 1 << b;
+            rc = lvae_rans_decode_batch_tabs(n_images, in, in_len, idx_ptr.data(), cnt.data(), qcdf, row_stride, cdf_len, offset, out_ptr.data(),
+                                             status.data(), n_threads, tabs.t);
+        }
+        if (rc != 0) {
+            if (failed_block) *failed_block = b;
+            if (status_dev && status_host && hipMemcpyAsync(status_host, status_dev, sizeof(int), hipMemcpyDeviceToHost, st) == hipSuccess &&
+                hipStreamSynchronize(st) == hipSuccess && *status_host != 0)
+                return -75;
+            return -74;
+        }
+        if (!prev_wide) {
+            LvaeWidenJob* j = lvae_widen_begin(n_images, out8_ptr.data(), out_ptr.data(), cnt.data());
+            if (j) widen.jobs.push_back(j);
+            else for (int i = 0; i < n_images; ++i) for (size_t e = 0; e < cnt[i]; ++e) out_ptr[i][e] = out8_ptr[i][e];
+        }
+        const double t2 = now_s();
+        t_gpu += t1 - t0; t_coder += t2 - t1;
+        stamp(2 + 4 * b, t0); stamp(3 + 4 * b, t_issued); stamp(4 + 4 * b, t1); stamp(5 + 4 * b, t2);
+    }
+    if (n_tail > 0) {
+        int rc = run_segment(tail_ops, n_tail, n_blocks);
+        if (rc == 0 && status_dev && status_host) rc = (int)hipMemcpyAsync(status_host, status_dev, sizeof(int), hipMemcpyDeviceToHost, st);
+        if (rc != 0) {
+            if (failed_block) *failed_block = n_blocks;
+            if (failed_op) *failed_op = bad;
+            return rc;
+        }
+    }
+    stamp(2 + 4 * n_blocks, now_s());
+    if (wide_blocks) *wide_blocks = wide;
+    if (seconds) { seconds[0] = t_gpu; seconds[1] = t_coder; }
+    return 0;
+}
+
+static int encode_blocks8_impl(const lvae_enc_block8* blocks, int n_blocks, int n_images, uint8_t* const* out, const size_t* out_cap,
+                               long* out_len, const int32_t* qcdf, int row_stride, const int32_t* cdf_len, const int32_t* offset,
+                               const int* status_dev, int* status_host, void* stream, void* side_stream, void* copy_stream, int n_threads,
+                               int* failed_block, int* failed_op, double* seconds, int* wide_blocks) {
+    if (!blocks || n_blocks <= 0 || n_blocks > 32 || n_images <= 0 || !out || !out_cap || !out_len || !qcdf || !cdf_len || !offset) return -22;
+    for (int b = 0; b < n_blocks; ++b) {
+        const lvae_enc_block8& k = blocks[b];
+        if (!k.ops || k.n_ops < 1 || !k.sym8_host || !k.sym_host || !k.idx_host || !k.wide || ((k.sym8_dev || k.idx_dev) && !copy_stream)) return -22;
+        const int kind = k.ops[k.n_ops - 1].kind;
+        if (kind != LVAE_OP_QUANTIZE && kind != LVAE_OP_QUANTIZE_SK) return -22;
+    }
+    hipStream_t st = (hipStream_t)stream, cs = (hipStream_t)copy_stream;
+    std::vector<hipEvent_t> evq(n_blocks, nullptr), ev(n_blocks, nullptr);
+    auto cleanup = [&]() { for (hipEvent_t e : evq) if (e) (void)hipEventDestroy(e); for (hipEvent_t e : ev) if (e) (void)hipEventDestroy(e); };
+    auto drain = [&]() { (void)hipStreamSynchronize(st); if (cs) (void)hipStreamSynchronize(cs); };
+    const double t0 = now_s();
+    int bad = -1;
+    for (int b = 0; b < n_blocks; ++b) *blocks[b].wide = 0;
+    for (int b = 0; b < n_blocks; ++b) {
+        const lvae_enc_block8& k = blocks[b];
+        const size_t cnt = k.per_image * n_images;
+        int rc = lvae_run_ops(k.ops, k.n_ops - 1, stream, side_stream, &bad);
+        if (rc == 0) { bad = k.n_ops - 1; rc = launch_quantize8(k.ops[k.n_ops - 1], k.sym8_dev ? k.sym8_dev : k.sym8_host, k.wide, stream, side_stream); }
+        hipStream_t es = st;
+        if (k.sym8_dev || k.idx_dev) {
+            es = cs;
+            if (rc == 0) rc = (int)hipEventCreateWithFlags(&evq[b], hipEventDisableTiming);
+            if (rc == 0) rc = (int)hipEventRecord(evq[b], st);
+            if (rc == 0) rc = (int)hipStreamWaitEvent(cs, evq[b], 0);
+            if (rc == 0 && k.sym8_dev) rc = (int)hipMemcpyAsync(k.sym8_host, k.sym8_dev, cnt, hipMemcpyDeviceToHost, cs);
+            if (rc == 0 && k.idx_dev) rc = (int)hipMemcpyAsync(k.idx_host, k.idx_dev, cnt, hipMemcpyDeviceToHost, cs);
+        }
+        if (rc == 0 && b == n_blocks - 1 && status_dev && status_host) rc = (int)hipMemcpyAsync(status_host, status_dev, sizeof(int), hipMemcpyDeviceToHost, es);
+        if (rc == 0) rc = (int)hipEventCreateWithFlags(&ev[b], hipEventDisableTiming);
+        if (rc == 0) rc = (int)hipEventRecord(ev[b], es);
+        if (rc != 0) {
+            if (failed_block) *failed_block = b;
+            if (failed_op) *failed_op = bad;
+            drain();
+            cleanup();
+            return rc;
+        }
+    }
+    const double t1 = now_s();
+    std::vector<const int8_t*> sym8_ptr(n_images);
+    std::vector<const int32_t*> sym_ptr(n_images);
+    std::vector<int32_t*> mirror_ptr(n_images);
+    std::vector<const uint8_t*> idx_ptr(n_images);
+    std::vector<size_t> cnt(n_images);
+    std::vector<LvaeEncJob*> jobs(n_blocks, nullptr);
+    double t_wait = 0.0, t_coder = 0.0;
+    int rc_all = 0, bad_block = -1, wide = 0;
+    auto end_jobs = [&]() {
+        for (int b = 0; b < n_blocks; ++b) {
+            if (!jobs[b]) continue;
+            const int rc = lvae_rans_encode_batch_end(jobs[b]);
+            jobs[b] = nullptr;
+            if (rc != 0 && rc_all == 0) { rc_all = rc; bad_block = b; }
+        }
+    };
+    for (int b = 0; b < n_blocks && rc_all == 0; ++b) {
+        const lvae_enc_block8& k = blocks[b];
+        const double tw = now_s();
+        int rc = (int)hipEventSynchronize(ev[b]);
+        t_wait += now_s() - tw;
+        if (rc == 0 && b == n_blocks - 1 && status_dev && status_host && *status_host != 0) rc = (*status_host & LVAE_STATUS_RANGE) ? -34 : -75;
+        if (rc == 0 && *(volatile int*)k.wide != 0) { wide |= 1 << b; continue; }
+        if (rc == 0) {
+            for (int i = 0; i < n_images; ++i) {
+                sym8_ptr[i] = k.sym8_host + (size_t)i * k.per_image;
+                mirror_ptr[i] = k.sym_host + (size_t)i * k.per_image;
+                idx_ptr[i] = k.idx_host + (size_t)i * k.per_image;
+                cnt[i] = k.per_image;
+            }
+            jobs[b] = lvae_rans_encode_batch_begin8(n_images, sym8_ptr.data(), mirror_ptr.data(), idx_ptr.data(), cnt.data(), qcdf, row_stride, cdf_len,
+                                                    offset, out + (size_t)b * n_images, out_cap + (size_t)b * n_images, out_len + (size_t)b * n_images, n_threads);
+            if (!jobs[b]) rc = -12;
+        }
+        if (rc != 0) { rc_all = rc; bad_block = b; }
+    }
+    const double tc = now_s();
+    end_jobs();
+    if (rc_all == 0 && wide != 0) {
+        int rc = (int)hipStreamSynchronize(st);
+        for (int b = 0; b < n_blocks && rc == 0; ++b) {
+            rc = lvae_run_ops(blocks[b].ops, blocks[b].n_ops, stream, side_stream, &bad);
+            if (rc != 0) { bad_block = b; if (failed_op) *failed_op = bad; }
+        }
+        if (rc == 0) rc = (int)hipStreamSynchronize(st);
+        for (int b = 0; b < n_blocks && rc == 0; ++b) {
+            if (!(wide >> b & 1)) continue;
+            const lvae_enc_block8& k = blocks[b];
+            for (int i = 0; i < n_images; ++i) {
+                sym_ptr[i] = k.sym_host + (size_t)i * k.per_image;
+                idx_ptr[i] = k.idx_host + (size_t)i * k.per_image;
+                cnt[i] = k.per_image;
+            }
+            jobs[b] = lvae_rans_encode_batch_begin(n_images, sym_ptr.data(), idx_ptr.data(), cnt.data(), qcdf, row_stride, cdf_len, offset,
+                                                   out + (size_t)b * n_images, out_cap + (size_t)b * n_images, out_len + (size_t)b * n_images, n_threads);
+            if (!jobs[b]) { rc = -12; bad_block = b; }
+        }
+        if (rc != 0 && rc_all == 0) rc_all = rc;
+        end_jobs();
+    }
+    t_coder = now_s() - tc;
+    if (rc_all != 0) {
+        if (failed_block) *failed_block = bad_block;
+        drain();
+        cleanup();
+        return rc_all;
+    }
+    cleanup();
+    if (wide_blocks) *wide_blocks = wide;
+    if (seconds) { seconds[0] = t1 - t0; seconds[1] = t_wait; seconds[2] = t_coder; }
+    return 0;
+}
+
 extern "C" int lvae_decode_blocks(const lvae_dec_block* blocks, int n_blocks, int n_images, const uint8_t* const* strings,
                                   const size_t* string_len, const int32_t* qcdf, int row_stride, const int32_t* cdf_len,
                                   const int32_t* offset, const lvae_op* tail_ops, int n_tail, const int* status_dev, int* status_host,
@@ -204,3 +451,31 @@
         return -12;
     }
 }
+
+extern "C" int lvae_decode_blocks8(const lvae_dec_block8* blocks, int n_blocks, int n_images, const uint8_t* const* strings,
+                                   const size_t* string_len, const int32_t* qcdf, int row_stride, const int32_t* cdf_len,
+                                   const int32_t* offset, const lvae_op* tail_ops, int n_tail, const int* status_dev, int* status_host,
+                                   void* stream, void* side_stream, int n_threads, int* failed_block, int* failed_op, double* seconds,
+                                   int* wide_blocks) {
+    try {
+        return decode_blocks8_impl(blocks, n_blocks, n_images, strings, string_len, qcdf, row_stride, cdf_len, offset, tail_ops, n_tail, status_dev,
+                                   status_host, stream, side_stream, n_threads, failed_block, failed_op, seconds, wide_blocks);
+    } catch (...) {
+        (void)hipStreamSynchronize((hipStream_t)stream);
+        return -12;
+    }
+}
+
+extern "C" int lvae_encode_blocks8(const lvae_enc_block8* blocks, int n_blocks, int n_images, uint8_t* const* out, const size_t* out_cap,
+                                   long* out_len, const int32_t* qcdf, int row_stride, const int32_t* cdf_len, const int32_t* offset,
+                                   const int* status_dev, int* status_host, void* stream, void* side_stream, void* copy_stream, int n_threads,
+                                   int* failed_block, int* failed_op, double* seconds, int* wide_blocks) {
+    try {
+        return encode_blocks8_impl(blocks, n_blocks, n_images, out, out_cap, out_len, qcdf, row_stride, cdf_len, offset, status_dev, status_host,
+                                   stream, side_stream, copy_stream, n_threads, failed_block, failed_op, seconds, wide_blocks);
+    } catch (...) {
+        (void)hipStreamSynchronize((hipStream_t)stream);
+        if (copy_stream) (void)hipStreamSynchronize((hipStream_t)copy_stream);
+        return -12;
+    }
+}
diff --git a/lossy-vae_amd/csrc/pointwise.hip b/lossy-vae_amd/csrc/pointwise.hip
--- a/lossy-vae_amd/csrc/pointwise.hip
+++ b/lossy-vae_amd/csrc/pointwise.hip
@@ -497,11 +497,41 @@
     }
 }
 
-template <bool SK>
-__global__ __launch_bounds__(256) void quantize_kernel(const float* __restrict__ qm, const float* __restrict__ pm, int32_t* __restrict__ sym,
+__device__ __forceinline__ void raster8_store(const int* tile, int8_t* __restrict__ sym, int b, int z, int HW, int c0, int zc, int p0, int np) {
+    const int cl = threadIdx.x >> 2, q0 = (threadIdx.x & 3) * 16;
+    if (cl >= zc || c0 + cl >= z || q0 >= np) return;
+    int8_t* dst = sym + ((long)b * z + c0 + cl) * HW + p0 + q0;
+    const int* src = tile + cl * CT_LD + q0;
+    if (q0 + 16 <= np && ((uintptr_t)dst & 15) == 0) {
+        uint32_t w[4];
+#pragma unroll
+        for (int k = 0; k < 4; ++k)
+            w[k] = (uint32_t)(src[4 * k] & 255) | ((uint32_t)(src[4 * k + 1] & 255) << 8) | ((uint32_t)(src[4 * k + 2] & 255) << 16) | ((uint32_t)src[4 * k + 3] << 24);
+        *reinterpret_cast<uint4*>(dst) = make_uint4(w[0], w[1], w[2], w[3]);
+    } else {
+        for (int k = 0; k < 16 && q0 + k < np; ++k) dst[k] = (int8_t)src[k];
+    }
+}
+__device__ __forceinline__ void raster8_load(int* tile, const int8_t* __restrict__ sym, int b, int z, int HW, int c0, int zc, int p0, int np) {
+    const int cl = threadIdx.x >> 2, q0 = (threadIdx.x & 3) * 16;
+    if (cl >= zc || c0 + cl >= z || q0 >= np) return;
+    const int8_t* src = sym + ((long)b * z + c0 + cl) * HW + p0 + q0;
+    int* dst = tile + cl * CT_LD + q0;
+    if (q0 + 16 <= np && ((uintptr_t)src & 15) == 0) {
+        const uint4 v = *reinterpret_cast<const uint4*>(src);
+        const uint32_t w[4] = {v.x, v.y, v.z, v.w};
+#pragma unroll
+        for (int k = 0; k < 16; ++k) dst[k] = (int)(int8_t)(w[k >> 2] >> (8 * (k & 3)));
+    } else {
+        for (int k = 0; k < 16 && q0 + k < np; ++k) dst[k] = (int)src[k];
+    }
+}
+
+template <bool SK, typename T = int32_t>
+__global__ __launch_bounds__(256) void quantize_kernel(const float* __restrict__ qm, const float* __restrict__ pm, T* __restrict__ sym,
                                                        float* __restrict__ zhat, int HW, int z, int ldz, int* __restrict__ status,
                                                        const float* __restrict__ ws, int S, long plane, const float* __restrict__ bias,
-                                                       float* __restrict__ qm_out) {
+                                                       float* __restrict__ qm_out, int* __restrict__ wide = nullptr) {
 #pragma clang fp contract(off)
     __shared__ int tile[CT_CH * CT_LD];
     const int b = blockIdx.z, p0 = blockIdx.x * CT_PIX, np = (HW - p0) < CT_PIX ? (HW - p0) : CT_PIX;
@@ -527,18 +557,29 @@
             const float r = rintf(q - mu);
             if (status && !(fabsf(r) < 2147483648.0f)) atomicOr(status, LVAE_STATUS_NONFINITE_LATENT);
             zhat[m * ldz + c] = r + mu;
-            tile[(c - c0) * CT_LD + pl] = (int32_t)r;
+            if constexpr (sizeof(T) == 1) {
+                const int32_t ri = (int32_t)r, rs = ri < -128 ? -128 : ri > 127 ? 127 : ri;
+                if (ri != rs) *wide = 1;
+                tile[(c - c0) * CT_LD + pl] = rs;
+            } else {
+                tile[(c - c0) * CT_LD + pl] = (int32_t)r;
+            }
         }
         __syncthreads();
-        for (int j = threadIdx.x; j < zc * CT_PIX; j += 256) {
-            const int cl = j / CT_PIX, pl = j - cl * CT_PIX;
-            if (pl < np && c0 + cl < z) sym[((long)b * z + c0 + cl) * HW + p0 + pl] = tile[cl * CT_LD + pl];
+        if constexpr (sizeof(T) == 1) {
+            raster8_store(tile, sym, b, z, HW, c0, zc, p0, np);
+        } else {
+            for (int j = threadIdx.x; j < zc * CT_PIX; j += 256) {
+                const int cl = j / CT_PIX, pl = j - cl * CT_PIX;
+                if (pl < np && c0 + cl < z) sym[((long)b * z + c0 + cl) * HW + p0 + pl] = tile[cl * CT_LD + pl];
+            }
         }
         __syncthreads();
     }
 }
 
-__global__ __launch_bounds__(256) void dequantize_kernel(const int32_t* __restrict__ sym, const float* __restrict__ pm, float* __restrict__ zhat,
+template <typename T = int32_t>
+__global__ __launch_bounds__(256) void dequantize_kernel(const T* __restrict__ sym, const float* __restrict__ pm, float* __restrict__ zhat,
                                                          int HW, int z, int ldz) {
     __shared__ int tile[CT_CH * CT_LD];
     const int b = blockIdx.z, p0 = blockIdx.x * CT_PIX, np = (HW - p0) < CT_PIX ? (HW - p0) : CT_PIX;
@@ -546,9 +587,13 @@
     {
         const int c0 = blockIdx.y * CT_CH;
         const int zc = (ldz - c0) < CT_CH ? (ldz - c0) : CT_CH;
-        for (int j = threadIdx.x; j < zc * CT_PIX; j += 256) {
-            const int cl = j / CT_PIX, pl = j - cl * CT_PIX;
-            if (pl < np && c0 + cl < z) tile[cl * CT_LD + pl] = sym[((long)b * z + c0 + cl) * HW + p0 + pl];
+        if constexpr (sizeof(T) == 1) {
+            raster8_load(tile, sym, b, z, HW, c0, zc, p0, np);
+        } else {
+            for (int j = threadIdx.x; j < zc * CT_PIX; j += 256) {
+                const int cl = j / CT_PIX, pl = j - cl * CT_PIX;
+                if (pl < np && c0 + cl < z) tile[cl * CT_LD + pl] = sym[((long)b * z + c0 + cl) * HW + p0 + pl];
+            }
         }
         __syncthreads();
         for (int i = threadIdx.x; i < np * zc; i += 256) {
@@ -966,7 +1011,30 @@
 extern "C" int lvae_dequantize_f32(const int32_t* sym, const float* pm, float* zhat, int B, int HW, int z, int ldz,
                                    void* stream) {
     if (!sym || !pm || !zhat || B <= 0 || B > 65535 || HW <= 0 || z <= 0 || ldz < z) return -22;
-    hipLaunchKernelGGL(dequantize_kernel, dim3((unsigned)((HW + CT_PIX - 1) / CT_PIX), (unsigned)((ldz + CT_CH - 1) / CT_CH), (unsigned)B), dim3(256), 0, (hipStream_t)stream, sym, pm,
+    hipLaunchKernelGGL(dequantize_kernel<int32_t>, dim3((unsigned)((HW + CT_PIX - 1) / CT_PIX), (unsigned)((ldz + CT_CH - 1) / CT_CH), (unsigned)B), dim3(256), 0, (hipStream_t)stream, sym, pm,
+                       zhat, HW, z, ldz);
+    return (int)hipGetLastError();
+}
+
+extern "C" int lvae_quantize8_f32(const float* qm, const float* pm, int8_t* sym, float* zhat, int B, int HW, int z, int ldz,
+                                  int* status, int* wide, void* stream) {
+    if (!qm || !pm || !sym || !zhat || !wide || B <= 0 || B > 65535 || HW <= 0 || z <= 0 || ldz < z) return -22;
+    hipLaunchKernelGGL((quantize_kernel<false, int8_t>), dim3((unsigned)((HW + CT_PIX - 1) / CT_PIX), (unsigned)((ldz + CT_CH - 1) / CT_CH), (unsigned)B), dim3(256), 0, (hipStream_t)stream, qm, pm, sym,
+                       zhat, HW, z, ldz, status, (const float*)nullptr, 0, 0L, (const float*)nullptr, (float*)nullptr, wide);
+    return (int)hipGetLastError();
+}
+
+extern "C" int lvae_quantize8_sk_f32(const float* ws, int S, const float* bias, float* qm, const float* pm, int8_t* sym, float* zhat, int B, int HW,
+                                     int z, int ldz, int* status, int* wide, void* stream) {
+    if (!ws || S < 2 || !bias || !qm || !pm || !sym || !zhat || !wide || B <= 0 || B > 65535 || HW <= 0 || z <= 0 || ldz < z) return -22;
+    hipLaunchKernelGGL((quantize_kernel<true, int8_t>), dim3((unsigned)((HW + CT_PIX - 1) / CT_PIX), (unsigned)((ldz + CT_CH - 1) / CT_CH), (unsigned)B), dim3(256), 0, (hipStream_t)stream,
+                       (const float*)nullptr, pm, sym, zhat, HW, z, ldz, status, ws, S, (long)B * HW * z, bias, qm, wide);
+    return (int)hipGetLastError();
+}
+
+extern "C" int lvae_dequantize8_f32(const int8_t* sym, const float* pm, float* zhat, int B, int HW, int z, int ldz, void* stream) {
+    if (!sym || !pm || !zhat || B <= 0 || B > 65535 || HW <= 0 || z <= 0 || ldz < z) return -22;
+    hipLaunchKernelGGL(dequantize_kernel<int8_t>, dim3((unsigned)((HW + CT_PIX - 1) / CT_PIX), (unsigned)((ldz + CT_CH - 1) / CT_CH), (unsigned)B), dim3(256), 0, (hipStream_t)stream, sym, pm,
                        zhat, HW, z, ldz);
     return (int)hipGetLastError();
 }
diff --git a/lossy-vae_amd/csrc/rans_host.cpp b/lossy-vae_amd/csrc/rans_host.cpp
--- a/lossy-vae_amd/csrc/rans_host.cpp
+++ b/lossy-vae_amd/csrc/rans_host.cpp
@@ -167,9 +167,10 @@
 };
 }
 
-extern "C" long lvae_rans_encode_with_indexes(const int32_t* sym, const uint8_t* idx, size_t n,
-                                              const int32_t* qcdf, int row_stride, const int32_t* cdf_len,
-                                              const int32_t* offset, uint8_t* out, size_t out_cap) {
+namespace {
+template <class Sym>
+long encode_stream(const Sym* sym, const uint8_t* idx, size_t n, const int32_t* qcdf, int row_stride, const int32_t* cdf_len,
+                   const int32_t* offset, uint8_t* out, size_t out_cap) {
     if (out_cap < 8) return -2;
     uint8_t* aligned = (uint8_t*)(((uintptr_t)out + 3) & ~(uintptr_t)3);
     const size_t cap_words = (out_cap - (size_t)(aligned - out)) / 4;
@@ -187,7 +188,7 @@
             cur_row = row_i;
         }
         const int32_t max_value = cur->max_value;
-        const int32_t value = sym[ii] - cur->offset;
+        const int32_t value = (int32_t)sym[ii] - cur->offset;
         const bool in_range = value >= 0 && value < max_value;
         EncEnt& e = cur->e[in_range ? value : max_value];
         if (__builtin_expect(!e.ready, 0)) {
@@ -216,6 +217,13 @@
     const size_t nbytes = (size_t)(((uint32_t*)aligned + cap_words) - w.ptr) * 4;
     std::memmove(out, w.ptr, nbytes);
     return (long)nbytes;
+}
+}
+
+extern "C" long lvae_rans_encode_with_indexes(const int32_t* sym, const uint8_t* idx, size_t n,
+                                              const int32_t* qcdf, int row_stride, const int32_t* cdf_len,
+                                              const int32_t* offset, uint8_t* out, size_t out_cap) {
+    return encode_stream(sym, idx, n, qcdf, row_stride, cdf_len, offset, out, out_cap);
 }
 
 extern "C" int lvae_rans_enc_step_selftest(uint64_t x, uint32_t start, uint32_t freq, uint64_t* by_division, uint64_t* by_reciprocal) {
@@ -286,8 +294,13 @@
 constexpr int kMpsCoolWindows = 8;
 constexpr int kMpsCoolMax = 512;
 
+constexpr int kSymbolTooWide = -7;
+template <class Sym>
+inline bool fits(int32_t v) { return sizeof(Sym) == 4 || (uint32_t)(v + 128) <= 255u; }
+
+template <class Sym>
 int decode_stream(const uint8_t* in, size_t in_len, const uint8_t* idx, size_t n, const int32_t* qcdf, int row_stride,
-                  const int32_t* cdf_len, const int32_t* offset, int32_t* sym_out, LvaeDecTabs& D) {
+                  const int32_t* cdf_len, const int32_t* offset, Sym* sym_out, LvaeDecTabs& D) {
     if (in_len < 8 || (in_len & 3)) return -1;
     std::vector<uint32_t> tmp;
     const uint32_t* words;
@@ -329,7 +342,9 @@
                 x = (x << 32) | wv;
                 if (overrun) return -3;
             }
-            sym_out[i] = R.msym + offset[row_i];
+            const int32_t v = R.msym + offset[row_i];
+            if (__builtin_expect(!fits<Sym>(v), 0)) return kSymbolTooWide;
+            sym_out[i] = (Sym)v;
             continue;
         }
         ++miss;
@@ -366,8 +381,10 @@
             if (raw & 1) value = -value - 1;
             else value += R.max_value;
         }
-        sym_out[i] = value + offset[row_i];
         if (overrun) return -3;
+        const int32_t v = (int32_t)((uint32_t)value + (uint32_t)offset[row_i]);
+        if (__builtin_expect(!fits<Sym>(v), 0)) return kSymbolTooWide;
+        sym_out[i] = (Sym)v;
     }
     return 0;
 }
@@ -491,26 +508,37 @@
 }
 
 struct LvaeEncJob {
-    std::vector<const int32_t*> sym;
+    std::vector<const void*> sym;
     std::vector<const uint8_t*> idx;
     std::vector<size_t> n, out_cap;
     std::vector<uint8_t*> out;
+    std::vector<int32_t*> mirror;
     long* out_len = nullptr;
     const int32_t *qcdf = nullptr, *cdf_len = nullptr, *offset = nullptr;
     int row_stride = 0;
+    bool bytes = false;
     std::shared_ptr<Job> job;
     void run(int s) {
-        out_len[s] = lvae_rans_encode_with_indexes(sym[s], idx[s], n[s], qcdf, row_stride, cdf_len, offset, out[s], out_cap[s]);
-    }
-};
-LvaeEncJob* lvae_rans_encode_batch_begin(int n_streams, const int32_t* const* sym, const uint8_t* const* idx, const size_t* n,
-                                         const int32_t* qcdf, int row_stride, const int32_t* cdf_len, const int32_t* offset,
-                                         uint8_t* const* out, const size_t* out_cap, long* out_len, int n_threads) {
+        if (!bytes) {
+            out_len[s] = encode_stream((const int32_t*)sym[s], idx[s], n[s], qcdf, row_stride, cdf_len, offset, out[s], out_cap[s]);
+            return;
+        }
+        const int8_t* b = (const int8_t*)sym[s];
+        out_len[s] = encode_stream(b, idx[s], n[s], qcdf, row_stride, cdf_len, offset, out[s], out_cap[s]);
+        if (!mirror.empty() && mirror[s]) for (size_t i = 0; i < n[s]; ++i) mirror[s][i] = b[i];
+    }
+};
+namespace {
+LvaeEncJob* encode_batch_begin(bool bytes, int n_streams, const void* const* sym, int32_t* const* mirror, const uint8_t* const* idx, const size_t* n,
+                               const int32_t* qcdf, int row_stride, const int32_t* cdf_len, const int32_t* offset,
+                               uint8_t* const* out, const size_t* out_cap, long* out_len, int n_threads) {
     if (n_streams < 0) return nullptr;
     LvaeEncJob* e = new (std::nothrow) LvaeEncJob;
     if (!e) return nullptr;
     try {
+    e->bytes = bytes;
     e->sym.assign(sym, sym + n_streams); e->idx.assign(idx, idx + n_streams); e->n.assign(n, n + n_streams);
+    if (mirror) e->mirror.assign(mirror, mirror + n_streams);
     e->out.assign(out, out + n_streams); e->out_cap.assign(out_cap, out_cap + n_streams);
     e->out_len = out_len; e->qcdf = qcdf; e->cdf_len = cdf_len; e->offset = offset; e->row_stride = row_stride;
     for (int s = 0; s < n_streams; ++s) out_len[s] = 0;
@@ -532,6 +560,17 @@
     }
     return e;
 }
+}
+LvaeEncJob* lvae_rans_encode_batch_begin(int n_streams, const int32_t* const* sym, const uint8_t* const* idx, const size_t* n,
+                                         const int32_t* qcdf, int row_stride, const int32_t* cdf_len, const int32_t* offset,
+                                         uint8_t* const* out, const size_t* out_cap, long* out_len, int n_threads) {
+    return encode_batch_begin(false, n_streams, (const void* const*)sym, nullptr, idx, n, qcdf, row_stride, cdf_len, offset, out, out_cap, out_len, n_threads);
+}
+LvaeEncJob* lvae_rans_encode_batch_begin8(int n_streams, const int8_t* const* sym, int32_t* const* mirror, const uint8_t* const* idx, const size_t* n,
+                                          const int32_t* qcdf, int row_stride, const int32_t* cdf_len, const int32_t* offset,
+                                          uint8_t* const* out, const size_t* out_cap, long* out_len, int n_threads) {
+    return encode_batch_begin(true, n_streams, (const void* const*)sym, mirror, idx, n, qcdf, row_stride, cdf_len, offset, out, out_cap, out_len, n_threads);
+}
 int lvae_rans_encode_batch_end(LvaeEncJob* e) {
     if (!e) return -12;
     const int n = (int)e->sym.size();
@@ -548,11 +587,57 @@
     return rc;
 }
 
+extern "C" int lvae_rans_encode_batch8(int n_streams, const int8_t* const* sym, const uint8_t* const* idx, const size_t* n, const int32_t* qcdf,
+                                       int row_stride, const int32_t* cdf_len, const int32_t* offset, uint8_t* const* out, const size_t* out_cap,
+                                       long* out_len, int n_threads) {
+    if (n_streams < 0) return -22;
+    return lvae_rans_encode_batch_end(lvae_rans_encode_batch_begin8(n_streams, sym, nullptr, idx, n, qcdf, row_stride, cdf_len, offset, out, out_cap, out_len, n_threads));
+}
+
+struct LvaeWidenJob {
+    std::vector<const int8_t*> src;
+    std::vector<int32_t*> dst;
+    std::vector<size_t> n;
+    std::shared_ptr<Job> job;
+    void run(int s) { for (size_t i = 0; i < n[s]; ++i) dst[s][i] = src[s][i]; }
+};
+LvaeWidenJob* lvae_widen_begin(int n_streams, const int8_t* const* src, int32_t* const* dst, const size_t* n) {
+    if (n_streams <= 0) return nullptr;
+    LvaeWidenJob* e = new (std::nothrow) LvaeWidenJob;
+    if (!e) return nullptr;
+    try {
+        e->src.assign(src, src + n_streams); e->dst.assign(dst, dst + n_streams); e->n.assign(n, n + n_streams);
+        auto j = std::make_shared<Job>();
+        j->n = n_streams;
+        j->max_workers = n_streams;
+        j->ctx = (void*)e;
+        j->run = [](void* c, int i) { ((LvaeWidenJob*)c)->run(i); };
+        e->job = j;
+        Pool::get().submit(j);
+    } catch (...) {
+        delete e;
+        return nullptr;
+    }
+    return e;
+}
+void lvae_widen_end(LvaeWidenJob* e) {
+    if (!e) return;
+    Job& j = *e->job;
+    const int n = (int)e->src.size();
+    Pool::work(j);
+    std::unique_lock<std::mutex> l(j.m);
+    j.cv.wait(l, [&] { return j.done.load() >= n; });
+    l.unlock();
+    delete e;
+}
+
 LvaeDecTabs* lvae_dec_tabs_new() { return new (std::nothrow) LvaeDecTabs; }
 void lvae_dec_tabs_free(LvaeDecTabs* t) { delete t; }
-int lvae_rans_decode_batch_tabs(int n_streams, const uint8_t* const* in, const size_t* in_len, const uint8_t* const* idx,
-                                const size_t* n, const int32_t* qcdf, int row_stride, const int32_t* cdf_len, const int32_t* offset,
-                                int32_t* const* sym_out, int* status, int n_threads, LvaeDecTabs* tabs) {
+namespace {
+template <class Sym>
+int decode_batch_tabs(int n_streams, const uint8_t* const* in, const size_t* in_len, const uint8_t* const* idx,
+                      const size_t* n, const int32_t* qcdf, int row_stride, const int32_t* cdf_len, const int32_t* offset,
+                      Sym* const* sym_out, int* status, int n_threads, LvaeDecTabs* tabs) {
     if (n_streams < 0 || !tabs) return -22;
     try {
         parallel_for(n_streams, n_threads, [&](int s) {
@@ -562,8 +647,29 @@
         });
     } catch (...) { return -12; }
     int rc = 0;
-    for (int s = 0; s < n_streams; ++s) if (status[s] < 0) rc = status[s];
+    for (int s = 0; s < n_streams; ++s) if (status[s] < 0 && (rc == 0 || rc == kSymbolTooWide)) rc = status[s];
     return rc;
+}
+}
+int lvae_rans_decode_batch_tabs(int n_streams, const uint8_t* const* in, const size_t* in_len, const uint8_t* const* idx,
+                                const size_t* n, const int32_t* qcdf, int row_stride, const int32_t* cdf_len, const int32_t* offset,
+                                int32_t* const* sym_out, int* status, int n_threads, LvaeDecTabs* tabs) {
+    return decode_batch_tabs(n_streams, in, in_len, idx, n, qcdf, row_stride, cdf_len, offset, sym_out, status, n_threads, tabs);
+}
+int lvae_rans_decode_batch_tabs8(int n_streams, const uint8_t* const* in, const size_t* in_len, const uint8_t* const* idx,
+                                 const size_t* n, const int32_t* qcdf, int row_stride, const int32_t* cdf_len, const int32_t* offset,
+                                 int8_t* const* sym_out, int* status, int n_threads, LvaeDecTabs* tabs) {
+    return decode_batch_tabs(n_streams, in, in_len, idx, n, qcdf, row_stride, cdf_len, offset, sym_out, status, n_threads, tabs);
+}
+
+extern "C" int lvae_rans_decode_batch8(int n_streams, const uint8_t* const* in, const size_t* in_len,
+                                       const uint8_t* const* idx, const size_t* n, const int32_t* qcdf,
+                                       int row_stride, const int32_t* cdf_len, const int32_t* offset,
+                                       int8_t* const* sym_out, int* status, int n_threads) {
+    if (n_streams < 0) return -22;
+    std::unique_ptr<LvaeDecTabs> D(new (std::nothrow) LvaeDecTabs);
+    if (!D) return -12;
+    return lvae_rans_decode_batch_tabs8(n_streams, in, in_len, idx, n, qcdf, row_stride, cdf_len, offset, sym_out, status, n_threads, D.get());
 }
 
 extern "C" int lvae_rans_decode_batch(int n_streams, const uint8_t* const* in, const size_t* in_len,
diff --git a/lossy-vae_amd/lvae/_native/__init__.py b/lossy-vae_amd/lvae/_native/__init__.py
--- a/lossy-vae_amd/lvae/_native/__init__.py
+++ b/lossy-vae_amd/lvae/_native/__init__.py
@@ -49,6 +49,16 @@
                 ('idx_host', C.c_void_p), ('per_image', C.c_size_t)]
 
 
+class DecBlock8(C.Structure):
+    _fields_ = [('ops', C.c_void_p), ('n_ops', C.c_int), ('idx_host', C.c_void_p), ('sym8_host', C.c_void_p), ('sym_host', C.c_void_p),
+                ('per_image', C.c_size_t)]
+
+
+class EncBlock8(C.Structure):
+    _fields_ = [('ops', C.c_void_p), ('n_ops', C.c_int), ('sym8_dev', C.c_void_p), ('sym8_host', C.c_void_p), ('sym_host', C.c_void_p),
+                ('idx_dev', C.c_void_p), ('idx_host', C.c_void_p), ('wide', C.c_void_p), ('per_image', C.c_size_t)]
+
+
 OP_KINDS = {name: k + 1 for k, name in enumerate([
     'lvae_gemm_f32', 'lvae_dwconv_ln_f32', 'lvae_dwconv_ln_h2', 'lvae_dwconv_ln_bf16', 'lvae_dwconv_ln_q8', 'lvae_stem_f32', 'lvae_stem_bf16',
     'lvae_bias_expand_f32', 'lvae_bias_expand_bf16', 'lvae_prior_index_f32', 'lvae_quantize_f32', 'lvae_dequantize_f32',
@@ -58,6 +68,7 @@
 OP_ORDER = len(OP_KINDS) + 1
 
 TRACE_MAGIC = 1985229328.0
+RANS_SYMBOL_TOO_WIDE = -7
 A_PLAIN, A_PATCH2, A_CONV3 = 0, 1, 2
 STATUS_RANGE, STATUS_NONFINITE_PRIOR, STATUS_NONFINITE_LATENT, STATUS_NONFINITE_IMAGE = 1, 2, 4, 8
 EPI_BIAS, EPI_BIAS_GELU, EPI_GAMMA_RES, EPI_RES = 0, 1, 2, 3
@@ -80,6 +91,8 @@
     'lvae_rans_enc_step_selftest': (_i, [C.c_uint64, C.c_uint32, C.c_uint32, _vp, _vp]),
     'lvae_rans_encode_batch': (_i, [_i, _vp, _vp, _vp, _vp, _i, _vp, _vp, _vp, _vp, _vp, _i]),
     'lvae_rans_decode_batch': (_i, [_i, _vp, _vp, _vp, _vp, _vp, _i, _vp, _vp, _vp, _vp, _i]),
+    'lvae_rans_encode_batch8': (_i, [_i, _vp, _vp, _vp, _vp, _i, _vp, _vp, _vp, _vp, _vp, _i]),
+    'lvae_rans_decode_batch8': (_i, [_i, _vp, _vp, _vp, _vp, _vp, _i, _vp, _vp, _vp, _vp, _i]),
     'lvae_gemm_f32': (_i, [C.POINTER(GemmDesc), _vp]),
     'lvae_gemm_num_configs': (_i, []),
     'lvae_gemm_h2_choice': (_i, [C.POINTER(GemmDesc), _i, _vp, _vp, _vp]),
@@ -107,6 +120,9 @@
     'lvae_quantize_sk_f32': (_i, [_vp, _i, _vp, _vp, _vp, _vp, _vp, _i, _i, _i, _i, _vp, _vp]),
     'lvae_quantize_f32': (_i, [_vp, _vp, _vp, _vp, _i, _i, _i, _i, _vp, _vp]),
     'lvae_dequantize_f32': (_i, [_vp, _vp, _vp, _i, _i, _i, _i, _vp]),
+    'lvae_quantize8_sk_f32': (_i, [_vp, _i, _vp, _vp, _vp, _vp, _vp, _i, _i, _i, _i, _vp, _vp, _vp]),
+    'lvae_quantize8_f32': (_i, [_vp, _vp, _vp, _vp, _i, _i, _i, _i, _vp, _vp, _vp]),
+    'lvae_dequantize8_f32': (_i, [_vp, _vp, _vp, _i, _i, _i, _i, _vp]),
     'lvae_lossless_params_f32': (_i, [_vp, _vp, _vp, _vp, _vp, _vp, _i, _f, _i, _i, _i, _vp, _vp]),
     'lvae_lossless_output_f32': (_i, [_vp, _vp, _vp, C.c_long, _vp, _vp]),
     'lvae_prior_sample_f32': (_i, [_vp, _vp, C.c_long, _i, _i, C.c_float, C.c_ulonglong, C.c_ulonglong, _vp]),
@@ -124,6 +140,8 @@
     'lvae_run_ops': (_i, [_vp, _i, _vp, _vp, _vp]),
     'lvae_decode_blocks': (_i, [_vp, _i, _i, _vp, _vp, _vp, _i, _vp, _vp, _vp, _i, _vp, _vp, _vp, _vp, _i, _vp, _vp, _vp]),
     'lvae_encode_blocks': (_i, [_vp, _i, _i, _vp, _vp, _vp, _vp, _i, _vp, _vp, _vp, _vp, _vp, _vp, _i, _vp, _vp, _vp]),
+    'lvae_decode_blocks8': (_i, [_vp, _i, _i, _vp, _vp, _vp, _i, _vp, _vp, _vp, _i, _vp, _vp, _vp, _vp, _i, _vp, _vp, _vp, _vp]),
+    'lvae_encode_blocks8': (_i, [_vp, _i, _i, _vp, _vp, _vp, _vp, _i, _vp, _vp, _vp, _vp, _vp, _vp, _vp, _i, _vp, _vp, _vp, _vp]),
     'lvae_sqerr_sum_f32': (_i, [_vp, _vp, _vp, _i, _l, _vp]),
     'lvae_sqerr_partials_f32': (_i, [_vp, _vp, _vp, _i, _l, _vp]),
     'lvae_msssim_f32': (_i, [_vp, _l, _l, _l, _vp, _l, _l, _l, _vp, _i, _i, _i, _i, _vp, _vp, _vp, _sz, _vp]),
diff --git a/lossy-vae_amd/lvae/models/base.py b/lossy-vae_amd/lvae/models/base.py
--- a/lossy-vae_amd/lvae/models/base.py
+++ b/lossy-vae_amd/lvae/models/base.py
@@ -186,6 +186,11 @@
             self.sym_host = torch.empty(n_sym, dtype=torch.int32).pin_memory()
             self.idx_host = torch.empty(n_sym, dtype=torch.uint8).pin_memory()
             self.sym_np, self.idx_np = self.sym_host.numpy(), self.idx_host.numpy()
+            self.sym8_all = self.new(n_sym, torch.int8)
+            self.sym8_host = torch.empty(n_sym, dtype=torch.int8).pin_memory()
+            self.wide_host = torch.zeros(32, dtype=torch.int32).pin_memory()
+            self.wide_blocks = {}
+            self.copy_stream = None
 
     def alloc_pos(self):
         self.pos_bufs = [self.new(self.B * hw, torch.float64) for _, hw in self.lat_shapes]
@@ -236,6 +241,7 @@
 class CodecBase(nn.Module):
     def _init_codec_base(self):
         self.coder_threads = 0
+        self.symbol_bytes = 1
         self.pipeline_groups = int(os.environ.get('LVAE_GROUPS', '2'))
         self.enc_groups = int(os.environ.get('LVAE_ENC_GROUPS', '0'))
         self.dec_groups = int(os.environ.get('LVAE_DEC_GROUPS', '0'))
@@ -301,12 +307,15 @@
                          type(self).__name__, self._prec, ' (package default)' if self._prec == DEFAULT_PRECISION else ' (set explicitly)')
 
     native_group_loops = True
+    enc_link_copies = False
 
 
     @staticmethod
-    def _alias_host(pl, seg, n_ops):
+    def _alias_host(pl, seg, n_ops, idx=True):
         raster_ops = {_native.OP_KINDS[k] for k in ('lvae_prior_index_f32', 'lvae_prior_index_sk_f32', 'lvae_quantize_f32', 'lvae_quantize_sk_f32', 'lvae_dequantize_f32')}
-        spans = [(pl.sym_all.data_ptr(), pl.sym_all.numel() * 4, pl.sym_host.data_ptr()), (pl.idx_all.data_ptr(), pl.idx_all.numel(), pl.idx_host.data_ptr())]
+        spans = [(pl.sym_all.data_ptr(), pl.sym_all.numel() * 4, pl.sym_host.data_ptr())]
+        if idx:
+            spans.append((pl.idx_all.data_ptr(), pl.idx_all.numel(), pl.idx_host.data_ptr()))
         out = (_native.Op * max(1, n_ops))()
         ctypes.memmove(out, seg, ctypes.sizeof(_native.Op) * n_ops)
         for o in out[:n_ops]:
@@ -321,23 +330,33 @@
         return out
 
     @classmethod
-    def _group_blocks(cls_, pl, kind, cuts, offs, n):
-        key = '_native_blocks_' + kind
+    def _group_blocks(cls_, pl, kind, cuts, offs, n, sym8=False, copies=False):
+        copies = bool(copies and sym8 and kind == 'enc')
+        key = '_native_blocks_' + kind + ('8' if sym8 else '') + ('c' if copies else '')
         cached = getattr(pl, key, None)
         if cached is None:
-            cls = _native.DecBlock if kind == 'dec' else _native.EncBlock
+            if sym8:
+                cls = _native.DecBlock8 if kind == 'dec' else _native.EncBlock8
+            else:
+                cls = _native.DecBlock if kind == 'dec' else _native.EncBlock
             arr = (cls * len(cuts))()
             segs, lo = [], 0
             for li, cut in enumerate(cuts):
                 seg, n_ops = pl._segment(lo, cut)
-                seg = cls_._alias_host(pl, seg, n_ops)
+                seg = cls_._alias_host(pl, seg, n_ops, idx=not copies)
                 segs.append(seg)
                 z, hw = pl.lat_shapes[li]
                 o = offs[li]
                 b = arr[li]
                 b.ops, b.n_ops, b.per_image = ctypes.cast(seg, ctypes.c_void_p).value, n_ops, z * hw
-                b.idx_dev, b.idx_host = None, pl.idx_host.data_ptr() + o
-                b.sym_dev, b.sym_host = None, pl.sym_host.data_ptr() + 4 * o
+                b.idx_host, b.sym_host = pl.idx_host.data_ptr() + o, pl.sym_host.data_ptr() + 4 * o
+                if sym8:
+                    b.sym8_host = pl.sym8_host.data_ptr() + o
+                    if kind == 'enc':
+                        b.wide = pl.wide_host.data_ptr() + 4 * li
+                        b.sym8_dev, b.idx_dev = (pl.sym8_all.data_ptr() + o, pl.idx_all.data_ptr() + o) if copies else (None, None)
+                else:
+                    b.idx_dev, b.sym_dev = None, None
                 lo = cut
             tail, n_tail = pl._segment(lo, len(pl.ops)) if kind == 'dec' else (None, 0)
             if n_tail:
@@ -351,8 +370,15 @@
             setattr(pl, key, cached)
         return cached
 
+    def _symbol_bytes(self):
+        sb = getattr(self, 'symbol_bytes', 1)
+        if sb not in (1, 4):
+            raise ValueError(f'symbol_bytes is 1 (int8 over the host link) or 4 (int32), not {sb!r}')
+        return sb
+
     def _decode_group_native(self, pl, cuts, offs, n, strings, tables, nthreads, stream, T=None):
-        arr, segs, tail, n_tail, early = self._group_blocks(pl, 'dec', cuts, offs, n)
+        sym8 = self._symbol_bytes() == 1
+        arr, segs, tail, n_tail, early = self._group_blocks(pl, 'dec', cuts, offs, n, sym8=sym8)
         nb = len(cuts)
         if early is not None:
             with torch.cuda.device(pl.device):
@@ -380,11 +406,16 @@
             secs[0], secs[1] = -64.0, _native.TRACE_MAGIC
         ss = pl.side_stream.cuda_stream if pl.side_stream is not None else None
         st_dev = pl.status_ptr()
+        wide = ctypes.c_int(0)
+        args = (arr, nb, n, sp, sl, qcdf.ctypes.data, qcdf.shape[1], cdf_len.ctypes.data, offset.ctypes.data,
+                ctypes.cast(tail, ctypes.c_void_p) if n_tail else None, n_tail, st_dev, pl.status_host.data_ptr(), ctypes.c_void_p(stream.cuda_stream),
+                ctypes.c_void_p(ss) if ss is not None else None, int(nthreads), ctypes.byref(fb), ctypes.byref(fo), secs)
         with torch.cuda.device(pl.device):
-            rc = _native.lib().lvae_decode_blocks(arr, nb, n, sp, sl, qcdf.ctypes.data, qcdf.shape[1], cdf_len.ctypes.data, offset.ctypes.data,
-                                                  ctypes.cast(tail, ctypes.c_void_p) if n_tail else None, n_tail, st_dev, pl.status_host.data_ptr(),
-                                                  ctypes.c_void_p(stream.cuda_stream),
-                                                  ctypes.c_void_p(ss) if ss is not None else None, int(nthreads), ctypes.byref(fb), ctypes.byref(fo), secs)
+            if sym8:
+                rc = _native.lib().lvae_decode_blocks8(*args, ctypes.byref(wide))
+                pl.wide_blocks['dec'] = wide.value
+            else:
+                rc = _native.lib().lvae_decode_blocks(*args)
         if rc != 0:
             stream.synchronize()
             word = int(pl.status_host[0]) if rc == -75 else 0
@@ -401,7 +432,8 @@
             T['dec_rans'] = T.get('dec_rans', 0) + secs[1]
 
     def _encode_group_native(self, pl, cuts, offs, n, tables, nthreads, stream, T=None):
-        arr, _segs, _tail, _nt, _early = self._group_blocks(pl, 'enc', cuts, offs, n)
+        sym8 = self._symbol_bytes() == 1
+        arr, _segs, _tail, _nt, _early = self._group_blocks(pl, 'enc', cuts, offs, n, sym8=sym8, copies=self.enc_link_copies)
         nb = len(cuts)
         qcdf, cdf_len, offset = tables
         caps = [8 * pl.lat_shapes[li][0] * pl.lat_shapes[li][1] + 64 for li in range(nb)]
@@ -415,10 +447,19 @@
         secs = (ctypes.c_double * 3)()
         ss = pl.side_stream.cuda_stream if pl.side_stream is not None else None
         st_dev = pl.status_ptr()
+        head = (arr, nb, n, op, oc, out_len, qcdf.ctypes.data, qcdf.shape[1], cdf_len.ctypes.data, offset.ctypes.data, st_dev, pl.status_host.data_ptr(),
+                ctypes.c_void_p(stream.cuda_stream), ctypes.c_void_p(ss) if ss is not None else None)
+        tail_ = (int(nthreads), ctypes.byref(fb), ctypes.byref(fo), secs)
         with torch.cuda.device(pl.device):
-            rc = _native.lib().lvae_encode_blocks(arr, nb, n, op, oc, out_len, qcdf.ctypes.data, qcdf.shape[1], cdf_len.ctypes.data, offset.ctypes.data,
-                                                  st_dev, pl.status_host.data_ptr(), ctypes.c_void_p(stream.cuda_stream),
-                                                  ctypes.c_void_p(ss) if ss is not None else None, int(nthreads), ctypes.byref(fb), ctypes.byref(fo), secs)
+            if sym8:
+                if pl.copy_stream is None and self.enc_link_copies:
+                    pl.copy_stream = torch.cuda.Stream(device=pl.device)
+                wide = ctypes.c_int(0)
+                cs = ctypes.c_void_p(pl.copy_stream.cuda_stream) if pl.copy_stream is not None else None
+                rc = _native.lib().lvae_encode_blocks8(*head, cs, *tail_, ctypes.byref(wide))
+                pl.wide_blocks['enc'] = wide.value
+            else:
+                rc = _native.lib().lvae_encode_blocks(*head, *tail_)
         if rc in (-34, -75):
             word = int(pl.status_host[0])
             self._reset_status(pl)
```

After: 176.8 Mpixels/s (median of 3 runs). Within noise of the previous version (+1.1%).
